# ChenyangQiQi/FateZero

Hardware: AMD Instinct MI355X
Metric: edited frames/sec (8f x 512^2 x 50 DDIM steps: capture inversion + 1 CFG edit, latents in/out) (higher is better)
Workload: dtype fp16; 1 GPU; config/teaser/jeep_posche.yaml shape: 8 x 512x512 (latents 8x64x64x4), 50-step DDIM inversion with HBM map capture + 50-step CFG edit (Replace, blend-masked self-attention), SD-1.x pseudo-3D UNet lora=160, random-init weights; frames=8, ddim_steps=50, n_edit=1, parallelism=single GPU, outputs_finite=True, n_ranks_seen=1

## Files before the change

fatezero_amd/_native.py:

```python
import ctypes as C
import os

HERE = os.path.dirname(os.path.abspath(__file__))
HIP_LIB = os.path.join(HERE, "libfatezero_hip.so")

FZ_ATTN_FLASH, FZ_ATTN_CAPTURE, FZ_ATTN_INJECT = 0, 1, 2
FZ_ATTN_CAPTURE8, FZ_ATTN_INJECT8 = 3, 4
FZ_MAX_KV_SLOTS = 4
FZ_CROSS_MAX_KEYS = 96
FZ_CROSS_P_STRIDE = 80
FZ_TEMPORAL_MAX_FRAMES = 256


class FzAttnSelfDesc(C.Structure):
    _fields_ = [
        ("n_frames", C.c_int32), ("frame0", C.c_int32), ("clip_len", C.c_int32), ("heads", C.c_int32),
        ("head_dim", C.c_int32), ("lq", C.c_int32), ("lkf", C.c_int32), ("n_kv", C.c_int32),
        ("kv_abs", C.c_int32 * FZ_MAX_KV_SLOTS), ("kv_val", C.c_int32 * FZ_MAX_KV_SLOTS),
        ("scale", C.c_float), ("mode", C.c_int32),
        ("q_frame_stride", C.c_int64), ("q_row_stride", C.c_int64),
        ("k_frame_stride", C.c_int64), ("k_row_stride", C.c_int64),
        ("vt_frame_stride", C.c_int64), ("vt_chan_stride", C.c_int64),
        ("o_frame_stride", C.c_int64), ("o_row_stride", C.c_int64),
        ("p_frame_stride", C.c_int64), ("p_head_stride", C.c_int64), ("p_row_stride", C.c_int64),
        ("p_frame_off", C.c_int32), ("mask_frame_off", C.c_int32),
        ("k_head_stride", C.c_int64),
        ("q_log2_scaled", C.c_int32), ("kv_clip_len", C.c_int32), ("kv_frame_off", C.c_int32), ("reserved0", C.c_int32),
    ]


class FzAttnCrossDesc(C.Structure):
    _fields_ = [
        ("n_frames", C.c_int32), ("frame0", C.c_int32), ("clip_len", C.c_int32), ("heads", C.c_int32),
        ("head_dim", C.c_int32), ("lq", C.c_int32), ("lk", C.c_int32),
        ("scale", C.c_float), ("mode", C.c_int32),
        ("q_frame_stride", C.c_int64), ("q_row_stride", C.c_int64),
        ("k_batch_stride", C.c_int64), ("k_row_stride", C.c_int64),
        ("vt_batch_stride", C.c_int64), ("vt_chan_stride", C.c_int64),
        ("o_frame_stride", C.c_int64), ("o_row_stride", C.c_int64),
        ("p_frame_stride", C.c_int64), ("p_head_stride", C.c_int64), ("p_row_stride", C.c_int64),
        ("p_frame_off", C.c_int32), ("store_cur", C.c_int32),
    ]


class FzGemmDesc(C.Structure):
    _fields_ = [
        ("rows", C.c_int64), ("rows_store", C.c_int64), ("in_features", C.c_int32), ("out_features", C.c_int32),
        ("ldx", C.c_int64), ("ldw", C.c_int64), ("ldy", C.c_int64), ("ldres", C.c_int64),
        ("batch", C.c_int32), ("epilogue", C.c_int32),
        ("x_batch_stride", C.c_int64), ("y_batch_stride", C.c_int64), ("res_batch_stride", C.c_int64),
        ("transpose_out", C.c_int32), ("tile_cfg", C.c_int32), ("split_k", C.c_int32), ("reserved0", C.c_int32),
        ("workspace_floats", C.c_int64), ("w_batch_stride", C.c_int64),
    ]


class FzXattnChain(C.Structure):
    _fields_ = [
        ("x", C.c_void_p), ("res", C.c_void_p), ("packed", C.c_void_p), ("kv_packed", C.c_void_p), ("bias_out", C.c_void_p),
        ("y", C.c_void_p), ("y_ln", C.c_void_p), ("ln_gamma", C.c_void_p), ("ln_beta", C.c_void_p),
        ("y1", C.c_void_p),
        ("rows", C.c_int64), ("rows_per_frame", C.c_int64),
        ("frames_per_batch", C.c_int32), ("channels", C.c_int32), ("heads", C.c_int32), ("lk", C.c_int32),
        ("scale", C.c_float), ("ln_eps", C.c_float), ("ln1_eps", C.c_float), ("front", C.c_int32),
    ]


FZ_GEMM_PLAIN, FZ_GEMM_GEGLU = 0, 1
FZ_GEMM_NO_STATS = 1

_P = C.c_void_p
_SIGS = {
    "fz_gemm": (C.c_int, [C.POINTER(FzGemmDesc), _P, _P, _P, _P, _P, _P, _P, _P]),
    "fz_ff_chain_ok": (C.c_int, [C.c_int64, C.c_int, C.c_int]),
    "fz_ff_chain_preferred": (C.c_int, [C.c_int64, C.c_int, C.c_int]),
    "fz_ff_chain_pack_bytes": (C.c_int64, [C.c_int, C.c_int]),
    "fz_ff_chain_pack": (C.c_int, [_P, _P, _P, _P, C.c_int, C.c_int, _P]),
    "fz_ff_chain": (C.c_int, [_P, _P, _P, _P, _P, _P, _P, C.c_float, _P, C.c_int64, C.c_int, C.c_int, _P]),
    "fz_xattn_chain_ok": (C.c_int, [C.c_int64, C.c_int64, C.c_int, C.c_int, C.c_int]),
    "fz_xattn_chain_preferred": (C.c_int, [C.c_int64, C.c_int64, C.c_int, C.c_int, C.c_int]),
    "fz_xattn_chain_pack_bytes": (C.c_int64, [C.c_int]),
    "fz_xattn_chain_kv_pack_bytes": (C.c_int64, [C.c_int]),
    "fz_xattn_chain_pack": (C.c_int, [_P, _P, _P, _P, _P, _P, _P, _P]),
    "fz_xattn_chain_kv_pack": (C.c_int, [_P, C.c_int64, C.c_int64, _P, C.c_int64, C.c_int64, C.c_int, C.c_int, _P, _P]),
    "fz_xattn_chain": (C.c_int, [C.POINTER(FzXattnChain), _P]),
    "fz_gemm_lnout": (C.c_int, [C.POINTER(FzGemmDesc), _P, _P, _P, _P, _P, _P, _P, _P, C.c_float, _P, C.c_int64, _P, _P]),
    "fz_gemm_qkvt": (C.c_int, [C.POINTER(FzGemmDesc), _P, _P, _P, _P, C.c_int, C.c_int64, C.c_int64, C.c_int64, _P]),
    "fz_gn_epilogue_chunks": (C.c_int, [C.c_int64]),
    "fz_gemm_gn": (C.c_int, [C.POINTER(FzGemmDesc), _P, _P, _P, _P, _P, _P, _P, C.c_int, C.c_int64, _P]),
    "fz_temporal_conv3_gn": (C.c_int, [_P, _P, _P, _P, _P, C.c_int64, _P, C.c_int, C.c_int, C.c_int, C.c_int, C.c_int, _P, C.c_int64,
                                       _P, C.c_int, _P]),
    "fz_groupnorm_from_partials": (C.c_int, [_P, _P, _P, _P, C.c_int, C.c_int, C.c_int, C.c_int, C.c_int, C.c_float, C.c_int, _P,
                                             C.c_int, _P, _P]),
    "fz_gemm_workspace_floats": (C.c_int64, [C.c_int64, C.c_int, C.c_int]),
    "fz_attn_self": (C.c_int, [C.POINTER(FzAttnSelfDesc), _P, _P, _P, _P, _P, _P, _P]),
    "fz_attn_cross": (C.c_int, [C.POINTER(FzAttnCrossDesc), _P, _P, _P, _P, _P, _P, _P, _P, _P]),
    "fz_attn_temporal": (C.c_int, [_P, _P, _P, _P, C.c_int, C.c_int, C.c_int, C.c_int, C.c_int, C.c_int64,
                                   C.c_int64, C.c_float, _P]),
    "fz_attn_temporal_ex": (C.c_int, [_P, _P, _P, _P, C.c_int, C.c_int, C.c_int, C.c_int, C.c_int, C.c_int, C.c_int64,
                                      C.c_int64, C.c_int64, C.c_float, _P]),
    "fz_blend_mask": (C.c_int, [_P, C.c_int, C.c_int, C.c_int64, C.c_int, C.c_int, C.c_int, C.c_int64, _P,
                                C.c_float, C.c_int, C.c_int, C.c_int, _P, _P, _P]),
    "fz_groupnorm_chunks": (C.c_int, [C.c_int, C.c_int]),
    "fz_groupnorm": (C.c_int, [_P, _P, _P, _P, C.c_int, C.c_int, C.c_int, C.c_int, C.c_int, C.c_float, C.c_int,
                               _P, _P]),
    "fz_groupnorm_cat": (C.c_int, [_P, C.c_int, _P, C.c_int, _P, _P, _P, C.c_int, C.c_int, C.c_int, C.c_int, C.c_float, C.c_int,
                                   _P, _P]),
    "fz_groupnorm_stats": (C.c_int, [_P, C.c_int, C.c_int, C.c_int, C.c_int, _P, _P]),
    "fz_groupnorm_apply": (C.c_int, [_P, _P, _P, _P, C.c_int, C.c_int, C.c_int, C.c_int, C.c_int, C.c_float, C.c_int, _P,
                                     C.c_int, C.c_int, _P, _P]),
    "fz_conv3x3_up2_ok": (C.c_int, [C.c_int, C.c_int, C.c_int, C.c_int, C.c_int]),
    "fz_conv3x3_up2_preferred": (C.c_int, [C.c_int, C.c_int, C.c_int, C.c_int, C.c_int]),
    "fz_conv3x3_up2_pack_halves": (C.c_int64, [C.c_int, C.c_int]),
    "fz_conv3x3_up2_pack": (C.c_int, [_P, _P, C.c_int, C.c_int, _P]),
    "fz_conv3x3_up2": (C.c_int, [_P, _P, _P, _P, C.c_int, C.c_int, C.c_int, C.c_int, C.c_int, _P]),
    "fz_conv3x3": (C.c_int, [_P, _P, _P, _P, C.c_int64, _P, _P, C.c_int, C.c_int, C.c_int, C.c_int, C.c_int, C.c_int,
                             C.c_int, C.c_int, _P, C.c_int64, C.c_int, C.c_int, _P]),
    "fz_temporal_conv3": (C.c_int, [_P, _P, _P, _P, _P, C.c_int64, _P, C.c_int, C.c_int, C.c_int, C.c_int, C.c_int, _P, C.c_int64,
                                    _P]),
    "fz_lora_pair_ok": (C.c_int, [C.c_int, C.c_int, C.c_int, C.c_int, C.c_int]),
    "fz_lora_pair_preferred": (C.c_int, [C.c_int, C.c_int, C.c_int, C.c_int, C.c_int]),
    "fz_lora_pair_gn_chunks": (C.c_int, [C.c_int, C.c_int, C.c_int, C.c_int, C.c_int, C.c_int]),
    "fz_lora_pair_gn": (C.c_int, [_P, _P, _P, _P, C.c_int64, _P, _P, C.c_int, C.c_int, C.c_int, C.c_int, C.c_int, _P, C.c_int, _P]),
    "fz_lora_pair": (C.c_int, [_P, _P, _P, _P, C.c_int64, _P, _P, C.c_int, C.c_int, C.c_int, C.c_int, C.c_int, _P]),
    "fz_layernorm": (C.c_int, [_P, _P, _P, _P, C.c_int64, C.c_int, C.c_float, _P]),
    "fz_geglu": (C.c_int, [_P, _P, C.c_int64, C.c_int, _P]),
    "fz_softmax_rows": (C.c_int, [_P, _P, C.c_int64, C.c_int, C.c_int64, C.c_int64, C.c_float, _P]),
    "fz_transpose_pad": (C.c_int, [_P, _P, C.c_int, C.c_int, C.c_int, C.c_int64, C.c_int64, C.c_int, _P]),
    "fz_latent_update": (C.c_int, [_P, _P, _P, C.c_float, C.c_float, C.c_float, _P, _P, _P, C.c_int, C.c_int, _P]),
    "fz_accumulate": (C.c_int, [_P, _P, C.c_int64, _P]),
    "fz_peer_put": (C.c_int, [_P, C.c_int64, _P, _P, C.c_int, C.c_uint32, _P, _P]),
    "fz_peer_wait": (C.c_int, [_P, C.c_uint64, C.c_uint32, _P, C.c_int64, _P]),
    "fz_plan_begin": (C.c_int, [C.POINTER(_P)]),
    "fz_plan_pause": (C.c_int, [_P, C.c_int]),
    "fz_plan_end": (C.c_int, [_P]),
    "fz_plan_launches": (C.c_int64, [_P]),
    "fz_plan_relocate": (C.c_int64, [_P, C.c_int64, C.c_int64, _P, C.c_int64, _P]),
    "fz_plan_replay": (C.c_int, [_P, C.c_int64, C.c_int64, _P]),
    "fz_plan_graph_launch": (C.c_int, [_P, _P]),
    "fz_plan_destroy": (None, [_P]),
    "fz_version": (C.c_char_p, []),
}

_lib = None
_lib_path = None
_is_test_backend = False


class NativeLibraryError(RuntimeError):
    pass


def _open(path):
    if not os.path.exists(path):
        raise NativeLibraryError(
            f"{path} is missing: build it with `python -m fatezero_amd.build` (hipcc --offload-arch=gfx950). "
            "The FateZero hot path has no CPU fallback.")
    try:
        lib = C.CDLL(path)
    except OSError as e:
        raise NativeLibraryError(f"cannot load {path}: {e}") from e
    for name, (res, args) in _SIGS.items():
        try:
# ... 43 lines not shown
```

fatezero_amd/csrc/elementwise.hip:

```cpp
#include "fz_rt.h"
#include "../../include/fatezero_hip.h"

FZ_KERNEL void __launch_bounds__(256) geglu_kernel(const half_t* __restrict__ x, half_t* __restrict__ y, int64_t rows, int inner) {
    const int vper = inner >> 3;
    const int64_t total = rows * vper;
    for (int64_t i = (int64_t)blockIdx.x * blockDim.x + threadIdx.x; i < total; i += (int64_t)gridDim.x * blockDim.x) {
        const int64_t r = i / vper;
        const int v = (int)(i % vper);
        const half8_t hv = fz_ld_h8(x + r * 2 * inner + v * 8);
        const half8_t gv = fz_ld_h8(x + r * 2 * inner + inner + v * 8);
        half8_t o;
#pragma unroll
        for (int e = 0; e < 8; ++e) {
            const float g = (float)gv[e];
            const float ge = fz_gelu_erf(g);
            o[e] = (half_t)((float)hv[e] * ge);
        }
        fz_st_h8(y + r * inner + v * 8, o);
    }
}

extern "C" int fz_geglu(const void* x, void* y, int64_t rows, int inner, void* stream) {
    if (!x || !y || rows <= 0 || inner <= 0 || (inner & 7)) return FZ_ERR_BAD_ARG;
    const int64_t total = rows * (inner >> 3);
// ... 139 lines not shown
        nx[c] = (half_t)zn;
    }
    if (next_in != nullptr) *reinterpret_cast<half4_t*>(next_in + i * 4) = nx;
}

extern "C" int fz_latent_update(float* z, const void* eps_u, const void* eps_c, float guidance, float cz, float ce,
                                const float* inv, const float* mask, void* next_in, int frames, int hw, void* stream) {
    if (!z || !eps_c || frames <= 0 || hw <= 0) return FZ_ERR_BAD_ARG;
    if ((mask != nullptr) != (inv != nullptr)) return FZ_ERR_BAD_ARG;
    const int64_t total = (int64_t)frames * hw;
    FZ_LAUNCH(latent_update_kernel, dim3((unsigned)((total + 255) / 256)), dim3(256), 0, stream, z, (const half_t*)eps_u,
              (const half_t*)eps_c, guidance, cz, ce, inv, mask, (half_t*)next_in, frames, hw);
    return fz_last_launch_status();
}

FZ_KERNEL void __launch_bounds__(256) accumulate_kernel(float* __restrict__ acc, const half_t* __restrict__ x, int64_t n8) {
    for (int64_t i = (int64_t)blockIdx.x * blockDim.x + threadIdx.x; i < n8; i += (int64_t)gridDim.x * blockDim.x) {
        const half8_t v = fz_ld_h8(x + i * 8);
        float* a = acc + i * 8;
#pragma unroll
        for (int e = 0; e < 8; ++e) a[e] += (float)v[e];
    }
}

extern "C" int fz_accumulate(float* acc, const void* x, int64_t n, void* stream) {
    if (!acc || !x || n <= 0 || (n & 7)) return FZ_ERR_BAD_ARG;
    const int64_t n8 = n >> 3;
    int blocks = (int)((n8 + 255) / 256);
    if (blocks > 4096) blocks = 4096;
    FZ_LAUNCH(accumulate_kernel, dim3(blocks), dim3(256), 0, stream, acc, (const half_t*)x, n8);
    return fz_last_launch_status();
}

extern "C" const char* fz_version(void) {
#ifdef FZ_EMU
    return "fatezero_amd 0.1 (CPU emulation build -- tests only)";
#else
    return "fatezero_amd 0.1 (hip gfx950)";
#endif
}
```

fatezero_amd/csrc/igemm.hip:

```cpp
#include "fz_rt.h"
#include <type_traits>
#include <atomic>
#include <utility>
#include <stdlib.h>
#include "../../include/fatezero_hip.h"

#ifdef FZ_IGEMM_TRIALS
__attribute__((weak)) int fz_igemm_trial_no_pp = 0;
extern "C" { __attribute__((weak)) int fz_igemm_trial_no_kg2 = 0; __attribute__((weak)) int fz_igemm_trial_no_halo = 0; __attribute__((weak)) int fz_igemm_trial_no_halo_split = 0; }
__attribute__((weak)) int fz_igemm_trial_pp_splitk_min = 0;
#endif
#ifdef FZ_IGEMM_TUNING
#define FZ_TUNING_FLAG(name) (getenv(name) != nullptr)
#else
#define FZ_TUNING_FLAG(name) false
#endif
#ifndef FZ_A_AUX
#define FZ_A_AUX 0
#endif
#define FZ_PP_ON 1
#define FZ_PP_NOPRIO 2
#define FZ_PP_NOSTAGGER 4
#define FZ_PP_PREP_IN_R 8
#define FZ_PP_K32 16
// ... 4 lines not shown
#ifdef FZ_IGEMM_TIMING
__device__ long long fz_igemm_timing[2][8];
__device__ long long fz_igemm_timing2[2][6];
#define FZ_TK_DECL() long long tacc_[8] = {0, 0, 0, 0, 0, 0, 0, 0}
#define FZ_TK(i)                              \
    __builtin_amdgcn_sched_barrier(0);        \
    const long long tk##i = clock64();        \
    __builtin_amdgcn_sched_barrier(0)
#define FZ_TK_ADD(slot, a, b) tacc_[slot] += (b) - (a)
#define FZ_TK_FLUSH()                                                                                      \
    do {                                                                                                   \
        if (blockIdx.x == 0 && blockIdx.y == 0 && blockIdx.z == 0 && (tid & 255) == 0)                     \
            for (int s_ = 0; s_ < 8; ++s_) fz_igemm_timing[tid >> 8][s_] = tacc_[s_];                       \
    } while (0)
#else
#define FZ_TK_DECL() ((void)0)
#define FZ_TK(i) ((void)0)
#define FZ_TK_ADD(slot, a, b) ((void)0)
#define FZ_TK_FLUSH() ((void)0)
#endif

FZ_DEVICE_GLOBAL __attribute__((aligned(16))) half_t fz_zero_page[8192];

struct IgArgs {
    const half_t* a;
    const half_t* b;
    half_t* y;
    float* part;
    const half_t* bias;
    const half_t* temb;
    const half_t* res;
    const half_t* res2;
    int64_t lda, ldb, ldy, ldres, a_bs, b_bs, y_bs, res_bs, temb_stride;
    int64_t Nb;
    int64_t temb_group;
    int Ma, Ma_store;
    int Cin, taps, kchunks;
    int N, Hi, Wi, Ho, Wo, stride, upsample, fpb;
    int ksplit, tiles_a;
    int group_b;
    int tiles_b;
    int nt_flat;
    half_t* yt;
    int64_t yt_bs, ldyt;
    int vt_split, vt_rows;
    float* gs_out;
    int gs_cpg, gs_groups, gs_chunks, gs_rpf;
    half_t* lno_y;
    const half_t* lno_gamma;
    const half_t* lno_beta;
    int64_t lno_ld;
    float lno_eps;
};

template <int WA, int TA, int WB, int TB, int BK, int NS, bool GEGLU, int PP = 0>
struct IgCfg {
    static_assert(BK == 32 || BK == 64, "K step of 32 or 64 halves");
    static_assert(!(PP & FZ_PP_ON) || (BK == 32 && NS == 4 && WA * WB == 8), "ping-pong loop: K step 32, 4 slots, 8 waves = two groups of 4");
    static constexpr bool LC = (PP & FZ_LC) != 0;
    static_assert(!LC || (!(PP & (FZ_PP_ON | FZ_KG2)) && BK == 32 && NS == 4 && WA * WB == 4), "loader / consumer loop: K step 32, 4 slots, 4 + 4 waves");
    static constexpr int KG = (PP & FZ_KG2) ? 2 : 1;
    static constexpr bool KGPP = (PP & FZ_KGPP) != 0;
    static_assert(KG == 1 || (!(PP & FZ_PP_ON) && (KGPP ? (BK == 32 && NS == 4) : BK == 64)), "K groups: ring loop with K step 64, or their own ping-pong loop");
    static_assert(!KGPP || KG == 2, "the K-group ping-pong loop needs the two groups");
    static constexpr int NWG = WA * WB;
    static constexpr int NW = (LC ? 2 : KG) * NWG, T = 64 * NW;
// ... 796 lines not shown
                            *reinterpret_cast<half4_t*>(crow + (wa * TA / 2 + i / 2) * 32 + 8 * gq + 4 * hi) = v;
                        }
                } else {
#pragma unroll
                    for (int i = 0; i < TA; ++i)
#pragma unroll
                        for (int gq = 0; gq < 4; ++gq) {
                            half4_t v;
                            if constexpr (VT) {
                                f32x2 pk;
                                pk[0] = acc[i][j][4 * gq];
                                pk[1] = acc[i][j][4 * gq + 1];
                                v = __builtin_bit_cast(half4_t, pk);
                            } else {
#pragma unroll
                                for (int e = 0; e < 4; ++e) v[e] = (half_t)acc[i][j][4 * gq + e];
                            }
                            *reinterpret_cast<half4_t*>(crow + (wa * TA + i) * 32 + 8 * gq + 4 * hi) = v;
                        }
                }
            }
        }
        __syncthreads();
        for (int id = tid; id < C::RP * OCH; id += C::T) {
            const int pl = id / OCH, ch = id - pl * OCH;
            const int64_t px = b0 + ps * C::RP + pl;
            const int co = o0 + ch * 8;
            if (px >= g.Nb || co >= Mo_store) continue;
            const half8_t v = fz_ld_h8(Cs + pl * C::CSTR + ch * 8);
            float f[8];
#pragma unroll
            for (int e = 0; e < 8; ++e) f[e] = co + e < Mo ? (float)v[e] : 0.0f;
            const bool full = vec_ok && co + 8 <= Mo;
            if (full) {
                if (g.temb != nullptr) {
                    const half8_t t = fz_ld_h8(g.temb + (px / g.temb_group) * g.temb_stride + co);
#pragma unroll
                    for (int e = 0; e < 8; ++e) f[e] += (float)t[e];
                }
                if (R1 != nullptr) {
                    const half8_t r = fz_ld_h8(R1 + px * g.ldres + co);
#pragma unroll
                    for (int e = 0; e < 8; ++e) f[e] += (float)r[e];
                }
                if (R2 != nullptr) {
                    const half8_t r = fz_ld_h8(R2 + px * g.ldres + co);
#pragma unroll
                    for (int e = 0; e < 8; ++e) f[e] += (float)r[e];
                }
            } else {
                if (g.temb != nullptr) {
                    const half_t* t = g.temb + (px / g.temb_group) * g.temb_stride + co;
                    for (int e = 0; e < 8; ++e)
                        if (co + e < Mo) f[e] += (float)t[e];
                }
                if (R1 != nullptr) {
                    const half_t* r = R1 + px * g.ldres + co;
                    for (int e = 0; e < 8; ++e)
                        if (co + e < Mo) f[e] += (float)r[e];
                }
                if (R2 != nullptr) {
                    const half_t* r = R2 + px * g.ldres + co;
                    for (int e = 0; e < 8; ++e)
                        if (co + e < Mo) f[e] += (float)r[e];
                }
            }
            half_t* dst = Y + px * g.ldy + co;
            if (full) {
                half8_t o;
#pragma unroll
                for (int e = 0; e < 8; ++e) o[e] = (half_t)f[e];
                fz_st_h8(dst, o);
                if constexpr (GS != 0) fz_st_h8(Cs + pl * C::CSTR + ch * 8, o);
            } else {
#pragma unroll
                for (int e = 0; e < 8; ++e)
                    if (co + e < Mo_store) dst[e] = (half_t)f[e];
            }
        }
        if constexpr (GS == -1) {
            static_assert(C::CW == 320, "the tile must hold whole 320-channel rows");
            __syncthreads();
            const int l8 = tid & 7;
            FzRow5 gmv, btv;
#pragma unroll
            for (int i = 0; i < 5; ++i) {
                gmv.c[i] = fz_ld_h8(g.lno_gamma + (l8 + 8 * i) * 8);
                btv.c[i] = fz_ld_h8(g.lno_beta + (l8 + 8 * i) * 8);
            }
            for (int rb = tid >> 3; rb < C::RP; rb += C::T >> 3) {
// ... 58 lines not shown
                float* out = g.gs_out + ((fr * g.gs_groups + (a0 / cpg + tid)) * g.gs_chunks + chunk) * 3;
                out[0] = cnt;
                out[1] = mean;
                out[2] = m2;
            }
        }
    }
#ifdef FZ_IGEMM_TIMING
    if (blockIdx.x == 0 && blockIdx.y == 0 && blockIdx.z == 0 && (tid & 255) == 0) {
        fz_igemm_timing2[tid >> 8][0] = tk_setup;
        fz_igemm_timing2[tid >> 8][1] = clock64() - tk_entry;
        fz_igemm_timing2[tid >> 8][2] = tw_entry;
        fz_igemm_timing2[tid >> 8][3] = tw_loop;
        fz_igemm_timing2[tid >> 8][4] = tw_loop_end;
        fz_igemm_timing2[tid >> 8][5] = wall_clock64();
    }
#endif
}

FZ_KERNEL void __launch_bounds__(256) igemm_reduce_kernel(IgArgs g, int batch) {
    const int q = g.Ma / 4;
    const int cl = threadIdx.x & 63, rl = fz_uniform((int)(threadIdx.x >> 6));
    const int64_t rows = g.Nb * batch;
    for (int64_t row = (int64_t)blockIdx.x * 4 + rl; row < rows; row += (int64_t)gridDim.x * 4) {
        int z = 0;
        int64_t px = row;
        if (batch > 1) {
            z = (int)(row / g.Nb);
            px = row - (int64_t)z * g.Nb;
        }
        const float* const p0 = g.part + row * g.Ma;
        const int64_t slab = (int64_t)batch * g.Nb * g.Ma;
        const half_t* const trow = g.temb != nullptr ? g.temb + (px / g.temb_group) * g.temb_stride : nullptr;
        const half_t* const r1 = g.res != nullptr ? g.res + (int64_t)z * g.res_bs + px * g.ldres : nullptr;
        const half_t* const r2 = g.res2 != nullptr ? g.res2 + (int64_t)z * g.res_bs + px * g.ldres : nullptr;
        half_t* const yrow = g.y + (int64_t)z * g.y_bs + px * g.ldy;
        const int c4 = (int)blockIdx.y * 64 + cl;
        if (c4 < q) {
            const int co = c4 * 4;
            f32x4 s = *reinterpret_cast<const f32x4*>(p0 + co);
            for (int k = 1; k < g.ksplit; ++k) {
                const f32x4 t = *reinterpret_cast<const f32x4*>(p0 + k * slab + co);
                s += t;
            }
            float f[4] = {s[0], s[1], s[2], s[3]};
            if (g.bias != nullptr)
                for (int e = 0; e < 4; ++e) f[e] += (float)g.bias[co + e];
            if (trow != nullptr)
                for (int e = 0; e < 4; ++e) f[e] += (float)trow[co + e];
            if (r1 != nullptr)
                for (int e = 0; e < 4; ++e) f[e] += (float)r1[co + e];
            if (r2 != nullptr)
                for (int e = 0; e < 4; ++e) f[e] += (float)r2[co + e];
            half4_t o;
            for (int e = 0; e < 4; ++e) o[e] = (half_t)f[e];
            *reinterpret_cast<half4_t*>(yrow + co) = o;
        }
    }
}

template <int CIN>
FZ_KERNEL void __launch_bounds__(256) conv3x3_small_cin_kernel(IgArgs g) {
    FZ_DYN_SMEM(raw);
    half_t* wl = reinterpret_cast<half_t*>(raw);
    const int kk = 9 * g.Cin;
    for (int id = threadIdx.x; id < kk * g.Ma; id += 256) {
        const int k = id / g.Ma, co = id - k * g.Ma;
// ... 336 lines not shown
        if (GEGLU || workspace == nullptr || (g.Ma % 4) || g.Ma_store != g.Ma || (g.ldy % 4)) return FZ_ERR_UNSUPPORTED;
        if ((int64_t)ksplit * batch * g.Nb * g.Ma > workspace_floats) return FZ_ERR_BAD_ARG;
        g.part = workspace;
    }
    const int rc = ig_dispatch_cfg<MODE, GEGLU>(cfg, g, batch, stream);
    if (rc != FZ_OK || ksplit == 1) return rc != FZ_OK ? rc : (gs_dropped ? FZ_GEMM_NO_STATS : FZ_OK);
    const int64_t rblocks = (g.Nb * batch + 3) / 4;
    dim3 grid((unsigned)(rblocks < 16384 ? rblocks : 16384), (unsigned)((g.Ma / 4 + 63) / 64)), block(256);
    FZ_LAUNCH(igemm_reduce_kernel, grid, block, 0, stream, g, batch);
    const int rc2 = fz_last_launch_status();
    return rc2 != FZ_OK ? rc2 : (gs_dropped ? FZ_GEMM_NO_STATS : FZ_OK);
}

extern "C" int64_t fz_gemm_workspace_floats(int64_t rows, int out_features, int batch) {
    const int64_t out = rows * (int64_t)out_features * (batch > 0 ? batch : 1);
    const int64_t cap = 64ll << 20;
    return 8 * out < cap ? 8 * out : (2 * out < cap ? cap : 2 * out);
}

extern "C" int fz_gemm(const FzGemmDesc* d, const void* x, const void* w, const void* bias, const void* res, const void* res2,
                       void* y, void* workspace, void* stream) {
    if (!d || !x || !w || !y || d->rows <= 0 || d->in_features <= 0 || d->out_features <= 0) return FZ_ERR_BAD_ARG;
    const int batch = d->batch > 0 ? d->batch : 1;
    IgArgs g = {};
    g.taps = 1;
    g.fpb = 1;
    g.Cin = d->in_features;
    g.temb = nullptr;
    g.temb_group = 1;
    g.res = (const half_t*)res;
    g.res2 = (const half_t*)res2;
    g.ldres = d->ldres ? d->ldres : d->ldy;
    g.res_bs = d->res_batch_stride;
    g.y = (half_t*)y;
    g.ldy = d->ldy;
    g.y_bs = d->y_batch_stride;
    if (d->ldx < d->in_features || d->ldw < d->in_features || (d->ldx % 8) || (d->ldw % 8)) return FZ_ERR_BAD_ARG;
    const bool geglu = d->epilogue == FZ_GEMM_GEGLU;
    if (d->epilogue != FZ_GEMM_PLAIN && !geglu) return FZ_ERR_BAD_ARG;
    if (!d->transpose_out) {
        g.a = (const half_t*)w;
        g.lda = d->ldw;
        g.a_bs = d->w_batch_stride;
        g.Ma = d->out_features;
        g.Ma_store = d->out_features;
        g.b = (const half_t*)x;
        g.ldb = d->ldx;
        g.b_bs = d->x_batch_stride;
        g.Nb = d->rows;
        g.bias = (const half_t*)bias;
        const int outw = geglu ? d->out_features / 2 : d->out_features;
        if (d->ldy < outw) return FZ_ERR_BAD_ARG;
        if (geglu) {
            if (d->out_features % 64 || res || res2) return FZ_ERR_UNSUPPORTED;
            return ig_run<0, true>(g, batch, d->tile_cfg, 1, nullptr, 0, stream);
        }
        return ig_run<0, false>(g, batch, d->tile_cfg, d->split_k, (float*)workspace, d->workspace_floats, stream);
    }
    if (geglu || bias || res || res2) return FZ_ERR_UNSUPPORTED;
    if (d->rows >= (1ll << 31)) return FZ_ERR_UNSUPPORTED;
    g.a = (const half_t*)x;
    g.lda = d->ldx;
    g.a_bs = d->x_batch_stride;
    g.Ma = (int)d->rows;
    g.Ma_store = d->rows_store > d->rows ? (int)d->rows_store : (int)d->rows;
    g.b = (const half_t*)w;
// ... 107 lines not shown
        (g.ldy % 8) || (g.ldres % 8) || (g.temb != nullptr && (g.temb_stride % 8))) return false;
    g.gs_out = partial;
    g.gs_cpg = cpg;
    g.gs_groups = groups;
    g.gs_rpf = (int)rows_per_frame;
    g.gs_chunks = (int)(rows_per_frame / 128);
    return true;
}

extern "C" int fz_gn_epilogue_chunks(int64_t rows_per_frame) { return rows_per_frame % 128 == 0 ? (int)(rows_per_frame / 128) : 0; }

extern "C" int fz_gemm_gn(const FzGemmDesc* d, const void* x, const void* w, const void* bias, const void* res, const void* res2, void* y,
                          float* gn_partial, int gn_groups, int64_t rows_per_frame, void* stream) {
    if (!d || !x || !w || !y || !gn_partial || d->rows <= 0 || d->in_features <= 0 || d->out_features <= 0) return FZ_ERR_BAD_ARG;
    if (d->epilogue != FZ_GEMM_PLAIN || d->transpose_out || d->batch > 1 || d->w_batch_stride) return FZ_ERR_UNSUPPORTED;
    if (d->ldx < d->in_features || d->ldw < d->in_features || (d->ldx % 8) || (d->ldw % 8) || d->ldy < d->out_features) return FZ_ERR_BAD_ARG;
    IgArgs g = {};
    g.taps = 1;
    g.fpb = 1;
    g.Cin = d->in_features;
    g.temb_group = 1;
    g.a = (const half_t*)w;
    g.lda = d->ldw;
    g.Ma = g.Ma_store = d->out_features;
    g.b = (const half_t*)x;
    g.ldb = d->ldx;
    g.Nb = d->rows;
    g.bias = (const half_t*)bias;
    g.res = (const half_t*)res;
    g.res2 = (const half_t*)res2;
    g.y = (half_t*)y;
    g.ldy = d->ldy;
    g.ldres = d->ldres ? d->ldres : d->ldy;
    const bool want = ig_gs_setup(g, gn_partial, gn_groups, rows_per_frame);
    const int rc = ig_run<0, false>(g, 1, d->tile_cfg, 1, nullptr, 0, stream);
    return rc != FZ_OK ? rc : (want ? FZ_OK : FZ_GEMM_NO_STATS);
}

extern "C" int fz_gemm_lnout(const FzGemmDesc* d, const void* x, const void* w, const void* bias, const void* res, const void* res2, void* y,
                             const void* gamma, const void* beta, float eps, void* y_ln, int64_t ld_ln, void* workspace, void* stream) {
    if (!d || !x || !w || !y || !gamma || !beta || !y_ln || d->rows <= 0 || d->in_features <= 0 || d->out_features <= 0) return FZ_ERR_BAD_ARG;
    if (d->epilogue != FZ_GEMM_PLAIN || d->transpose_out || d->batch > 1 || d->w_batch_stride) return FZ_ERR_UNSUPPORTED;
    if (d->ldx < d->in_features || d->ldw < d->in_features || (d->ldx % 8) || (d->ldw % 8) || d->ldy < d->out_features || ld_ln < d->out_features)
        return FZ_ERR_BAD_ARG;
    IgArgs g = {};
    g.taps = 1;
    g.fpb = 1;
    g.Cin = d->in_features;
    g.temb_group = 1;
    g.a = (const half_t*)w;
    g.lda = d->ldw;
    g.Ma = g.Ma_store = d->out_features;
    g.b = (const half_t*)x;
    g.ldb = d->ldx;
    g.Nb = d->rows;
    g.bias = (const half_t*)bias;
    g.res = (const half_t*)res;
    g.res2 = (const half_t*)res2;
    g.y = (half_t*)y;
    g.ldy = d->ldy;
    g.ldres = d->ldres ? d->ldres : d->ldy;
    g.lno_y = (half_t*)y_ln;
    g.lno_gamma = (const half_t*)gamma;
    g.lno_beta = (const half_t*)beta;
    g.lno_ld = ld_ln;
    g.lno_eps = eps;
    return ig_run<0, false>(g, 1, d->tile_cfg, d->split_k, (float*)workspace, d->workspace_floats, stream);
}

static int temporal_conv3_impl(const void* x, const void* wt, const void* res, const void* res2, const void* temb, int64_t temb_stride,
                               void* y, int n, int tokens, int cin, int cout, int clip_len, void* workspace, int64_t workspace_floats,
                               float* gn_partial, int gn_groups, void* stream);

extern "C" int fz_temporal_conv3_gn(const void* x, const void* wt, const void* res, const void* res2, const void* temb,
                                    int64_t temb_stride, void* y, int n, int tokens, int cin, int cout, int clip_len, void* workspace,
                                    int64_t workspace_floats, float* gn_partial, int gn_groups, void* stream) {
    if (!gn_partial || gn_groups <= 0) return FZ_ERR_BAD_ARG;
    return temporal_conv3_impl(x, wt, res, res2, temb, temb_stride, y, n, tokens, cin, cout, clip_len, workspace, workspace_floats,
                               gn_partial, gn_groups, stream);
}

extern "C" int fz_temporal_conv3(const void* x, const void* wt, const void* res, const void* res2, const void* temb,
                                int64_t temb_stride, void* y, int n, int tokens, int cin, int cout, int clip_len,
                                void* workspace, int64_t workspace_floats, void* stream) {
    return temporal_conv3_impl(x, wt, res, res2, temb, temb_stride, y, n, tokens, cin, cout, clip_len, workspace, workspace_floats, nullptr,
                               0, stream);
}

static int temporal_conv3_impl(const void* x, const void* wt, const void* res, const void* res2, const void* temb, int64_t temb_stride,
                               void* y, int n, int tokens, int cin, int cout, int clip_len, void* workspace, int64_t workspace_floats,
                               float* gn_partial, int gn_groups, void* stream) {
    if (!x || !wt || !y || n <= 0 || tokens <= 0 || clip_len <= 0 || n % clip_len) return FZ_ERR_BAD_ARG;
    IgArgs g = {};
    g.taps = 3;
// ... 97 lines not shown
```

fatezero_amd/csrc/norms.hip:

```cpp
#include "fz_rt.h"
#include "../../include/fatezero_hip.h"
#include <stdlib.h>

static int gn_tb(int tokens, int channels) {
    const int V = channels / 8;
    const int R = V >= 256 ? 1 : 256 / (V > 0 ? V : 1);
    int tb = 64;
    while (tb > 8 && tb > 16 * R) tb >>= 1;
    while (tb > 8 && tokens / tb < 32) tb >>= 1;
    return tb;
}

extern "C" int fz_groupnorm_chunks(int tokens, int channels) {
    const int tb = gn_tb(tokens, channels);
    return (tokens + tb - 1) / tb;
}

struct GnArgs {
    const half_t* x;
    const half_t* x2;
    int C1;
    half_t* y;
    const half_t *gamma, *beta;
    float* partial;
    float* stats;
    int n_frames, span, tokens, C, G, chunks, V, R;
    int tb;
    int fin_span;
    int pchunks;
    float eps;
    int silu;
};

template <int ROWS>
FZ_KERNEL void __launch_bounds__(ROWS > 0 ? 512 : 1024) gn_stats_kernel(GnArgs a) {
    FZ_DYN_SMEM(raw);
    float* red = reinterpret_cast<float*>(raw);
    float* gmean = red + a.R * a.C;
    const int tid = threadIdx.x, v = tid % a.V, r = tid / a.V;
    const int chunk = blockIdx.x, n = blockIdx.y;
    const int t0 = chunk * a.tb;
    const int t1 = min(t0 + a.tb, a.tokens);
    const int cg = a.C / a.G;
    const float cnt = (float)((t1 - t0) * cg);
    const bool second = v * 8 >= a.C1;
    const int64_t rs = second ? a.C - a.C1 : a.C1;
    const half_t* base = (second ? a.x2 + ((int64_t)n * a.tokens) * rs + (v * 8 - a.C1) : a.x + ((int64_t)n * a.tokens) * rs + v * 8);
    float s[8];
#pragma unroll
    for (int e = 0; e < 8; ++e) s[e] = 0.0f;
    half8_t xr[ROWS > 0 ? ROWS : 1];
    if (ROWS > 0) {
#pragma unroll
        for (int i = 0; i < ROWS; ++i) {
            int t = t0 + r + i * a.R;
            t = t < t1 ? t : t1 - 1;
            xr[i] = fz_ld_h8(base + (int64_t)t * rs);
        }
#pragma unroll
        for (int i = 0; i < ROWS; ++i) {
            if (t0 + r + i * a.R < t1) {
#pragma unroll
                for (int e = 0; e < 8; ++e) s[e] += (float)xr[i][e];
            }
        }
    } else {
        for (int t = t0 + r; t < t1; t += a.R) {
            const half8_t xv = fz_ld_h8(base + (int64_t)t * rs);
#pragma unroll
            for (int e = 0; e < 8; ++e) s[e] += (float)xv[e];
        }
    }
#pragma unroll
    for (int e = 0; e < 8; ++e) red[r * a.C + v * 8 + e] = s[e];
    __syncthreads();
    if (tid < a.G) {
        float sum = 0.0f;
        for (int rr = 0; rr < a.R; ++rr)
            for (int c = tid * cg; c < (tid + 1) * cg; ++c) sum += red[rr * a.C + c];
        gmean[tid] = sum / cnt;
// ... 116 lines not shown
    const int sp = (int)blockIdx.x / a.G, g = (int)blockIdx.x % a.G;
    const int wave = threadIdx.x >> 6, lane = threadIdx.x & 63;
    const int total = a.fin_span * a.pchunks, per = (total + 3) / 4;
    float cnt, mean, m2;
    gn_merge_range(a, sp, g, lane, min(wave * per, total), min((wave + 1) * per, total), cnt, mean, m2);
    if (lane == 0) { part[wave][0] = cnt; part[wave][1] = mean; part[wave][2] = m2; }
    __syncthreads();
    if (threadIdx.x == 0) {
        cnt = part[0][0]; mean = part[0][1]; m2 = part[0][2];
        for (int w = 1; w < 4; ++w) chan_merge(cnt, mean, m2, part[w][0], part[w][1], part[w][2]);
        a.stats[(sp * a.G + g) * 2 + 0] = mean;
        a.stats[(sp * a.G + g) * 2 + 1] = 1.0f / sqrtf(m2 / cnt + a.eps);
    }
}

FZ_KERNEL void gn_apply_kernel(GnArgs a) {
    const int tid = threadIdx.x, v = tid % a.V, r = tid / a.V;
    const int chunk = blockIdx.x, n = blockIdx.y;
    const int t0 = chunk * a.tb;
    const int t1 = min(t0 + a.tb, a.tokens);
    const int cg = a.C / a.G;
    const int sp = n / a.span;
    float sc[8], sh[8];
    const half8_t gv = fz_ld_h8(a.gamma + v * 8), bv = fz_ld_h8(a.beta + v * 8);
#pragma unroll
    for (int e = 0; e < 8; ++e) {
        const int g = (v * 8 + e) / cg;
        const float mean = a.stats[(sp * a.G + g) * 2 + 0], rstd = a.stats[(sp * a.G + g) * 2 + 1];
        sc[e] = rstd * (float)gv[e];
        sh[e] = (float)bv[e] - mean * sc[e];
    }
    const bool second = v * 8 >= a.C1;
    const int64_t rs = second ? a.C - a.C1 : a.C1;
    const half_t* xb = (second ? a.x2 + ((int64_t)n * a.tokens) * rs + (v * 8 - a.C1) : a.x + ((int64_t)n * a.tokens) * rs + v * 8);
    half_t* yb = a.y + ((int64_t)n * a.tokens) * a.C + v * 8;
#pragma unroll 4
    for (int t = t0 + r; t < t1; t += a.R) {
        const half8_t xv = fz_ld_h8(xb + (int64_t)t * rs);
        half8_t yv;
#pragma unroll
        for (int e = 0; e < 8; ++e) {
            float f = (float)xv[e] * sc[e] + sh[e];
            if (a.silu) f = f / (1.0f + __builtin_expf(-f));
            yv[e] = (half_t)f;
        }
        fz_st_h8(yb + (int64_t)t * a.C, yv);
    }
}

#define GN_FUSED_THREADS 1024
#define GN_FUSED_MAX_NE 20
#define GN_FUSED_MAX_PAIRS (GN_FUSED_THREADS * GN_FUSED_MAX_NE)

FZ_DEVICE float gn_block_sum(float v, float* red, int tid) {
#pragma unroll
    for (int msk = 1; msk < 64; msk <<= 1) v += fz_shfl_xor(v, msk);
    __syncthreads();
    if ((tid & 63) == 0) red[tid >> 6] = v;
    __syncthreads();
    float s = 0.0f;
#pragma unroll
    for (int w = 0; w < GN_FUSED_THREADS / 64; ++w) s += red[w];
    return s;
}

template <int NE>
FZ_KERNEL void __launch_bounds__(GN_FUSED_THREADS) gn_fused_kernel(GnArgs a) {
    FZ_SHARED float red[GN_FUSED_THREADS / 64];
    FZ_SHARED float gsc[128], gsh[128];
    const int tid = threadIdx.x;
    const int sp = (int)blockIdx.x / a.G, g = (int)blockIdx.x % a.G;
    const int cg = a.C / a.G, P = cg >> 1;
    const int total = a.span * a.tokens * P;
    const int c0 = g * cg;
    const int64_t row0 = (int64_t)sp * a.span * a.tokens;
    const uint32_t rs1 = (uint32_t)a.C1, rs2 = (uint32_t)(a.C - a.C1);
    const half_t* const src1 = a.x + row0 * a.C1;
    const half_t* const src2 = a.x2 != nullptr ? a.x2 + row0 * (a.C - a.C1) : src1;
    half_t* const dst = a.y + row0 * a.C + c0;
    const int drow = GN_FUSED_THREADS / P, dpr = GN_FUSED_THREADS - drow * P;
    const int row = tid / P, pr = tid - row * P;
    const int last_row = a.span * a.tokens - 1;
    half2_t v[NE];
    {
        int r = row, q = pr;
#pragma unroll
        for (int i = 0; i < NE; ++i) {
            const int rr = r < last_row ? r : last_row;
            const uint32_t ch = (uint32_t)(c0 + 2 * q);
            const half_t* p = ch >= rs1 ? src2 + ((uint32_t)rr * rs2 + (ch - rs1)) : src1 + ((uint32_t)rr * rs1 + ch);
            v[i] = *reinterpret_cast<const half2_t*>(p);
            FZ_SCHED_FENCE();
            r += drow;
            q += dpr;
            if (q >= P) { q -= P; ++r; }
        }
    }
    const float cnt = (float)total * 2.0f;
    float s = 0.0f;
#pragma unroll
    for (int i = 0; i < NE; ++i)
        if (tid + GN_FUSED_THREADS * i < total) s += (float)v[i][0] + (float)v[i][1];
    const float mean = gn_block_sum(s, red, tid) / cnt;
#pragma unroll
    for (int i = 0; i < NE; ++i) FZ_PIN_V(v[i]);
    s = 0.0f;
#pragma unroll
    for (int i = 0; i < NE; ++i)
        if (tid + GN_FUSED_THREADS * i < total) {
            const float d0 = (float)v[i][0] - mean, d1 = (float)v[i][1] - mean;
            s += d0 * d0 + d1 * d1;
// ... 19 lines not shown
                float f1 = (float)v[i][1] * gsc[2 * q + 1] + gsh[2 * q + 1];
                if (a.silu) {
                    f0 = f0 / (1.0f + __builtin_expf(-f0));
                    f1 = f1 / (1.0f + __builtin_expf(-f1));
                }
                half2_t o;
                o[0] = (half_t)f0;
                o[1] = (half_t)f1;
                *reinterpret_cast<half2_t*>(dst + ((uint32_t)r * (uint32_t)a.C + 2u * (uint32_t)q)) = o;
            }
            FZ_SCHED_FENCE();
            r += drow;
            q += dpr;
            if (q >= P) { q -= P; ++r; }
        }
    }
}

#ifdef FZ_GN_TRIALS
template <int NE>
FZ_KERNEL void __launch_bounds__(GN_FUSED_THREADS) gn_fused2_kernel(GnArgs a) {
    FZ_SHARED float red[GN_FUSED_THREADS / 64];
    const int tid = threadIdx.x;
    const int sp = (int)blockIdx.x / a.G, g = (int)blockIdx.x % a.G;
    const int cg = a.C / a.G, P = cg >> 1;
    const int R = GN_FUSED_THREADS / P;
    const int rows = a.span * a.tokens;
    const int r0 = tid / P, q = tid - r0 * P;
    const bool active = r0 < R;
    const int ch = g * cg + 2 * q;
    const int64_t row0 = (int64_t)sp * rows;
    const bool second = ch >= a.C1;
    const uint32_t rs = (uint32_t)(second ? a.C - a.C1 : a.C1);
    const half_t* const src = second ? a.x2 + row0 * (a.C - a.C1) + (ch - a.C1) : a.x + row0 * a.C1 + ch;
    half_t* const dst = a.y + row0 * a.C + ch;
    const uint32_t step_in = (uint32_t)R * rs, step_out = (uint32_t)R * (uint32_t)a.C;
    const int r_first = active ? r0 : 0;
    half2_t v[NE];
    {
        uint32_t off = (uint32_t)r_first * rs;
        const uint32_t off_max = (uint32_t)(rows - 1) * rs;
#pragma unroll
        for (int i = 0; i < NE; ++i) {
            v[i] = *reinterpret_cast<const half2_t*>(src + (off < off_max ? off : off_max));
            FZ_SCHED_FENCE();
            off += step_in;
        }
    }
    const int r_lim = active ? rows - r0 : 0;
    const float cnt = (float)rows * (float)cg;
    float s = 0.0f;
#pragma unroll
    for (int i = 0; i < NE; ++i)
        if (i * R < r_lim) s += (float)v[i][0] + (float)v[i][1];
    const float mean = gn_block_sum(s, red, tid) / cnt;
#pragma unroll
    for (int i = 0; i < NE; ++i) FZ_PIN_V(v[i]);
    s = 0.0f;
#pragma unroll
    for (int i = 0; i < NE; ++i)
        if (i * R < r_lim) {
            const float d0 = (float)v[i][0] - mean, d1 = (float)v[i][1] - mean;
            s += d0 * d0 + d1 * d1;
        }
    const float var = gn_block_sum(s, red, tid) / cnt;
    const float rstd = 1.0f / sqrtf(var + a.eps);
#pragma unroll
// ... 55 lines not shown
    } else if (ne <= 4) {
        FZ_LAUNCH(gn_fused_kernel<4>, grid, block, 0, stream, a);
    } else if (ne <= 5) {
        FZ_LAUNCH(gn_fused_kernel<5>, grid, block, 0, stream, a);
    } else if (ne <= 8) {
        FZ_LAUNCH(gn_fused_kernel<8>, grid, block, 0, stream, a);
    } else if (ne <= 10) {
        FZ_LAUNCH(gn_fused_kernel<10>, grid, block, 0, stream, a);
    } else if (ne <= 16) {
        FZ_LAUNCH(gn_fused_kernel<16>, grid, block, 0, stream, a);
    } else {
        FZ_LAUNCH(gn_fused_kernel<GN_FUSED_MAX_NE>, grid, block, 0, stream, a);
    }
    return true;
}

static void gn_launch_stats(const GnArgs& a, dim3 grid, dim3 block, size_t smem, void* stream) {
    const int rows = (a.tb + a.R - 1) / a.R;
    if (rows > 32 || block.x > 512) {
        FZ_LAUNCH(gn_stats_kernel<0>, grid, block, smem, stream, a);
    } else if (rows <= 12) {
        FZ_LAUNCH(gn_stats_kernel<12>, grid, block, smem, stream, a);
    } else if (rows <= 24) {
        FZ_LAUNCH(gn_stats_kernel<24>, grid, block, smem, stream, a);
    } else {
        FZ_LAUNCH(gn_stats_kernel<32>, grid, block, smem, stream, a);
    }
}

static int gn_setup(GnArgs& a, int n_frames, int span, int tokens, int channels, int groups, int& threads, size_t& smem) {
    if (n_frames <= 0 || span <= 0 || n_frames % span || channels % 8 || channels % groups || groups > 64)
        return FZ_ERR_BAD_ARG;
    a.n_frames = n_frames; a.span = span; a.fin_span = span; a.tokens = tokens; a.C = channels; a.G = groups;
    a.tb = gn_tb(tokens, channels);
    a.chunks = fz_groupnorm_chunks(tokens, channels);
    a.pchunks = a.chunks;
    a.V = channels / 8;
    if (a.V > 1024) return FZ_ERR_UNSUPPORTED;
    a.R = a.V >= 256 ? 1 : 256 / a.V;
    if (a.V * a.R < 64) return FZ_ERR_UNSUPPORTED;
    threads = a.V * a.R;
    smem = ((size_t)a.R * channels + groups) * sizeof(float);
    return FZ_OK;
}

extern "C" int fz_groupnorm(const void* x, void* y, const void* gamma, const void* beta, int n_frames, int span,
                            int tokens, int channels, int groups, float eps, int silu, float* partial, void* stream) {
    if (!x || !y || !gamma || !beta || !partial) return FZ_ERR_BAD_ARG;
    GnArgs a;
    int threads;
    size_t smem;
    const int rc = gn_setup(a, n_frames, span, tokens, channels, groups, threads, smem);
    if (rc != FZ_OK) return rc;
    a.x = (const half_t*)x; a.x2 = nullptr; a.C1 = channels;
    a.y = (half_t*)y; a.gamma = (const half_t*)gamma; a.beta = (const half_t*)beta;
    a.eps = eps; a.silu = silu;
    a.partial = partial;
    a.stats = partial + (int64_t)n_frames * a.chunks * groups * 3;
    if (gn_try_fused(a, stream)) return fz_last_launch_status();
    dim3 grid(a.chunks, n_frames), block(threads);
    gn_launch_stats(a, grid, block, smem, stream);
    const int nst = (n_frames / span) * groups;
    FZ_LAUNCH(gn_finalize_kernel, dim3(nst), dim3(64), 0, stream, a);
    FZ_LAUNCH(gn_apply_kernel, grid, block, 0, stream, a);
    return fz_last_launch_status();
}

extern "C" int fz_groupnorm_cat(const void* x1, int channels1, const void* x2, int channels2, void* y, const void* gamma,
                                const void* beta, int n_frames, int span, int tokens, int groups, float eps, int silu, float* partial,
                                void* stream) {
    if (!x1 || !x2 || !y || !gamma || !beta || !partial || channels1 <= 0 || channels2 <= 0 || (channels1 % 8) || (channels2 % 8))
        return FZ_ERR_BAD_ARG;
    GnArgs a;
    int threads;
    size_t smem;
    const int rc = gn_setup(a, n_frames, span, tokens, channels1 + channels2, groups, threads, smem);
    if (rc != FZ_OK) return rc;
    a.x = (const half_t*)x1; a.x2 = (const half_t*)x2; a.C1 = channels1;
    a.y = (half_t*)y; a.gamma = (const half_t*)gamma; a.beta = (const half_t*)beta;
    a.eps = eps; a.silu = silu;
    a.partial = partial;
    a.stats = partial + (int64_t)n_frames * a.chunks * groups * 3;
    if (gn_try_fused(a, stream)) return fz_last_launch_status();
    dim3 grid(a.chunks, n_frames), block(threads);
    gn_launch_stats(a, grid, block, smem, stream);
    FZ_LAUNCH(gn_finalize_kernel, dim3((n_frames / span) * groups), dim3(64), 0, stream, a);
    FZ_LAUNCH(gn_apply_kernel, grid, block, 0, stream, a);
    return fz_last_launch_status();
}

extern "C" int fz_groupnorm_stats(const void* x, int n_frames, int tokens, int channels, int groups, float* partial,
                                  void* stream) {
    if (!x || !partial) return FZ_ERR_BAD_ARG;
    GnArgs a;
    int threads;
    size_t smem;
    const int rc = gn_setup(a, n_frames, 1, tokens, channels, groups, threads, smem);
    if (rc != FZ_OK) return rc;
    a.x = (const half_t*)x; a.x2 = nullptr; a.C1 = channels;
    a.y = nullptr; a.gamma = nullptr; a.beta = nullptr; a.eps = 0.0f; a.silu = 0;
    a.partial = partial; a.stats = nullptr;
    gn_launch_stats(a, dim3(a.chunks, n_frames), dim3(threads), smem, stream);
    return fz_last_launch_status();
}

extern "C" int fz_groupnorm_apply(const void* x, void* y, const void* gamma, const void* beta, int n_frames, int span,
                                  int tokens, int channels, int groups, float eps, int silu, const float* partial_all,
                                  int stat_sets, int frames_per_set, float* stats, void* stream) {
    if (!x || !y || !gamma || !beta || !partial_all || !stats || stat_sets <= 0 || frames_per_set <= 0) return FZ_ERR_BAD_ARG;
    GnArgs a;
    int threads;
// ... 134 lines not shown
```

fatezero_amd/csrc/xattn_chain.hip:

```cpp
#include "fz_rt.h"
#include <atomic>
#include <type_traits>
#include "../../include/fatezero_hip.h"

namespace {
constexpr int XC_C = 320;
constexpr int XC_H = 8, XC_D = 40;
constexpr int XC_KS = XC_C / 16;
constexpr int XC_CT = XC_C / 32;
constexpr int XC_ROWS = 128;
constexpr int XC_FRAG = 1024;
constexpr int XC_SLOTF = 41;
constexpr int XC_SLOT = XC_SLOTF * XC_FRAG;
constexpr int XC_NSLOT = 3;
constexpr int XC_HOFF = XC_NSLOT * XC_SLOT;
constexpr int XC_HPAIR = 8;
constexpr int XC_HBYTES = 4 * XC_HPAIR * XC_FRAG;
constexpr int XC_COFF = XC_HOFF + XC_HBYTES;
constexpr int XC_CBYTES = 2 * XC_FRAG;
constexpr size_t XC_LDS_BYTES = XC_COFF + XC_CBYTES;
constexpr int XC_OSTR = XC_C + 8;
constexpr int XC_BLK = 110;
constexpr int XC_NBLK = 5;
constexpr int XC_KVH = 21;
// ... 27 lines not shown
template <typename T>
FZ_DEVICE T* xc_uniform_ptr(T* p) {
#ifdef FZ_EMU
    return p;
#else
    const uint64_t v = (uint64_t)(uintptr_t)p;
    const uint32_t lo = __builtin_amdgcn_readfirstlane((uint32_t)v), hi = __builtin_amdgcn_readfirstlane((uint32_t)(v >> 32));
    return reinterpret_cast<T*>((uintptr_t)(((uint64_t)hi << 32) | lo));
#endif
}

#ifdef XC_TIMING
__device__ long long xc_timing[2][8];
#define XC_TK(i) __builtin_amdgcn_sched_barrier(0); const long long tk##i = clock64(); __builtin_amdgcn_sched_barrier(0)
#define XC_TK_ADD(slot, a, b) tacc[slot] += (b) - (a)
#else
#define XC_TK(i) ((void)0)
#define XC_TK_ADD(slot, a, b) ((void)0)
#endif

struct XcArgs {
    const half_t* xn;
    const half_t* res;
    const char* wpack;
    const char* kvpack;
    const half_t* bo;
    half_t* y;
    half_t* yln;
    const half_t* gamma;
    const half_t* beta;
    half_t* y1;
    int64_t rows, rows_per_frame;
    int frames_per_batch, lk;
    float cs;
    float eps, eps1;
};

template <bool FRONT>
FZ_KERNEL void __launch_bounds__(512, 2) xattn_chain_kernel(XcArgs g) {
    FZ_DYN_SMEM(raw);
    const int tid = threadIdx.x, wave = fz_uniform(tid >> 6), lane = tid & 63, l31 = lane & 31, hi = lane >> 5;
    const bool is_qa = wave < 4;
    const int pair = wave & 3;
    const int nt = gridDim.x, bid = blockIdx.x;
    const int q8 = nt >> 3, r8 = nt & 7, xcd = bid & 7;
    const int blk = (xcd < r8 ? xcd * (q8 + 1) : r8 * (q8 + 1) + (xcd - r8) * q8) + (bid >> 3);
    const int64_t row0 = (int64_t)blk * XC_ROWS + pair * 32;
    const int batch = (int)(((int64_t)blk * XC_ROWS / g.rows_per_frame) / g.frames_per_batch);
    const char* const kv = g.kvpack + (int64_t)batch * (XC_H * XC_KVH * XC_FRAG);
    const char* const wmain = g.wpack + (FRONT ? XC_FRONTF * XC_FRAG : 0);
    unsigned char* const hbase = raw + XC_HOFF + pair * XC_HPAIR * XC_FRAG;
    const uint32_t lane_off = (uint32_t)lane * 16u;
    constexpr int NSTEP = (FRONT ? XC_FRONT_STEPS : 0) + XC_MAIN_STEPS;

    const int w4 = wave & 3;
    auto dma = [&](const char* src, int n, unsigned char* dst) __attribute__((always_inline)) {
#pragma unroll
        for (int i = 0; i < 10; ++i) {
            const int j = w4 + 4 * i;
            if (j < n) fz_glds16_so(xc_uniform_ptr(src + j * XC_FRAG), lane_off, xc_uniform_ptr(dst + j * XC_FRAG));
        }
    };
    auto slot_of = [&](int n) __attribute__((always_inline)) -> unsigned char* { return raw + (n % XC_NSLOT) * XC_SLOT; };
    auto issue_step = [&](int n) __attribute__((always_inline)) {
        unsigned char* dst = slot_of(n);
        if (FRONT && n < XC_FRONT_STEPS) {
            dma(g.wpack + (2 + (n < 4 ? 30 * n : 120 + 40 * (n - 4))) * XC_FRAG, n < 4 ? 30 : 40, dst);
            return;
        }
        const int m = n - (FRONT ? XC_FRONT_STEPS : 0), hp = m >> 2, k = m & 3;
        const char* b = wmain + hp * (XC_BLK * XC_FRAG);
        if (k == 0) {
            if (hp < 4) dma(b, 30, dst);
        } else if (k == 1) {
            if (hp < 4) dma(b + 30 * XC_FRAG, 30, dst);
            if (hp >= 1) dma(b + 60 * XC_FRAG, 10, dst + 30 * XC_FRAG);
        } else {
            if (hp < 4) dma(kv + (2 * hp + (k - 2)) * (XC_KVH * XC_FRAG), XC_KVH, dst);
            if (hp >= 1) dma(b + (k == 2 ? 70 : 90) * XC_FRAG, 20, dst + XC_KVH * XC_FRAG);
        }
    };
    const int my_parity = is_qa ? 0 : 1;
    int step = 0;
#ifdef XC_TIMING
    long long tacc[8] = {0, 0, 0, 0, 0, 0, 0, 0};
    const long long tk_start = clock64();
#endif
    auto sync_step = [&]() __attribute__((always_inline)) {
        XC_TK(0);
        if ((step & 1) == my_parity) fz_wait_vm0();
        XC_TK(1);
        fz_barrier_nodrain();
        XC_TK(2);
        if ((step & 1) == my_parity && step + 2 < NSTEP) issue_step(step + 2);
        XC_TK(3);
        XC_TK_ADD(0, tk0, tk1);
        XC_TK_ADD(1, tk1, tk2);
        XC_TK_ADD(2, tk2, tk3);
        ++step;
    };
    auto slot_base = [&](int n) __attribute__((always_inline)) -> fz_lds_addr { return fz_lds_addr_of(slot_of(n)) + lane_off; };

    f32x16 yacc[XC_CT];

    if (is_qa) {
        half8_t xb[XC_KS];
        const int64_t row = row0 + l31;
        {
            const half_t* src = g.xn + row * XC_C + hi * 8;
#pragma unroll
            for (int s = 0; s < XC_KS; ++s) xb[s] = fz_ld_h8(src + s * 16);
        }
#pragma unroll
        for (int s = 0; s < XC_KS; ++s) FZ_PIN_V(xb[s]);
        issue_step(0);

        if constexpr (FRONT) {
            half8_t hv[XC_KS];
            const unsigned char* const cst = raw + XC_COFF + (hi * 8) * 2;
            half8_t rv[8];
            auto take_rv = [&](int nf) __attribute__((always_inline)) {
#pragma unroll
                for (int f = 0; f < 8; ++f)
                    if (f < nf) rv[f] = *reinterpret_cast<const half8_t*>(hbase + f * XC_FRAG + lane_off);
            };
            auto front_pass = [&](auto T0c, auto NTc, auto RV0c, auto TAKEc) __attribute__((always_inline)) {
                constexpr int T0 = decltype(T0c)::value, NT = decltype(NTc)::value, RV0 = decltype(RV0c)::value, TAKE = decltype(TAKEc)::value;
                constexpr int NSUB = NT == 3 ? 2 : 1, KPS = XC_KS / NSUB;
                f32x16 acc[NT];
#pragma unroll
                for (int c = 0; c < NT; ++c) acc[c] = fz_zero_f16v();
#pragma unroll
                for (int q = 0; q < NSUB; ++q) {
                    const int n = step;
                    sync_step();
                    if (q == 0 && TAKE > 0) take_rv(TAKE);
                    const fz_lds_addr base = slot_base(n);
                    half8_t fa[2 * NT], fb[2 * NT];
                    auto ldf = [&](half8_t* f, int kk) __attribute__((always_inline)) {
#pragma unroll
                        for (int i = 0; i < 2 * NT; ++i) f[i] = fz_lds_ld_h8(base, (kk * NT + i) * XC_FRAG);
                    };
// ... 215 lines not shown
                sync_step();
                if (live) {
                    XC_TK(6);
                    head(qf, slot_base(n), oga);
                    XC_TK(7);
                    XC_TK_ADD(6, tk6, tk7);
                    *reinterpret_cast<half8_t*>(hbase + lane_off) = oga[0];
                    *reinterpret_cast<half8_t*>(hbase + XC_FRAG + lane_off) = oga[1];
                }
            }
            {
                const int n = step;
                sync_step();
                if (live) {
                    XC_TK(6);
                    head(qf + 3, slot_base(n), ogb);
                    XC_TK(7);
                    XC_TK_ADD(6, tk6, tk7);
                    half8_t mid;
#pragma unroll
                    for (int e = 0; e < 8; ++e) mid[e] = hi ? ogb[2][e] : oga[2][e];
                    *reinterpret_cast<half8_t*>(hbase + 2 * XC_FRAG + lane_off) = mid;
                    *reinterpret_cast<half8_t*>(hbase + 3 * XC_FRAG + lane_off) = ogb[0];
                    *reinterpret_cast<half8_t*>(hbase + 4 * XC_FRAG + lane_off) = ogb[1];
                }
            }
        }
    } else {
        fz_setprio_hi();
#pragma unroll
        for (int c = 0; c < XC_CT; ++c) yacc[c] = fz_zero_f16v();
        if constexpr (FRONT) {
            const int64_t row = row0 + l31;
            const half_t* rs = g.res + row * XC_C + hi * 8;
            half8_t ra[8];
#pragma unroll
            for (int f = 0; f < 6; ++f) ra[f] = fz_ld_h8(rs + f * 16);
            if (w4 == 0) {
                fz_glds16_so(xc_uniform_ptr(g.wpack), lane_off, xc_uniform_ptr(raw + XC_COFF));
                fz_glds16_so(xc_uniform_ptr(g.wpack + XC_FRAG), lane_off, xc_uniform_ptr(raw + XC_COFF + XC_FRAG));
            }
            issue_step(1);
            fz_wait_vm0();
#pragma unroll
            for (int f = 0; f < 6; ++f) *reinterpret_cast<half8_t*>(hbase + f * XC_FRAG + lane_off) = ra[f];
            sync_step();
#pragma unroll
            for (int f = 0; f < 6; ++f) ra[f] = fz_ld_h8(rs + (6 + f) * 16);
            fz_wait_vm0();
#pragma unroll
            for (int f = 0; f < 6; ++f) FZ_PIN_V(ra[f]);
            fz_barrier_nodrain();
            if (step + 2 < NSTEP) issue_step(step + 2);
            ++step;
#pragma unroll
            for (int f = 0; f < 6; ++f) *reinterpret_cast<half8_t*>(hbase + f * XC_FRAG + lane_off) = ra[f];
            sync_step();
#pragma unroll
            for (int f = 0; f < 8; ++f) ra[f] = fz_ld_h8(rs + (12 + f) * 16);
            fz_wait_vm0();
#pragma unroll
            for (int f = 0; f < 8; ++f) FZ_PIN_V(ra[f]);
            fz_barrier_nodrain();
            if (step + 2 < NSTEP) issue_step(step + 2);
            ++step;
#pragma unroll
            for (int f = 0; f < 8; ++f) *reinterpret_cast<half8_t*>(hbase + f * XC_FRAG + lane_off) = ra[f];
// ... 38 lines not shown
#pragma unroll
                for (int c = 0; c < XC_CT; ++c) yacc[c] = fz_mfma_32x32x16_f16(fb[c], hf[2 * k - 2], yacc[c]);
            }
        }
    }

#ifdef XC_TIMING
    tacc[3] = clock64() - tk_start;
#endif
    fz_wait_vm0();
    __syncthreads();
    half_t* Call = reinterpret_cast<half_t*>(raw);
    if (!is_qa) {
        half_t* Cs = Call + pair * 32 * XC_OSTR;
#pragma unroll
        for (int c = 0; c < XC_CT; ++c)
#pragma unroll
            for (int gq = 0; gq < 4; ++gq) {
                const int co = c * 32 + 8 * gq + 4 * hi;
                half4_t bv;
                if (g.bo != nullptr) {
                    bv = *reinterpret_cast<const half4_t*>(g.bo + co);
                } else {
#pragma unroll
                    for (int e = 0; e < 4; ++e) bv[e] = (half_t)0.0f;
                }
                half4_t v;
#pragma unroll
                for (int e = 0; e < 4; ++e) v[e] = (half_t)(yacc[c][4 * gq + e] + (float)bv[e]);
                *reinterpret_cast<half4_t*>(Cs + l31 * XC_OSTR + co) = v;
            }
    }
    __syncthreads();
    const half_t* resp = FRONT ? g.y1 : g.res;
    const int l8 = lane & 7;
    FzRow5 gmv, btv;
    if (g.yln != nullptr) {
#pragma unroll
        for (int i = 0; i < 5; ++i) {
            gmv.c[i] = fz_ld_h8(g.gamma + (l8 + 8 * i) * 8);
            btv.c[i] = fz_ld_h8(g.beta + (l8 + 8 * i) * 8);
        }
    }
#pragma unroll
    for (int it = 0; it < 2; ++it) {
        const int rl = wave * 16 + it * 8 + (lane >> 3);
        const int64_t px = (int64_t)blk * XC_ROWS + rl;
        FzRow5 v;
#pragma unroll
        for (int i = 0; i < 5; ++i) {
            const half8_t a = fz_ld_h8(Call + rl * XC_OSTR + (l8 + 8 * i) * 8);
            float f[8];
#pragma unroll
            for (int e = 0; e < 8; ++e) f[e] = (float)a[e];
            if (resp != nullptr) {
                const half8_t r = fz_ld_h8(resp + px * XC_C + (l8 + 8 * i) * 8);
#pragma unroll
                for (int e = 0; e < 8; ++e) f[e] += (float)r[e];
            }
#pragma unroll
            for (int e = 0; e < 8; ++e) v.c[i][e] = (half_t)f[e];
            fz_st_h8(g.y + px * XC_C + (l8 + 8 * i) * 8, v.c[i]);
        }
#ifdef XC_DEBUG_XN
        continue;
#endif
        if (g.yln == nullptr) continue;
// ... 100 lines not shown

extern "C" int fz_xattn_chain_preferred(int64_t rows, int64_t rows_per_frame, int channels, int heads, int lk) {
    return fz_xattn_chain_ok(rows, rows_per_frame, channels, heads, lk) && rows >= 128 * 192;
}

extern "C" int64_t fz_xattn_chain_pack_bytes(int with_front) { return (int64_t)((with_front ? XC_FRONTF : 0) + XC_NBLK * XC_BLK) * XC_FRAG; }

extern "C" int64_t fz_xattn_chain_kv_pack_bytes(int batch) { return batch > 0 ? (int64_t)batch * XC_H * XC_KVH * XC_FRAG : 0; }

extern "C" int fz_xattn_chain_pack(const void* wq, const void* wo, const void* wo1, const void* bias_out1, const void* ln1_gamma,
                                   const void* ln1_beta, void* packed, void* stream) {
    if (!wq || !wo || !packed) return FZ_ERR_BAD_ARG;
    if (wo1 != nullptr && (!ln1_gamma || !ln1_beta)) return FZ_ERR_BAD_ARG;
    XcPackArgs g = {(const half_t*)wq, (const half_t*)wo, (const half_t*)wo1, (const half_t*)bias_out1, (const half_t*)ln1_gamma,
                    (const half_t*)ln1_beta, (char*)packed};
    const int64_t total = fz_xattn_chain_pack_bytes(wo1 != nullptr) / 16;
    FZ_LAUNCH(xattn_chain_pack_kernel, dim3((unsigned)((total + 255) / 256)), dim3(256), 0, stream, g);
    return fz_last_launch_status();
}

extern "C" int fz_xattn_chain_kv_pack(const void* k, int64_t k_batch_stride, int64_t k_row_stride, const void* vt, int64_t vt_batch_stride,
                                      int64_t vt_chan_stride, int batch, int lk, void* packed, void* stream) {
    if (!k || !vt || !packed || batch <= 0 || lk <= 0 || lk > FZ_CROSS_MAX_KEYS) return FZ_ERR_BAD_ARG;
    if ((k_batch_stride | k_row_stride | vt_batch_stride | vt_chan_stride) & 7) return FZ_ERR_BAD_ARG;
    XcKvArgs g = {(const half_t*)k, (const half_t*)vt, (char*)packed, k_batch_stride, k_row_stride, vt_batch_stride, vt_chan_stride, batch, lk};
    const int64_t total = fz_xattn_chain_kv_pack_bytes(batch) / 16;
    FZ_LAUNCH(xattn_chain_kv_pack_kernel, dim3((unsigned)((total + 255) / 256)), dim3(256), 0, stream, g);
    return fz_last_launch_status();
}

extern "C" int fz_xattn_chain(const FzXattnChain* d, void* stream) {
    if (!d || !d->x || !d->packed || !d->kv_packed || !d->y) return FZ_ERR_BAD_ARG;
    if (!fz_xattn_chain_ok(d->rows, d->rows_per_frame, d->channels, d->heads, d->lk)) return FZ_ERR_UNSUPPORTED;
    if (d->frames_per_batch <= 0) return FZ_ERR_BAD_ARG;
    if (d->y_ln != nullptr && (!d->ln_gamma || !d->ln_beta)) return FZ_ERR_BAD_ARG;
    const bool front = d->front != 0;
    if (front && (!d->res || !d->y1)) return FZ_ERR_BAD_ARG;
    XcArgs g = {};
    g.xn = (const half_t*)d->x;
    g.res = (const half_t*)d->res;
    g.wpack = (const char*)d->packed;
    g.kvpack = (const char*)d->kv_packed;
    g.bo = (const half_t*)d->bias_out;
    g.y = (half_t*)d->y;
    g.yln = (half_t*)d->y_ln;
    g.gamma = (const half_t*)d->ln_gamma;
    g.beta = (const half_t*)d->ln_beta;
    g.y1 = (half_t*)d->y1;
    g.rows = d->rows;
    g.rows_per_frame = d->rows_per_frame;
    g.frames_per_batch = d->frames_per_batch;
    g.lk = d->lk;
    g.cs = d->scale * 1.4426950408889634f;
    g.eps = d->ln_eps;
    g.eps1 = d->ln1_eps;
    const int64_t nwg = d->rows / XC_ROWS;
#ifndef FZ_EMU
    static std::atomic<uint64_t> attr_set_mask[2] = {{0}, {0}};
    int dev = 0;
    if (hipGetDevice(&dev) != hipSuccess) return FZ_ERR_LAUNCH;
    if (dev >= 64 || !(attr_set_mask[front].load(std::memory_order_relaxed) >> dev & 1)) {
        const void* fn = front ? reinterpret_cast<const void*>(&xattn_chain_kernel<true>) : reinterpret_cast<const void*>(&xattn_chain_kernel<false>);
        if (hipFuncSetAttribute(fn, hipFuncAttributeMaxDynamicSharedMemorySize, (int)XC_LDS_BYTES) != hipSuccess) return FZ_ERR_LAUNCH;
        if (dev < 64) attr_set_mask[front].fetch_or(1ull << dev, std::memory_order_relaxed);
    }
#endif
    if (front) {
        FZ_LAUNCH(xattn_chain_kernel<true>, dim3((unsigned)nwg), dim3(512), XC_LDS_BYTES, stream, g);
    } else {
        FZ_LAUNCH(xattn_chain_kernel<false>, dim3((unsigned)nwg), dim3(512), XC_LDS_BYTES, stream, g);
    }
    return fz_last_launch_status();
}
```

fatezero_amd/issue.py:

```python
import ctypes as C
import os

import torch
from torch.utils._python_dispatch import TorchDispatchMode

from . import _native as N
from . import kernels as K

_TENSOR_FIELDS = ("p", "row_mask", "mapper_t", "coef", "cur_out", "capture_first")
_PARK_BASE = 0x7000_0000_0000_0000

_ALLOC_OPS = {"aten.empty.memory_format", "aten.empty_like.default", "aten.empty_strided.default", "aten.new_empty.default",
              "aten.new_empty_strided.default"}
_VIEW_OPS = {"aten.view.default", "aten._unsafe_view.default", "aten.reshape.default", "aten._reshape_alias.default", "aten.as_strided.default",
             "aten.slice.Tensor", "aten.select.int", "aten.permute.default", "aten.transpose.int", "aten.t.default", "aten.expand.default",
             "aten.unsqueeze.default", "aten.squeeze.dim", "aten.squeeze.default", "aten.detach.default", "aten.alias.default",
             "aten.split.Tensor", "aten.split_with_sizes.default", "aten.unbind.int", "aten.narrow.default", "aten.unflatten.int",
             "aten.flatten.using_ints", "aten.chunk.default", "aten.view_as.default", "aten.lift_fresh.default", "aten.unfold.default",
             "aten.movedim.int"}


class _Watch(TorchDispatchMode):

    def __init__(self, rec):
# ... 45 lines not shown
                    self.pool_ctx = self.enter_pool()
                    self.pool_ctx.__enter__()
        N.check(L.fz_plan_pause(self.handle, 1), "fz_plan_pause")
        if self.pool_ctx is not None:
            self.pool_ctx.__exit__(None, None, None)
            self.pool_ctx = None
        self.live += 1
        try:
            plan = planner(*args)
        finally:
            self.live -= 1
            if self.enter_pool is not None:
                self.pool_ctx = self.enter_pool()
                self.pool_ctx.__enter__()
            N.check(L.fz_plan_pause(self.handle, 0), "fz_plan_pause")
        self.events.append(_Event(args, int(L.fz_plan_launches(self.handle)), plan))
        return plan


class PlanMismatch(RuntimeError):
    """A replay met a forward its plan does not describe (another kind of controller step, a tensor of another size, an argument word
    that is not the pointer it was taken for)."""


_recording = None
ENABLED = True


def recording():
    return _recording


def _model_switches():
    from .video_diffusion.models import attention as A, lora as Lo, resnet as R
    return (A.QKV_FUSION, A.LN_FROM_PRODUCER, R.GN_FROM_EPILOGUE, Lo.LORA_PAIR_FUSION, Lo.LORA_PAIR_GN, Lo.LORA_PAIR_ALWAYS)


class ForwardPlan:

    def __init__(self, handle, events, keep, out, inputs, n_launches, ctx_kv, scratch=()):
        self.handle, self.events, self.keep, self.out = handle, events, keep, out
        self.scratch = list(scratch)
        self.graph_ok = True
        self.inputs = inputs
        self.n = n_launches
        self.ctx_kv = ctx_kv
        self.replays = 0
        self._lib = N.lib()

    def __del__(self):
        try:
            if self.handle is not None:
                self._lib.fz_plan_destroy(self.handle)
                self.handle = None
        except Exception:
            pass

    def _relocate(self, first, count, slot, tensor, what):
        ptr = tensor.data_ptr()
        if ptr == slot[0]:
            return
        nbytes = tensor.numel() * tensor.element_size()
        if nbytes != slot[1]:
            raise PlanMismatch(f"issue plan: {what} changed size ({slot[1]} -> {nbytes} bytes): the plan does not describe this forward")
        self._move(first, count, slot, nbytes, ptr, what)

    def _move(self, first, count, slot, nbytes, new_ptr, what):
        n = N.lib().fz_plan_relocate(self.handle, first, count, C.c_void_p(slot[0]), nbytes, C.c_void_p(new_ptr))
# ... 80 lines not shown
class IssuePlans:
    MAX_PLANS = 8
    _pool = None

    def __init__(self, unet, graph=None):
        self.unet = unet
        self.graph = (os.environ.get("FZ_ISSUE_GRAPH", "1") != "0") if graph is None else bool(graph)
        self.seen = {}
        self.plans = {}
        self._probe = None
        self.stats = {"walked": 0, "recorded": 0, "replayed": 0, "contexts_bound": 0, "unsupported": 0, "unrecordable": []}

    def _controller(self):
        if self._probe is None:
            from .video_diffusion.models.attention import CrossAttention
            self._probe = next(m for m in self.unet.modules() if isinstance(m, CrossAttention))
        return self._probe.controller

    def clear(self):
        self.seen.clear()
        self.plans.clear()

    def _key(self, x, temb_act, ctx, controller):
        from . import dist as D
        if D.active_shard() is not None or x.data.dtype != torch.float16 or not x.data.is_contiguous():
            return None
        if controller is None:
            sig = ("none",)
        else:
            sig_fn = getattr(controller, "issue_signature", None)
            sig = None if sig_fn is None or getattr(controller, "attention_plan", None) is None else sig_fn()
            if sig is None:
                return None
        return (tuple(x.data.shape), x.b, x.f, x.h, x.w, str(x.data.device), K._scratch_key(x.data)[1], tuple(temb_act.shape), tuple(ctx.shape),
                ctx.dtype, type(controller), sig, _model_switches())

    @classmethod
    def _pool_entry(cls, device):
        if torch.device(device).type != "cuda":
            return None
        if cls._pool is None:
            cls._pool = torch.cuda.MemPool()
        pool = cls._pool
        return lambda: torch.cuda.use_mem_pool(pool, device=device)

    def _record(self, key, x, temb_act, ctx, controller):
        global _recording
        L = N.lib()
        handle = C.c_void_p()
        N.check(L.fz_plan_begin(C.byref(handle)), "fz_plan_begin")
        enter_pool = self._pool_entry(x.data.device)
        rec = _Recording(handle, None if enter_pool is not None else [])
        rec.enter_pool = enter_pool
        _recording = rec
        try:
            with _Watch(rec):
                if enter_pool is not None:
                    rec.pool_ctx = enter_pool()
                    rec.pool_ctx.__enter__()
                try:
                    out = self.unet._forward_body(x, temb_act, ctx)
                finally:
                    if rec.pool_ctx is not None:
                        rec.pool_ctx.__exit__(None, None, None)
                        rec.pool_ctx = None
        except BaseException:
            _recording = None
# ... 96 lines not shown
```

fatezero_amd/kernels.py:

```python
import ctypes as C
from typing import List, Optional, Sequence, Tuple

import torch

from . import _native as N

FZ_ATTN_FLASH, FZ_ATTN_CAPTURE, FZ_ATTN_INJECT = N.FZ_ATTN_FLASH, N.FZ_ATTN_CAPTURE, N.FZ_ATTN_INJECT
FZ_ATTN_CAPTURE8, FZ_ATTN_INJECT8 = N.FZ_ATTN_CAPTURE8, N.FZ_ATTN_INJECT8
MAP8_DTYPES = (torch.uint8, torch.float8_e5m2)
CROSS_P_STRIDE = N.FZ_CROSS_P_STRIDE
CROSS_KEYS = N.FZ_CROSS_MAX_KEYS
TEMPORAL_MAX_FRAMES = N.FZ_TEMPORAL_MAX_FRAMES
SUPPORTED_HEAD_DIMS = (16, 32, 40, 64, 80, 128, 160)


def _raw_stream(dev_index: int) -> int:
    return torch._C._cuda_getCurrentRawStream(dev_index)


def refresh_stream():
    """Kept for callers of earlier revisions: the launch stream is read from PyTorch at EVERY launch now (per device), so there is
    nothing to refresh."""


# ... 224 lines not shown
    plan = _gn_plans.get(key)
    if plan is None:
        n, tokens, c = x.shape
        assert x.is_contiguous()
        _chk16(x, gamma, beta)
        chunks = N.lib().fz_groupnorm_chunks(tokens, c)
        need = n * chunks * groups * 3 + (n // span) * groups * 2
        skey = _scratch_key(x)
        buf = _gn_scratch.get(skey)
        if buf is None or buf.numel() < need:
            buf = torch.empty(max(need, 1 << 20), dtype=torch.float32, device=x.device)
            _gn_scratch[skey] = buf
            _gn_plans.clear()
            _scratch_gen[0] += 1
        plan = _gn_plans[key] = (n, tokens, c, buf.data_ptr(), buf)
    n, tokens, c, scratch, _ = plan
    if not x.is_contiguous() or x.dtype != torch.float16 or gamma.dtype != torch.float16 or beta.dtype != torch.float16 or \
            ((x.data_ptr() | gamma.data_ptr() | beta.data_ptr()) & 15):
        raise ValueError("fz_groupnorm: x must be contiguous fp16, gamma / beta fp16, all 16-byte aligned")
    if out is None:
        out = torch.empty_like(x)
    elif not out.is_contiguous() or out.dtype != torch.float16 or out.shape != x.shape or (out.data_ptr() & 15):
        raise ValueError("fz_groupnorm: out must be a contiguous fp16 tensor of x's shape")
    rc = N.lib().fz_groupnorm(x.data_ptr(), out.data_ptr(), gamma.data_ptr(), beta.data_ptr(), n, span, tokens, c, groups, eps,
                              1 if silu else 0, scratch, _stream(x))
    if rc:
        N.check(rc, "fz_groupnorm")
    return out


def groupnorm_cat(x1: torch.Tensor, x2: torch.Tensor, gamma: torch.Tensor, beta: torch.Tensor, *, span: int, groups: int, eps: float,
                  silu: bool) -> torch.Tensor:
    n, tokens, c1 = x1.shape
    c2 = x2.shape[2]
    if not (x1.is_contiguous() and x2.is_contiguous() and x2.shape[:2] == x1.shape[:2] and x1.dtype == x2.dtype == torch.float16
            and gamma.dtype == beta.dtype == torch.float16 and gamma.numel() == c1 + c2):
        raise ValueError("fz_groupnorm_cat: two contiguous fp16 tensors [N, tokens, C1] / [N, tokens, C2], gamma / beta over C1 + C2")
    _chk16(x1, x2, gamma, beta)
    c = c1 + c2
    chunks = N.lib().fz_groupnorm_chunks(tokens, c)
    need = n * chunks * groups * 3 + (n // span) * groups * 2
    skey = _scratch_key(x1)
    buf = _gn_scratch.get(skey)
    if buf is None or buf.numel() < need:
        buf = torch.empty(max(need, 1 << 20), dtype=torch.float32, device=x1.device)
        _gn_scratch[skey] = buf
        _gn_plans.clear()
        _scratch_gen[0] += 1
    out = torch.empty(n, tokens, c, dtype=torch.float16, device=x1.device)
    N.check(N.lib().fz_groupnorm_cat(x1.data_ptr(), c1, x2.data_ptr(), c2, out.data_ptr(), gamma.data_ptr(), beta.data_ptr(), n, span,
                                     tokens, groups, eps, 1 if silu else 0, buf.data_ptr(), _stream(x1)), "fz_groupnorm_cat")
    return out


def groupnorm_stats(x: torch.Tensor, *, groups: int) -> torch.Tensor:
    n, tokens, c = x.shape
    assert x.is_contiguous()
    _chk16(x)
    chunks = N.lib().fz_groupnorm_chunks(tokens, c)
    partial = torch.empty(n, groups, chunks, 3, dtype=torch.float32, device=x.device)
    N.check(N.lib().fz_groupnorm_stats(_ptr(x), n, tokens, c, groups, _ptr(partial), _stream(x)), "fz_groupnorm_stats")
    return partial


def groupnorm_apply(x: torch.Tensor, gamma: torch.Tensor, beta: torch.Tensor, partial_all: torch.Tensor, *, span: int,
                    groups: int, eps: float, silu: bool, out: Optional[torch.Tensor] = None):
    n, tokens, c = x.shape
    assert x.is_contiguous() and partial_all.is_contiguous() and partial_all.dtype == torch.float32
    sets, per_set = partial_all.shape[0], partial_all.shape[1]
    assert n // span == sets and partial_all.shape[3] == N.lib().fz_groupnorm_chunks(tokens, c)
    _chk16(x, gamma, beta)
    if out is None:
        out = torch.empty_like(x)
    stats = torch.empty(sets, groups, 2, dtype=torch.float32, device=x.device)
    N.check(N.lib().fz_groupnorm_apply(_ptr(x), _ptr(out), _ptr(gamma), _ptr(beta), n, span, tokens, c, groups, float(eps),
                                       1 if silu else 0, _ptr(partial_all), sets, per_set, _ptr(stats), _stream(x)),
            "fz_groupnorm_apply")
    return out


def groupnorm_from_partial(x: torch.Tensor, gamma: torch.Tensor, beta: torch.Tensor, partial: torch.Tensor, *, span: int, groups: int,
                           eps: float, silu: bool) -> torch.Tensor:
    n, tokens, c = x.shape
    if not (x.is_contiguous() and x.dtype == torch.float16 and partial.is_contiguous() and partial.dtype == torch.float32
            and partial.dim() == 4 and partial.shape[0] == n and partial.shape[1] == groups and partial.shape[3] == 3 and n % span == 0):
        raise ValueError("fz_groupnorm_from_partials: x [N, tokens, C] contiguous fp16, partial [N, groups, chunks, 3] fp32")
    _chk16(x, gamma, beta)
    out = torch.empty_like(x)
    stats = torch.empty(n // span, groups, 2, dtype=torch.float32, device=x.device)
    N.check(N.lib().fz_groupnorm_from_partials(x.data_ptr(), out.data_ptr(), gamma.data_ptr(), beta.data_ptr(), n, span, tokens, c, groups,
                                               float(eps), 1 if silu else 0, partial.data_ptr(), partial.shape[2], stats.data_ptr(),
                                               _stream(x)), "fz_groupnorm_from_partials")
    return out


def gemm_gn(x: torch.Tensor, w: torch.Tensor, bias: Optional[torch.Tensor], *, res: Optional[torch.Tensor] = None, gn_groups: int,
            rows_per_frame: int):
    k, o = x.shape[-1], w.shape[0]
    rows = x.numel() // k
    if not gn_epilogue_ok(rows_per_frame, o, gn_groups) or rows % rows_per_frame or not x.is_contiguous():
        return _gemm_unwrapped(x, w, bias, res=res), None
    _chk16(x, w, bias, res)
    y = torch.empty(tuple(x.shape[:-1]) + (o,), dtype=torch.float16, device=x.device)
    if res is not None and (not res.is_contiguous() or res.shape != y.shape):
        return _gemm_unwrapped(x, w, bias, res=res), None
    d = N.FzGemmDesc()
    d.rows, d.in_features, d.out_features = rows, k, o
    d.ldx, d.ldw, d.ldy, d.ldres = k, w.stride(0), o, o
    d.batch, d.epilogue = 1, N.FZ_GEMM_PLAIN
    partial = torch.empty(rows // rows_per_frame, gn_groups, rows_per_frame // 128, 3, dtype=torch.float32, device=x.device)
    rc = N.lib().fz_gemm_gn(C.byref(d), x.data_ptr(), w.data_ptr(), None if bias is None else bias.data_ptr(),
                            None if res is None else res.data_ptr(), None, y.data_ptr(), partial.data_ptr(), gn_groups, rows_per_frame,
                            _stream(x))
    if rc == N.FZ_GEMM_NO_STATS:
        return y, None
    if rc:
        N.check(rc, "fz_gemm_gn")
    return y, partial


def pack_conv3x3_weight(w: torch.Tensor) -> torch.Tensor:
    return w.detach().permute(0, 2, 3, 1).reshape(w.shape[0], 9, w.shape[1]).to(torch.float16).contiguous()


_ws = {}


def pack_geglu(w: torch.Tensor, b: Optional[torch.Tensor]):
    two, k = w.shape
    inner = two // 2
    assert inner % 32 == 0, inner
    wp = torch.stack([w[:inner].reshape(inner // 32, 32, k), w[inner:].reshape(inner // 32, 32, k)], 1).reshape(two, k)
    bp = None
    if b is not None:
        bp = torch.stack([b[:inner].reshape(inner // 32, 32), b[inner:].reshape(inner // 32, 32)], 1).reshape(two)
    return wp.contiguous(), (None if bp is None else bp.contiguous())


_WS_FLOATS = 64 << 20


_SCRATCH_STREAMS_MAX = 4
_scratch_lru = []


def _scratch_key(t_or_device):
    dev = t_or_device.device if isinstance(t_or_device, torch.Tensor) else torch.device(t_or_device)
    if dev.type != "cuda":
        return (dev, 0)
    key = (dev, _raw_stream(dev.index if dev.index is not None else torch.cuda.current_device()))
    if not _scratch_lru or _scratch_lru[-1] != key:
        if key in _scratch_lru:
            _scratch_lru.remove(key)
        _scratch_lru.append(key)
        while len(_scratch_lru) > _SCRATCH_STREAMS_MAX:
            old = _scratch_lru.pop(0)
            if _ws.pop(old, None) is not None:
                _scratch_gen[0] += 1
            if _gn_scratch.pop(old, None) is not None:
                _gn_plans.clear()
                _scratch_gen[0] += 1
    return key


def _ws_ptr(device):
    key = _scratch_key(device)
    buf = _ws.get(key)
    if buf is None:
        buf = _ws[key] = torch.empty(_WS_FLOATS, dtype=torch.float32, device=device)
        _scratch_gen[0] += 1
    return buf.data_ptr()


_gemm_plans = {}


def gemm(x: torch.Tensor, w: torch.Tensor, bias: Optional[torch.Tensor] = None, *, res: Optional[torch.Tensor] = None,
         res2: Optional[torch.Tensor] = None, out: Optional[torch.Tensor] = None, geglu: bool = False, tile_cfg: int = 0,
         split_k: int = 0):
    key = (x.shape, x.stride(), w.shape, w.stride(0), geglu, tile_cfg, split_k, x.device,
           None if res is None else res.stride(), res2 is not None, None if out is None else (out.shape, out.stride()))
    plan = _gemm_plans.get(key)
    if plan is None:
        plan = _gemm_plans[key] = _gemm_plan(x, w, bias, res, res2, out, geglu, tile_cfg, split_k)
    d_ref, out_shape, want_ws, _keep = plan
    if out is None:
        out = torch.empty(out_shape, dtype=torch.float16, device=x.device)
    ptrs = x.data_ptr() | w.data_ptr() | out.data_ptr()
    for t in (bias, res, res2):
        if t is not None:
            if t.dtype != torch.float16:
                raise ValueError("fz_gemm: bias / res / res2 must be fp16")
            ptrs |= t.data_ptr()
    if (ptrs & 15) or x.dtype != torch.float16 or w.dtype != torch.float16:
        raise ValueError("fz_gemm operands must be fp16 and 16-byte aligned")
    if res is not None and res2 is not None and res2.stride() != res.stride():
        raise ValueError("fz_gemm: res2 must have the layout of res")
    rc = N.lib().fz_gemm(d_ref, x.data_ptr(), w.data_ptr(), None if bias is None else bias.data_ptr(),
                         None if res is None else res.data_ptr(), None if res2 is None else res2.data_ptr(), out.data_ptr(),
                         _ws_ptr(x.device) if want_ws else None, _stream(x))
    if rc:
        N.check(rc, "fz_gemm")
    return out


def gemm_lnout(x: torch.Tensor, w: torch.Tensor, bias: Optional[torch.Tensor], ln, *, res: Optional[torch.Tensor] = None,
               res2: Optional[torch.Tensor] = None, tile_cfg: int = 0, split_k: int = 0):
    k, o = x.shape[-1], w.shape[0]
    rows = x.numel() // k
    gam, bet, eps = ln
    if (o != 320 or x.dtype != torch.float16 or not x.is_contiguous() or (res is not None and (not res.is_contiguous() or res.shape[-1] != o))
            or (res2 is not None and (not res2.is_contiguous() or res2.shape[-1] != o)) or gam.dtype != torch.float16):
        return _gemm_unwrapped(x, w, bias, res=res, res2=res2), None
    _chk16(x, w, bias, res, res2, gam, bet)
    y = torch.empty(tuple(x.shape[:-1]) + (o,), dtype=torch.float16, device=x.device)
    yln = torch.empty_like(y)
    d = N.FzGemmDesc()
    d.rows, d.in_features, d.out_features = rows, k, o
    d.ldx, d.ldw, d.ldy, d.ldres = k, w.stride(0), o, o
    d.batch, d.epilogue, d.tile_cfg, d.split_k = 1, N.FZ_GEMM_PLAIN, tile_cfg, split_k
    want_ws = o % 4 == 0 and (k >= 1024 or split_k > 1) and 2 * rows * o <= _WS_FLOATS
    if want_ws:
        d.workspace_floats = _WS_FLOATS
    rc = N.lib().fz_gemm_lnout(C.byref(d), x.data_ptr(), w.data_ptr(), _ptr(bias), _ptr(res), _ptr(res2), y.data_ptr(), gam.data_ptr(),
                               bet.data_ptr(), float(eps), yln.data_ptr(), o, _ws_ptr(x.device) if want_ws else None, _stream(x))
    if rc == N.FZ_GEMM_NO_STATS:
        return y, None
    if rc:
        N.check(rc, "fz_gemm_lnout")
    return y, yln


_gemm_unwrapped = gemm


def gemm_batched(x: torch.Tensor, w: torch.Tensor, out: Optional[torch.Tensor] = None):
    b, rows, k = x.shape
    o = w.shape[1]
    assert w.shape == (b, o, k) and x.stride(2) == 1 and w.stride(2) == 1 and x.dtype == w.dtype == torch.float16
    if out is None:
        out = torch.empty(b, rows, o, dtype=torch.float16, device=x.device)
    assert out.shape == (b, rows, o) and out.stride(2) == 1 and out.dtype == torch.float16
    for t in (x, w, out):
        if (t.data_ptr() & 15) or (t.stride(0) % 8) or (t.stride(1) % 8):
            raise ValueError("fz_gemm (batched): 16-byte aligned operands, row / batch strides multiples of 8 halves")
    d = N.FzGemmDesc()
    d.rows, d.in_features, d.out_features = rows, k, o
    d.ldx, d.ldw, d.ldy = x.stride(1), w.stride(1), out.stride(1)
    d.batch, d.epilogue = b, N.FZ_GEMM_PLAIN
    d.x_batch_stride, d.w_batch_stride, d.y_batch_stride = x.stride(0), w.stride(0), out.stride(0)
    want_ws = o % 4 == 0 and 2 * b * rows * o <= _WS_FLOATS
    d.workspace_floats = _WS_FLOATS if want_ws else 0
    rc = N.lib().fz_gemm(C.byref(d), x.data_ptr(), w.data_ptr(), None, None, None, out.data_ptr(),
                         _ws_ptr(x.device) if want_ws else None, _stream(x))
    if rc:
        N.check(rc, "fz_gemm (batched)")
    return out


def _gemm_plan(x, w, bias, res, res2, out, geglu, tile_cfg, split_k):
    k = x.shape[-1]
    o = w.shape[0]
    ow = o // 2 if geglu else o
    rows = x.numel() // k
    assert x.stride(-1) == 1 and w.stride(1) == 1 and w.shape[1] == k
    ldx = x.stride(-2) if x.dim() > 1 else k
    for d in range(x.dim() - 2):
        assert x.stride(d) == x.stride(d + 1) * x.shape[d + 1], "x must have a single row stride"
    _chk16(x, w, bias, res, res2)
    out_shape = tuple(x.shape[:-1]) + (ow,)
    ldy = ow
    if out is not None:
        assert out.stride(-1) == 1 and out.shape[-1] == ow and out.numel() // ow == rows and out.dtype == torch.float16
        ldy = out.stride(-2) if out.dim() > 1 else ow
    d = N.FzGemmDesc()
    d.rows, d.in_features, d.out_features = rows, k, o
    d.ldx, d.ldw, d.ldy = ldx, w.stride(0), ldy
    d.batch, d.epilogue = 1, (N.FZ_GEMM_GEGLU if geglu else N.FZ_GEMM_PLAIN)
    d.tile_cfg, d.split_k = tile_cfg, split_k
    for r in (res, res2):
        if r is not None:
            assert r.shape[-1] == ow and r.stride(-1) == 1 and r.numel() // ow == rows and r.dtype == torch.float16
    if res is not None:
        d.ldres = res.stride(-2) if res.dim() > 1 else ow
        if res2 is not None:
            assert (res2.stride(-2) if res2.dim() > 1 else ow) == d.ldres
    want_ws = (not geglu) and o % 4 == 0 and (k >= 1024 or split_k > 1) and 2 * rows * o <= _WS_FLOATS
    if want_ws:
        d.workspace_floats = _WS_FLOATS
    return (C.byref(d), out_shape, want_ws, d)


_vt_plans = {}


def gemm_vt(x: torch.Tensor, w: torch.Tensor, lp: int, out: Optional[torch.Tensor] = None, tile_cfg: int = 0):
    key = (x.shape, x.stride(), w.shape, w.stride(0), lp, tile_cfg, x.device, None if out is None else out.stride())
    plan = _vt_plans.get(key)
    n, l, k = x.shape
    c = w.shape[0]
    if out is None:
        out = torch.empty(n, c, lp, dtype=torch.float16, device=x.device)
    if plan is None:
        assert x.stride(2) == 1 and w.stride(1) == 1 and lp >= l and lp % 8 == 0
        _chk16(x, w, out)
        d = N.FzGemmDesc()
        d.rows, d.rows_store, d.in_features, d.out_features = l, lp, k, c
        d.ldx, d.ldw, d.ldy = x.stride(1), w.stride(0), out.stride(1)
        d.batch, d.x_batch_stride, d.y_batch_stride = n, x.stride(0), out.stride(0)
        d.transpose_out, d.tile_cfg = 1, tile_cfg
        plan = _vt_plans[key] = (C.byref(d), d)
    rc = N.lib().fz_gemm(plan[0], x.data_ptr(), w.data_ptr(), None, None, None, out.data_ptr(), None, _stream(x))
    if rc:
        N.check(rc, "fz_gemm(vt)")
    return out
# ... 69 lines not shown
    for t in vs:
        if t is not None and (t.dtype != torch.float16 or t.numel() != 320):
            raise ValueError("fz_xattn_chain_pack: fp16 [320] bias / LayerNorm parameters")
    if wo1 is not None and (vs[1] is None or vs[2] is None):
        raise ValueError("fz_xattn_chain_pack: the front form needs the LayerNorm's gamma and beta")
    _chk16(*ws, *vs)
    out = torch.empty(N.lib().fz_xattn_chain_pack_bytes(int(wo1 is not None)), dtype=torch.uint8, device=wq.device)
    rc = N.lib().fz_xattn_chain_pack(ws[0].data_ptr(), ws[1].data_ptr(), ws[2].data_ptr() if wo1 is not None else None, _ptr(vs[0]), _ptr(vs[1]),
                                     _ptr(vs[2]), out.data_ptr(), _stream(wq))
    if rc:
        N.check(rc, "fz_xattn_chain_pack")
    return out


def xattn_chain_kv_pack(k: torch.Tensor, vt: torch.Tensor, lk: int, out: Optional[torch.Tensor] = None) -> torch.Tensor:
    b = k.shape[0]
    if k.dtype != torch.float16 or vt.dtype != torch.float16 or vt.shape[0] != b or k.shape[2] < 320 or vt.shape[1] != 320 or \
            vt.shape[2] < CROSS_KEYS or k.stride(2) != 1 or vt.stride(2) != 1 or k.shape[1] < lk:
        raise ValueError(f"fz_xattn_chain_kv_pack: k [B, >= lk, 320] / vt [B, 320, >= 96] fp16, got {tuple(k.shape)} / {tuple(vt.shape)}")
    _chk16(k, vt)
    nbytes = N.lib().fz_xattn_chain_kv_pack_bytes(b)
    if out is None:
        out = torch.empty(nbytes, dtype=torch.uint8, device=k.device)
    elif out.numel() != nbytes or out.dtype != torch.uint8 or out.device != k.device:
        raise ValueError("fz_xattn_chain_kv_pack: `out` does not fit this context")
    rc = N.lib().fz_xattn_chain_kv_pack(k.data_ptr(), k.stride(0), k.stride(1), vt.data_ptr(), vt.stride(0), vt.stride(1), b, lk,
                                        out.data_ptr(), _stream(k))
    if rc:
        N.check(rc, "fz_xattn_chain_kv_pack")
    return out


def xattn_chain(x: torch.Tensor, packed: torch.Tensor, kv_packed: torch.Tensor, bias_out: Optional[torch.Tensor], *, res: Optional[torch.Tensor],
                frames_per_batch: int, heads: int, lk: int, scale: float, ln=None, front_eps: Optional[float] = None):
    n, l, c = x.shape
    rows = n * l
    front = front_eps is not None
    ts = [x] + ([] if res is None else [res])
    for t in ts:
        if t.dtype != torch.float16 or not t.is_contiguous() or t.shape != x.shape:
            raise ValueError("fz_xattn_chain: x / res must be contiguous fp16 tensors of one shape")
    if not xattn_chain_ok(rows, l, c, heads, lk):
        raise ValueError(f"fz_xattn_chain: unsupported shape {tuple(x.shape)} heads {heads} lk {lk}")
    if packed.numel() != N.lib().fz_xattn_chain_pack_bytes(int(front)) or packed.dtype != torch.uint8 or packed.data_ptr() % 16:
        raise ValueError("fz_xattn_chain: `packed` is not the stream of xattn_chain_pack for this form")
    nb = (n + frames_per_batch - 1) // frames_per_batch
    if kv_packed.numel() < N.lib().fz_xattn_chain_kv_pack_bytes(nb) or kv_packed.dtype != torch.uint8 or kv_packed.data_ptr() % 16:
        raise ValueError("fz_xattn_chain: `kv_packed` does not cover the batch")
    d = N.FzXattnChain()
    keep = [x, res, bias_out]
    y = torch.empty_like(x)
    yln = None
    d.x, d.res, d.packed, d.kv_packed, d.bias_out, d.y = x.data_ptr(), _ptr(res), packed.data_ptr(), kv_packed.data_ptr(), _ptr(bias_out), y.data_ptr()
    if ln is not None:
        gam, bet, eps = ln
        if gam.dtype != torch.float16 or bet.dtype != torch.float16:
            raise ValueError("fz_xattn_chain: LayerNorm weight / bias must be fp16")
        yln = torch.empty_like(x)
        d.y_ln, d.ln_gamma, d.ln_beta, d.ln_eps = yln.data_ptr(), gam.data_ptr(), bet.data_ptr(), float(eps)
        keep += [gam, bet]
    y1 = None
    if front:
        if res is None:
            raise ValueError("fz_xattn_chain: the front form needs the residual")
        y1 = torch.empty_like(x)
        d.front, d.y1, d.ln1_eps = 1, y1.data_ptr(), float(front_eps)
    _chk16(*[t for t in keep if t is not None])
    d.rows, d.rows_per_frame, d.frames_per_batch, d.channels, d.heads, d.lk, d.scale = rows, l, frames_per_batch, c, heads, lk, float(scale)
    rc = N.lib().fz_xattn_chain(C.byref(d), _stream(x))
    if rc:
        N.check(rc, "fz_xattn_chain")
    return (y, yln, y1) if front else (y, yln)


_qkvt_plans = {}


def gemm_qkvt_ok(x: torch.Tensor, w: torch.Tensor, split: int) -> bool:
    return x.dim() == 3 and x.shape[1] % 64 == 0 and split % 64 == 0 and 0 < split < w.shape[0] and x.shape[2] % 8 == 0


def gemm_qkvt(x: torch.Tensor, w: torch.Tensor, split: int, tile_cfg: int = 0):
    n, l, k = x.shape
    o = w.shape[0]
    cv = o - split
    key = (x.shape, x.stride(), w.shape, w.stride(0), split, tile_cfg, x.device)
    plan = _qkvt_plans.get(key)
    if plan is None:
        if not gemm_qkvt_ok(x, w, split) or x.stride(2) != 1 or w.stride(1) != 1 or w.shape[1] != k or x.stride(0) != l * x.stride(1):
            raise ValueError("fz_gemm_qkvt: x [N, L, K] with L % 64 == 0 and a single row stride, w [split + Cv, K], split % 64 == 0")
        d = N.FzGemmDesc()
        d.rows, d.in_features, d.out_features = n * l, k, o
        d.ldx, d.ldw, d.ldy = x.stride(1), w.stride(0), split
        d.batch, d.epilogue, d.tile_cfg = 1, N.FZ_GEMM_PLAIN, tile_cfg
        plan = _qkvt_plans[key] = (C.byref(d), d)
    if x.dtype != torch.float16 or w.dtype != torch.float16 or ((x.data_ptr() | w.data_ptr()) & 15):
        raise ValueError("fz_gemm_qkvt operands must be fp16 and 16-byte aligned")
    y = torch.empty(n, l, split, dtype=torch.float16, device=x.device)
# ... 179 lines not shown
    if out is None:
        out = torch.empty(x.shape, dtype=x.dtype, device=x.device)
    N.check(N.lib().fz_softmax_rows(_ptr(x), _ptr(out), rows, cols, ldx, cols, float(scale), _stream(x)), "fz_softmax_rows")
    return out


def transpose_pad(x: torch.Tensor, lp: int, out=None):
    n, l, c = x.shape
    assert x.stride(2) == 1 and x.dtype == torch.float16
    if out is None:
        out = torch.empty(n, c, lp, dtype=x.dtype, device=x.device)
    N.check(N.lib().fz_transpose_pad(_ptr(x), _ptr(out), n, l, c, x.stride(0), x.stride(1), lp, _stream(x)),
            "fz_transpose_pad")
    return out


def latent_update(z: torch.Tensor, eps_u: Optional[torch.Tensor], eps_c: torch.Tensor, guidance: float, cz: float,
                  ce: float, *, inv: Optional[torch.Tensor] = None, mask: Optional[torch.Tensor] = None,
                  next_in: Optional[torch.Tensor] = None):
    _, frames, hw = z.shape
    assert z.dtype == torch.float32 and z.is_contiguous() and eps_c.is_contiguous() and eps_c.dtype == torch.float16
    N.check(N.lib().fz_latent_update(_ptr(z), _ptr(eps_u), _ptr(eps_c), float(guidance), float(cz), float(ce), _ptr(inv),
                                     _ptr(mask), _ptr(next_in), frames, hw, _stream(z)), "fz_latent_update")
    return z


def accumulate(acc: torch.Tensor, x: torch.Tensor):
    assert acc.dtype == torch.float32 and x.dtype == torch.float16 and acc.numel() == x.numel()
    assert acc.is_contiguous() and x.is_contiguous()
    N.check(N.lib().fz_accumulate(_ptr(acc), _ptr(x), x.numel(), _stream(x)), "fz_accumulate")
    return acc


def version() -> str:
    return N.lib().fz_version().decode()
```

fatezero_amd/video_diffusion/models/attention.py:

```python
import copy
import os
from dataclasses import dataclass
from typing import Optional

import torch
from torch import nn

from ... import dist as D
from ... import issue as _issue
from ... import kernels as K
from .resnet import Tokens, _LinearParams, _NormParams, group_norm_tokens

_LOG2E = 1.4426950408889634


@dataclass
class SpatioTemporalTransformerModelOutput:
    sample: torch.Tensor


class AttnPlan:
    __slots__ = ("n_plain", "mode", "p", "row_mask", "mapper_t", "coef", "cur_out", "capture_first")

    def __init__(self, n_plain, mode=K.FZ_ATTN_FLASH, p=None, row_mask=None, mapper_t=None, coef=None, cur_out=None,
# ... 74 lines not shown
        if kvp is not None:
            K.xattn_chain_kv_pack(kk, vt, ctx.shape[1], out=kvp)
        self._ctx_kv = (ctx, ctx._version, kk, vt, kvp)

    def _context_kv(self, ctx, want_pack=False):
        kvc = self._ctx_kv
        if kvc is None or kvc[0] is not ctx or kvc[1] != ctx._version:
            kk = self.to_k.apply(ctx)
            vt = K.gemm_vt(ctx, self.to_v.packed(ctx.dtype, ctx.device)[0], K.CROSS_KEYS)
            kvc = self._ctx_kv = (ctx, ctx._version, kk, vt, None)
        if want_pack and kvc[4] is None:
            kvc = self._ctx_kv = kvc[:4] + (K.xattn_chain_kv_pack(kvc[2], kvc[3], ctx.shape[1]),)
        return kvc[2], kvc[3], kvc[4]

    def _chain_applies(self, n, lq, c, dtype, ctx):
        return (XATTN_CHAIN and lq > 32 ** 2 and dtype == torch.float16 and ctx.dtype == torch.float16 and self.inner_dim == c
                and self.to_q.bias is None and D.active_shard() is None and K.xattn_chain_preferred(n * lq, lq, c, self.heads, ctx.shape[1]))

    def _chain_weights(self, device, front=None):
        key = (str(device), None if front is None else (id(front[0]), id(front[1])))
        p = self._xchain.get(key)
        if p is None:
            wq = self.to_q.packed(torch.float16, device)[0]
            wo = self.to_out[0].packed(torch.float16, device)[0]
            fr = None
            if front is not None:
                w1, b1 = front[0].packed(torch.float16, device)
                fr = (w1, b1) + tuple(front[1].packed(device))
            p = self._xchain[key] = K.xattn_chain_pack(wq, wo, fr)
        return p

    def forward_cross_after(self, x: Tokens, o1, attn1_out, hs, norm_in, ctx, clip: int, ln_next):
        n, lq, c = o1.shape
        plan = _plan_for(self.controller, True, self.place_in_unet, n, clip, self.heads, lq, ctx.shape[1], o1.device)
        if plan is None or (plan.mode == K.FZ_ATTN_FLASH):
            _, _, kvp = self._context_kv(ctx, want_pack=True)
            packed = self._chain_weights(o1.device, (attn1_out, norm_in))
            g3, b3 = ln_next.packed(o1.device)
            bo = self.to_out[0].packed(o1.dtype, o1.device)[1]
            y, yln, _ = K.xattn_chain(o1, packed, kvp, bo, res=hs, frames_per_batch=clip, heads=self.heads, lk=ctx.shape[1], scale=self.scale,
                                      ln=(g3, b3, ln_next.eps), front_eps=norm_in.eps)
            return y, yln
        hs1, n_in = _out_proj(attn1_out, o1, hs, norm_in)
        if n_in is None:
            n_in = layer_norm_tokens(norm_in, hs1)
        return self.forward_cross(x.like(n_in), ctx, clip, residual=hs1, ln_next=ln_next, plan=plan)

    def _generic_controller_call(self, controller, is_cross, q, k, vt, out, clip, lq, lk_total, run_capture, run_inject):
        n = q.shape[0]
        width = K.CROSS_P_STRIDE if is_cross else lk_total
        p = torch.empty(n, self.heads, lq, width, dtype=torch.float16, device=q.device)
        run_capture(p)
        view = p[..., :lk_total] if is_cross else p
        new = controller(view, is_cross, self.place_in_unet)
        if new is not view:
            view.copy_(new)
        run_inject(p)

    def forward_cross(self, x: Tokens, ctx, clip: int, residual=None, ln_next=None, plan=False):
        n, lq, c = x.data.shape
        ctrl = self.controller
        if plan is False:
            if (ln_next is not None and residual is not None and residual.is_contiguous()
                    and self._chain_applies(n, lq, c, x.data.dtype, ctx)):
                plan = _plan_for(ctrl, True, self.place_in_unet, n, clip, self.heads, lq, ctx.shape[1], x.data.device)
                if plan is None or plan.mode == K.FZ_ATTN_FLASH:
                    _, _, kvp = self._context_kv(ctx, want_pack=True)
                    xn = x.data.contiguous()
                    g3, b3 = ln_next.packed(xn.device)
                    return K.xattn_chain(xn, self._chain_weights(xn.device), kvp, self.to_out[0].packed(xn.dtype, xn.device)[1],
                                         res=residual, frames_per_batch=clip, heads=self.heads, lk=ctx.shape[1], scale=self.scale,
                                         ln=(g3, b3, ln_next.eps))
        q = self.to_q.apply(x.data)
        kk, vt, _ = self._context_kv(ctx)
        lk = ctx.shape[1]
        out = torch.empty(n, lq, self.inner_dim, dtype=q.dtype, device=q.device)
        kw = dict(clip_len=clip, heads=self.heads, lk=lk, scale=self.scale)
        if plan is False:
            plan = _plan_for(ctrl, True, self.place_in_unet, n, clip, self.heads, lq, lk, q.device)
        if plan is None:
            if lq > 32 ** 2:
                K.attn_cross(q, kk, vt, out, mode=K.FZ_ATTN_FLASH, **kw)
            else:
                ident = torch.eye(K.CROSS_KEYS, dtype=torch.float16, device=q.device)
                coef = torch.zeros(2, K.CROSS_KEYS, dtype=torch.float32, device=q.device)
                coef[0] = 1.0
                self._generic_controller_call(
                    ctrl, True, q, kk, vt, out, clip, lq, lk,
                    lambda p: K.attn_cross(q, kk, vt, out, mode=K.FZ_ATTN_CAPTURE, p=p, **kw),
                    lambda p: K.attn_cross(q, kk, vt, out, mode=K.FZ_ATTN_INJECT, p=p, mapper_t=ident, coef=coef, **kw))
        elif plan.mode == K.FZ_ATTN_FLASH:
            K.attn_cross(q, kk, vt, out, mode=K.FZ_ATTN_FLASH, **kw)
        else:
            if plan.n_plain > 0:
                K.attn_cross(q, kk, vt, out, mode=K.FZ_ATTN_FLASH, frame0=0, n_frames=plan.n_plain, **kw)
            if plan.n_plain < n:
                K.attn_cross(q, kk, vt, out, mode=plan.mode, frame0=plan.n_plain, n_frames=n - plan.n_plain, p=plan.p,
                             mapper_t=plan.mapper_t, coef=plan.coef, cur_out=plan.cur_out, **kw)
        return _out_proj(self.to_out[0], out, residual, ln_next)

    def forward_temporal(self, x_norm, batch: int, clip: int, residual=None):
        n, l, c = x_norm.shape
        if self._qkv is None or self._qkv.device != x_norm.device:
            self._qkv = torch.cat([self._qk_weight(x_norm.dtype, x_norm.device),
                                   self.to_v.packed(x_norm.dtype, x_norm.device)[0]], 0).contiguous()
# ... 28 lines not shown
    def __init__(self, shard, batch, clip, index_list):
        self.shard, self.batch, self.clip = shard, batch, clip
        rel = [i for i in index_list if not isinstance(i, str)]
        self.left, self.right = max([0] + [-i for i in rel]), max([0] + [i for i in rel])
        self.anchors = [a for a in dict.fromkeys(K.kv_slots([i], shard.clip_len)[1][0] for i in index_list if isinstance(i, str))]
        kabs, kval = [], []
        for i in index_list:
            if isinstance(i, str):
                kabs.append(1)
                kval.append(self.left + clip + self.right + self.anchors.index(K.kv_slots([i], shard.clip_len)[1][0]))
            else:
                kabs.append(0)
                kval.append(int(i))
        self.ext = dict(kv_slots_override=(kabs, kval), kv_clip_len=self.left + clip + self.right + len(self.anchors),
                        kv_frame_off=self.left)

    def _wanted(self, r):
        fr = self.shard.frames_of(r)
        return list(range(fr.start - self.left, fr.start)) + list(range(fr.stop, fr.stop + self.right)) + self.anchors

    def post(self, t):
        t4 = t.reshape(self.batch, self.clip, *t.shape[1:])
        return t4, self.shard.fetch_frames_async(t4, self._wanted, tag="kv")

    def extend(self, handle):
        t4, pend = handle
        got = pend.wait()
        e = torch.cat([got[:, :self.left], t4, got[:, self.left:]], dim=1)
        return e.reshape(self.batch * e.shape[1], *t4.shape[2:])


class SparseCausalAttention(CrossAttention):

    def forward_self(self, x: Tokens, clip: int, index_list, residual=None, ln_next=None, raw_out=False):
        n, lq, c = x.data.shape
        xn = x.data
        d_head = self.inner_dim // self.heads
        folded = d_head % 16 != 0 and d_head % 8 == 0
        wqk = self._qk_weight(xn.dtype, xn.device, self.scale * _LOG2E if folded else 1.0)
        kw = dict(clip_len=clip, heads=self.heads, index_list=index_list, scale=self.scale, q_log2_scaled=folded)
        shard = D.active_shard()
        if shard is not None and len(index_list) > 0:
            skv = _ShardedKV(shard, n // clip, clip, index_list)
            kk = K.gemm(xn, wqk[self.inner_dim:])
            hk = skv.post(kk)
            vt = K.gemm_vt(xn, self.to_v.packed(xn.dtype, xn.device)[0], K.pad64(lq))
            hv = skv.post(vt)
            q = K.gemm(xn, wqk[: self.inner_dim])
            kk, vt = skv.extend(hk), skv.extend(hv)
            kw.update(skv.ext)
        else:
            wv = self.to_v.packed(xn.dtype, xn.device)[0]
            if QKV_FUSION and lq % 64 == 0 and (2 * self.inner_dim) % 64 == 0 and xn.is_contiguous():
                c = self._qkv_self
                if c is None or c[0] is not wqk or c[1] is not wv:
                    c = self._qkv_self = (wqk, wv, torch.cat([wqk, wv], 0).contiguous())
                qk, vt = K.gemm_qkvt(xn, c[2], 2 * self.inner_dim)
            else:
                qk = K.gemm(xn, wqk)
                vt = K.gemm_vt(xn, wv, K.pad64(lq))
            q, kk = qk[..., : self.inner_dim], qk[..., self.inner_dim:]
        out = torch.empty(n, lq, self.inner_dim, dtype=xn.dtype, device=xn.device)
        n_kv = max(1, len(index_list))
        ctrl = self.controller
        plan = _plan_for(ctrl, False, self.place_in_unet, n, clip, self.heads, lq, n_kv * lq, xn.device)
        if plan is None:
            if lq > 32 ** 2:
                K.attn_self(q, kk, vt, out, mode=K.FZ_ATTN_FLASH, **kw)
            else:
                self._generic_controller_call(
                    ctrl, False, q, kk, vt, out, clip, lq, n_kv * lq,
                    lambda p: K.attn_self(q, kk, vt, out, mode=K.FZ_ATTN_CAPTURE, p=p, **kw),
                    lambda p: K.attn_self(q, None, vt, out, mode=K.FZ_ATTN_INJECT, p=p, **kw))
        elif plan.mode == K.FZ_ATTN_FLASH and plan.capture_first is None:
            K.attn_self(q, kk, vt, out, mode=K.FZ_ATTN_FLASH, **kw)
        else:
            if plan.n_plain > 0:
                K.attn_self(q, kk, vt, out, mode=K.FZ_ATTN_FLASH, frame0=0, n_frames=plan.n_plain, **kw)
            if plan.n_plain < n:
                rest = dict(frame0=plan.n_plain, n_frames=n - plan.n_plain)
                if plan.capture_first is not None:
                    K.attn_self(q, kk, vt, out, mode=K.self_mode_for(K.FZ_ATTN_CAPTURE, plan.capture_first), p=plan.capture_first,
                                **rest, **kw)
                if plan.mode in (K.FZ_ATTN_INJECT, K.FZ_ATTN_INJECT8):
                    K.attn_self(q, kk if plan.row_mask is not None else None, vt, out, mode=plan.mode, p=plan.p,
                                row_mask=plan.row_mask, **rest, **kw)
                elif not (plan.mode == K.FZ_ATTN_FLASH and plan.capture_first is not None):
                    K.attn_self(q, kk, vt, out, mode=plan.mode, p=plan.p, **rest, **kw)
        if raw_out:
            return out
        return _out_proj(self.to_out[0], out, residual, ln_next)


class _GEGLU(nn.Module):
    def __init__(self, dim, inner):
        super().__init__()
        self.proj = _LinearParams(dim, inner * 2)
        self._packed = None
# ... 44 lines not shown
        else:
            h = K.geglu(g.proj.apply(x))
        return _out_proj(self.net[2], h, res, ln_next)


class SpatioTemporalTransformerBlock(nn.Module):

    def __init__(self, dim, num_attention_heads, attention_head_dim, cross_attention_dim=None, model_config: dict = {},
                 **unused):
        super().__init__()
        self.model_config = copy.deepcopy(model_config)
        if "least_sc_channel" in model_config and dim < model_config["least_sc_channel"]:
            self.model_config["SparseCausalAttention_index"] = []
        self.attn1 = SparseCausalAttention(query_dim=dim, heads=num_attention_heads, dim_head=attention_head_dim)
        self.norm1 = _NormParams(dim)
        self.attn2 = CrossAttention(query_dim=dim, cross_attention_dim=cross_attention_dim, heads=num_attention_heads,
                                    dim_head=attention_head_dim)
        self.norm2 = _NormParams(dim)
        self.attn_temporal = CrossAttention(query_dim=dim, heads=num_attention_heads, dim_head=attention_head_dim)
        nn.init.zeros_(self.attn_temporal.to_out[0].weight.data)
        self.norm_temporal = _NormParams(dim)
        self.ff = FeedForward(dim)
        self.norm3 = _NormParams(dim)

    @property
    def sc_index(self):
        return self.model_config.get("SparseCausalAttention_index", [-1, "first"])

    def forward_tokens(self, x: Tokens, ctx, prenorm1=None):
        hs = x.data
        clip = x.f
        lnp = LN_FROM_PRODUCER and hs.shape[-1] == LN_FROM_PRODUCER_C and hs.dtype == torch.float16 and D.active_shard() is None
        n1 = prenorm1 if prenorm1 is not None else layer_norm_tokens(self.norm1, hs)
        if (lnp and XATTN_CHAIN_FRONT and hs.is_contiguous()
                and self.attn2._chain_applies(hs.shape[0], hs.shape[1], hs.shape[2], hs.dtype, ctx)):
            o1 = self.attn1.forward_self(x.like(n1), clip, self.sc_index, raw_out=True)
            hs, n3 = self.attn2.forward_cross_after(x, o1, self.attn1.to_out[0], hs, self.norm2, ctx, clip, self.norm3)
        else:
            hs, n2 = self.attn1.forward_self(x.like(n1), clip, self.sc_index, residual=hs, ln_next=self.norm2 if lnp else None)
            if n2 is None:
                n2 = layer_norm_tokens(self.norm2, hs)
            hs, n3 = self.attn2.forward_cross(x.like(n2), ctx, clip, residual=hs, ln_next=self.norm3 if lnp else None)
        if n3 is None:
            n3 = layer_norm_tokens(self.norm3, hs)
        hs, nt = self.ff.apply(n3, res=hs, ln_next=self.norm_temporal if lnp else None)
        if nt is None:
            nt = layer_norm_tokens(self.norm_temporal, hs)
        hs = self.attn_temporal.forward_temporal(nt, x.b, clip, residual=hs)
        return x.like(hs)


class SpatioTemporalTransformerModel(nn.Module):

    def __init__(self, num_attention_heads=16, attention_head_dim=88, in_channels=None, num_layers=1,
                 norm_num_groups=32, cross_attention_dim=None, model_config: dict = {}, use_linear_projection=False, **unused):
        super().__init__()
        assert num_layers == 1
        inner = num_attention_heads * attention_head_dim
        self.use_linear_projection = use_linear_projection
        self.norm = _NormParams(in_channels, norm_num_groups, 1e-6)
        self.proj_in = _Conv1x1Params(in_channels, inner, linear=use_linear_projection)
        self.transformer_blocks = nn.ModuleList([SpatioTemporalTransformerBlock(
            inner, num_attention_heads, attention_head_dim, cross_attention_dim=cross_attention_dim,
            model_config=model_config)])
        self.proj_out = _Conv1x1Params(inner, in_channels, linear=use_linear_projection)

    def forward_tokens(self, x: Tokens, ctx) -> Tokens:
        h = group_norm_tokens(self.norm, x, span_frames=False, silu=False)
        blk = self.transformer_blocks[0]
        pre1 = None
        if (LN_FROM_PRODUCER and self.proj_in.weight.shape[0] == LN_FROM_PRODUCER_C and h.data.dtype == torch.float16 and h.data.is_contiguous()
                and D.active_shard() is None):
            y, pre1 = self.proj_in.apply_lnout(h.data, blk.norm1)
            h = h.like(y)
        else:
            h = h.like(self.proj_in.apply(h.data))
        h = blk.forward_tokens(h, ctx, prenorm1=pre1)
        from .resnet import GN_FROM_EPILOGUE
        if GN_FROM_EPILOGUE and D.active_shard() is None:
            y, part = self.proj_out.apply_gn(h.data, res=x.data, groups=self.norm.num_groups, rows_per_frame=x.data.shape[1])
            out = x.like(y)
            out.gn = None if part is None else (part, self.norm.num_groups)
            return out
        return x.like(self.proj_out.apply(h.data, res=x.data))


class _Conv1x1Params(nn.Module):

    def __init__(self, cin, cout, linear=False):
        super().__init__()
        self.weight = nn.Parameter(torch.empty((cout, cin) if linear else (cout, cin, 1, 1)))
        nn.init.kaiming_uniform_(self.weight, a=5 ** 0.5)
        self.bias = nn.Parameter(torch.zeros(cout))
        self._packed = None

    def _pack(self, x):
        if self._packed is None or self._packed[0].dtype != x.dtype or self._packed[0].device != x.device:
            self._packed = (self.weight.detach().reshape(self.weight.shape[0], -1).to(device=x.device, dtype=x.dtype).contiguous(),
                            self.bias.detach().to(device=x.device, dtype=x.dtype))
        return self._packed

    def apply(self, x, res=None):
        w, b = self._pack(x)
        return K.gemm(x, w, b, res=res)

    def apply_lnout(self, x, norm):
        w, b = self._pack(x)
        g, be = norm.packed(x.device)
        return K.gemm_lnout(x, w, b, (g, be, norm.eps))

    def apply_gn(self, x, res, groups, rows_per_frame):
        w, b = self._pack(x)
        return K.gemm_gn(x, w, b, res=res, gn_groups=groups, rows_per_frame=rows_per_frame)
```

fatezero_amd/video_diffusion/models/resnet.py:

```python
import copy
import os

import torch
from torch import nn

from ... import dist as D
from ... import kernels as K
from .lora import LoRALinearLayer, _Conv1dParams, pack_temporal_weight, temporal_conv_tokens


GN_FROM_EPILOGUE = os.environ.get("FZ_NO_GN_EPILOGUE") is None
CONV_UP2 = os.environ.get("FZ_NO_CONV_UP2") is None


class Tokens:
    __slots__ = ("data", "b", "f", "h", "w", "gn")

    def __init__(self, data, b, f, h, w, gn=None):
        self.data, self.b, self.f, self.h, self.w, self.gn = data, b, f, h, w, gn

    @property
    def c(self):
        return self.data.shape[-1]

    def like(self, data, h=None, w=None):
        return Tokens(data, self.b, self.f, self.h if h is None else h, self.w if w is None else w)

    @staticmethod
    def cat(a, b):
        return CatTokens(a, b)

    @staticmethod
    def from_bcfhw(x):
        b, c, f, h, w = x.shape
        return Tokens(x.permute(0, 2, 3, 4, 1).reshape(b * f, h * w, c).contiguous(), b, f, h, w)

    def to_bcfhw(self):
        return self.data.view(self.b, self.f, self.h, self.w, self.c).permute(0, 4, 1, 2, 3)


class CatTokens(Tokens):
    __slots__ = ("parts", "_cat")

    def __init__(self, a: Tokens, b: Tokens):
        self.parts, self._cat = (a.data, b.data), None
        self.b, self.f, self.h, self.w, self.gn = a.b, a.f, a.h, a.w, None

    @property
    def data(self):
        if self._cat is None:
            self._cat = torch.cat(self.parts, dim=-1)
        return self._cat

    @property
    def c(self):
        return self.parts[0].shape[-1] + self.parts[1].shape[-1]


class PseudoConv3d(nn.Module):

    def __init__(self, in_channels, out_channels, kernel_size, temporal_kernel_size=None, model_config: dict = {},
                 temporal_downsample=False, stride=1, padding=0):
        super().__init__()
        self.in_channels, self.out_channels, self.kernel_size = in_channels, out_channels, kernel_size
        self.stride = stride
        self.padding = padding[0] if isinstance(padding, (tuple, list)) else padding
        self.weight = nn.Parameter(torch.empty(out_channels, in_channels, kernel_size, kernel_size))
        self.bias = nn.Parameter(torch.zeros(out_channels))
        nn.init.kaiming_uniform_(self.weight, a=5 ** 0.5)
        if temporal_kernel_size is None:
            temporal_kernel_size = kernel_size
        assert not temporal_downsample, "temporal_downsample is not used by any shipped config"
        if kernel_size > 1:
            if "lora" in model_config:
                self.conv_temporal = LoRALinearLayer(out_channels, out_channels, rank=model_config["lora"])
            else:
                self.conv_temporal = _Conv1dParams(out_channels, out_channels, temporal_kernel_size, bias=True)
                nn.init.dirac_(self.conv_temporal.weight.data)
        else:
            self.conv_temporal = None
        self._packed = None
        self._packed_up = None

    def _pack(self, dtype, device):
        if self._packed is None or self._packed[0].dtype != dtype or self._packed[0].device != device:
            if dtype != torch.float16:
                raise RuntimeError("the MI355X engine computes in fp16 storage / fp32 accumulation: call unet.half()")
            w = self.weight.detach().to(device=device, dtype=dtype)
            if self.kernel_size == 1:
                w = w.reshape(self.out_channels, self.in_channels).contiguous()
            else:
                assert self.kernel_size == 3 and self.padding == 1, "the pseudo-3D UNet only uses 3x3 pad-1 and 1x1 convolutions"
                w = K.pack_conv3x3_weight(w)
            bias = self.bias.detach().to(device=device, dtype=dtype)
            wtt = btt = None
            if self.conv_temporal is not None and not isinstance(self.conv_temporal, LoRALinearLayer):
                tw, tb = self.conv_temporal.weight.detach(), self.conv_temporal.bias.detach()
                ident = torch.zeros_like(tw)
                nn.init.dirac_(ident)
                if not (bool((tw == ident).all()) and bool((tb == 0).all())):
                    wtt = pack_temporal_weight(tw, dtype, device)
                    btt = tb.to(device=device, dtype=dtype)
            self._packed = (w, bias, wtt, btt)
        return self._packed

    def forward_tokens(self, x: Tokens, residual=None, temb=None, upsample=False, gn_groups: int = 0) -> Tokens:
        probe = x.parts[0] if isinstance(x, CatTokens) and x._cat is None else x.data
        w, bias, wtt, btt = self._pack(probe.dtype, probe.device)
        n, hw = probe.shape[0], probe.shape[1]
        lora = self.conv_temporal if isinstance(self.conv_temporal, LoRALinearLayer) else None
        plain_t = self.conv_temporal is not None and lora is None and wtt is not None
        temporal_active = plain_t or (lora is not None and not lora.is_noop(probe.dtype, probe.device))
        fuse_tail = not temporal_active
        if self.kernel_size == 1 and isinstance(x, CatTokens) and x._cat is None and residual is None and temb is None \
                and x.parts[0].shape[-1] % 8 == 0:
            c1 = x.parts[0].shape[-1]
            y = K.gemm(x.parts[1], w[:, c1:], None, res=K.gemm(x.parts[0], w[:, :c1], bias))
            oh, ow = x.h, x.w
            fused = fuse_tail
        elif self.kernel_size == 1:
            y = K.gemm(x.data, w, bias, res=residual if (fuse_tail and temb is None) else None)
            oh, ow = x.h, x.w
            fused = fuse_tail and temb is None
        else:
            xin = x.data if x.data.is_contiguous() else x.data.contiguous()
            up2 = upsample and CONV_UP2 and self.stride == 1 and self.in_channels % 64 == 0 and self.out_channels % 160 == 0
            if up2 and (self._packed_up is None or self._packed_up[0] is not w):
                self._packed_up = (w, K.pack_conv3x3_up2_weight(w))
            if up2 and K.conv3x3_up2_preferred(n, x.h, x.w, self.in_channels, self.out_channels):
                y, (oh, ow) = K.conv3x3_up2(xin, self._packed_up[1], bias, hw=(x.h, x.w))
                fused = fuse_tail and temb is None and residual is None
            else:
                y, (oh, ow) = K.conv3x3(xin, w, bias, hw=(x.h, x.w), stride=self.stride, upsample=upsample,
                                        temb=temb if fuse_tail else None, frames_per_batch=x.f,
                                        res=residual if fuse_tail else None)
                fused = fuse_tail
        gn = None
        if lora is not None and temporal_active:
            y4 = lora.forward_tokens(y.view(x.b, x.f, oh * ow, self.out_channels), temb=temb, residual=residual, gn_groups=gn_groups)
            if isinstance(y4, tuple):
                y4, part = y4
                gn = None if part is None else (part, gn_groups)
            y = y4.reshape(n, oh * ow, self.out_channels)
            fused = True
        elif plain_t:
            rows = btt[None, :].expand(x.b, -1) if temb is None else temb + btt
            shard = D.active_shard()
            y4 = y.view(x.b, x.f, oh * ow, self.out_channels)
            if shard is not None:
                y4 = temporal_conv_tokens(shard.with_halo(y4, 1, 1, zero_outside=True, tag="temporal_conv"), wtt, rows_add=rows.contiguous())[:, 1:-1]
                y = y4.reshape(n, oh * ow, self.out_channels)
                if residual is not None:
                    y = y + residual
            else:
                y = temporal_conv_tokens(y4, wtt, rows_add=rows.contiguous(), residual=residual).reshape(n, oh * ow, self.out_channels)
            fused = True
        if not fused:
            if temb is not None:
                y = (y.view(x.b, x.f * oh * ow, self.out_channels) + temb[:, None, :]).view(n, oh * ow, self.out_channels)
            if residual is not None:
                y = y + residual
        out = x.like(y, oh, ow)
        out.gn = gn
        return out


class _NormParams(nn.Module):

    def __init__(self, channels, groups=None, eps=1e-5):
        super().__init__()
        self.weight = nn.Parameter(torch.ones(channels))
        self.bias = nn.Parameter(torch.zeros(channels))
        self.num_groups, self.eps = groups, eps
        self._packed = None

    def packed(self, device):
        if self._packed is None or self._packed[0].device != device:
            self._packed = (self.weight.detach().to(device=device, dtype=torch.float16).contiguous(),
                            self.bias.detach().to(device=device, dtype=torch.float16).contiguous())
        return self._packed


def group_norm_tokens(norm: _NormParams, x: Tokens, *, span_frames: bool, silu: bool) -> Tokens:
    lazy = isinstance(x, CatTokens) and x._cat is None
    g, b = norm.packed((x.parts[0] if lazy else x.data).device)
    shard = D.active_shard()
    if shard is not None and span_frames:
        n, _, _ = x.data.shape
        part = K.groupnorm_stats(x.data, groups=norm.num_groups)
        allp = shard.all_gather_frames(part.view(n // x.f, x.f, *part.shape[1:]), tag="groupnorm").contiguous()
        y = K.groupnorm_apply(x.data, g, b, allp, span=x.f, groups=norm.num_groups, eps=norm.eps, silu=silu)
        return x.like(y)
    if not lazy and x.gn is not None and x.gn[1] == norm.num_groups and x.gn[0].shape[0] == x.data.shape[0]:
        y = K.groupnorm_from_partial(x.data, g, b, x.gn[0], span=(x.f if span_frames else 1), groups=norm.num_groups, eps=norm.eps, silu=silu)
        return Tokens(y, x.b, x.f, x.h, x.w)
    if isinstance(x, CatTokens) and x._cat is None and x.parts[0].shape[-1] % 8 == 0 and x.parts[1].shape[-1] % 8 == 0:
        y = K.groupnorm_cat(x.parts[0], x.parts[1], g, b, span=(x.f if span_frames else 1), groups=norm.num_groups, eps=norm.eps,
                            silu=silu)
        return Tokens(y, x.b, x.f, x.h, x.w)
    y = K.groupnorm(x.data, g, b, span=(x.f if span_frames else 1), groups=norm.num_groups, eps=norm.eps, silu=silu)
    return Tokens(y, x.b, x.f, x.h, x.w)


def upsample_nearest2x(x: Tokens) -> Tokens:
    n, hw, c = x.data.shape
    y = x.data.view(n, x.h, 1, x.w, 1, c).expand(n, x.h, 2, x.w, 2, c).reshape(n, 4 * hw, c)
    return x.like(y, 2 * x.h, 2 * x.w)


class UpsamplePseudo3D(nn.Module):

    def __init__(self, channels, use_conv=False, use_conv_transpose=False, out_channels=None, name="conv",
                 model_config: dict = {}, **kwargs):
        super().__init__()
        assert use_conv and not use_conv_transpose
        self.channels, self.out_channels = channels, out_channels or channels
        self.conv = PseudoConv3d(self.channels, self.out_channels, 3, padding=1, model_config=model_config)

    def forward_tokens(self, x: Tokens) -> Tokens:
        return self.conv.forward_tokens(x, upsample=True)


class DownsamplePseudo3D(nn.Module):

    def __init__(self, channels, use_conv=False, out_channels=None, padding=1, model_config: dict = {}, name="conv"):
        super().__init__()
        assert use_conv and padding == 1
        self.channels, self.out_channels = channels, out_channels or channels
        self.conv = PseudoConv3d(self.channels, self.out_channels, 3, stride=2, padding=padding, model_config=model_config)

    def forward_tokens(self, x: Tokens) -> Tokens:
        return self.conv.forward_tokens(x)


# ... 52 lines not shown
```

fatezero_amd/video_diffusion/models/unet_3d_blocks.py:

```python
import torch
from torch import nn

from .attention import SpatioTemporalTransformerModel
from .resnet import DownsamplePseudo3D, ResnetBlockPseudo3D, Tokens, UpsamplePseudo3D


def _resnet(cin, cout, temb, eps, groups, scale, mc):
    return ResnetBlockPseudo3D(in_channels=cin, out_channels=cout, temb_channels=temb, eps=eps, groups=groups,
                               output_scale_factor=scale, model_config=mc)


def _transformer(heads, channels, cross_dim, groups, mc, linear=False):
    return SpatioTemporalTransformerModel(heads, channels // heads, in_channels=channels, num_layers=1,
                                          cross_attention_dim=cross_dim, norm_num_groups=groups, model_config=mc,
                                          use_linear_projection=linear)


class CrossAttnDownBlockPseudo3D(nn.Module):
    has_cross_attention = True

    def __init__(self, in_channels, out_channels, temb_channels, num_layers=1, resnet_eps=1e-6, resnet_groups=32,
                 attn_num_head_channels=1, cross_attention_dim=1280, output_scale_factor=1.0, add_downsample=True,
                 model_config: dict = {}, use_linear_projection=False, **unused):
        super().__init__()
# ... 4 lines not shown
                                                      resnet_groups, model_config, use_linear_projection) for _ in range(num_layers)])
        self.downsamplers = None
        if add_downsample:
            self.downsamplers = nn.ModuleList([DownsamplePseudo3D(out_channels, use_conv=True, out_channels=out_channels,
                                                                  padding=1, name="op", model_config=model_config)])

    def forward_tokens(self, x: Tokens, temb_act, ctx):
        outs = []
        for resnet, attn in zip(self.resnets, self.attentions):
            x = attn.forward_tokens(resnet.forward_tokens(x, temb_act), ctx)
            outs.append(x)
        if self.downsamplers is not None:
            x = self.downsamplers[0].forward_tokens(x)
            outs.append(x)
        return x, outs


class DownBlockPseudo3D(nn.Module):
    has_cross_attention = False

    def __init__(self, in_channels, out_channels, temb_channels, num_layers=1, resnet_eps=1e-6, resnet_groups=32,
                 output_scale_factor=1.0, add_downsample=True, model_config: dict = {}, **unused):
        super().__init__()
        self.resnets = nn.ModuleList([_resnet(in_channels if i == 0 else out_channels, out_channels, temb_channels,
                                              resnet_eps, resnet_groups, output_scale_factor, model_config)
                                      for i in range(num_layers)])
        self.downsamplers = None
        if add_downsample:
            self.downsamplers = nn.ModuleList([DownsamplePseudo3D(out_channels, use_conv=True, out_channels=out_channels,
                                                                  padding=1, name="op", model_config=model_config)])

    def forward_tokens(self, x: Tokens, temb_act, ctx=None):
        outs = []
        for resnet in self.resnets:
            x = resnet.forward_tokens(x, temb_act)
            outs.append(x)
        if self.downsamplers is not None:
            x = self.downsamplers[0].forward_tokens(x)
            outs.append(x)
        return x, outs


class UNetMidBlockPseudo3DCrossAttn(nn.Module):
    has_cross_attention = True

    def __init__(self, in_channels, temb_channels, resnet_eps=1e-6, resnet_groups=32, attn_num_head_channels=1,
                 output_scale_factor=1.0, cross_attention_dim=1280, model_config: dict = {},
                 use_linear_projection=False, **unused):
        super().__init__()
        self.resnets = nn.ModuleList([_resnet(in_channels, in_channels, temb_channels, resnet_eps, resnet_groups,
                                              output_scale_factor, model_config) for _ in range(2)])
        self.attentions = nn.ModuleList([_transformer(attn_num_head_channels, in_channels, cross_attention_dim,
                                                      resnet_groups, model_config, use_linear_projection)])

    def forward_tokens(self, x: Tokens, temb_act, ctx):
        x = self.resnets[0].forward_tokens(x, temb_act)
        x = self.attentions[0].forward_tokens(x, ctx)
        return self.resnets[1].forward_tokens(x, temb_act)


def _cat_skip(x: Tokens, skip: Tokens) -> Tokens:
    return Tokens.cat(x, skip)


class CrossAttnUpBlockPseudo3D(nn.Module):
    has_cross_attention = True

    def __init__(self, in_channels, out_channels, prev_output_channel, temb_channels, num_layers=1, resnet_eps=1e-6,
                 resnet_groups=32, attn_num_head_channels=1, cross_attention_dim=1280, output_scale_factor=1.0,
                 add_upsample=True, model_config: dict = {}, use_linear_projection=False, **unused):
        super().__init__()
        res = []
        for i in range(num_layers):
            skip_c = in_channels if (i == num_layers - 1) else out_channels
            rin = prev_output_channel if i == 0 else out_channels
            res.append(_resnet(rin + skip_c, out_channels, temb_channels, resnet_eps, resnet_groups, output_scale_factor,
                               model_config))
        self.resnets = nn.ModuleList(res)
        self.attentions = nn.ModuleList([_transformer(attn_num_head_channels, out_channels, cross_attention_dim,
                                                      resnet_groups, model_config, use_linear_projection) for _ in range(num_layers)])
        self.upsamplers = None
        if add_upsample:
            self.upsamplers = nn.ModuleList([UpsamplePseudo3D(out_channels, use_conv=True, out_channels=out_channels,
                                                              model_config=model_config)])

    def forward_tokens(self, x: Tokens, skips, temb_act, ctx):
        for resnet, attn in zip(self.resnets, self.attentions):
            x = resnet.forward_tokens(_cat_skip(x, skips.pop()), temb_act)
            x = attn.forward_tokens(x, ctx)
        if self.upsamplers is not None:
            x = self.upsamplers[0].forward_tokens(x)
        return x


class UpBlockPseudo3D(nn.Module):
    has_cross_attention = False

    def __init__(self, in_channels, prev_output_channel, out_channels, temb_channels, num_layers=1, resnet_eps=1e-6,
                 resnet_groups=32, output_scale_factor=1.0, add_upsample=True, model_config: dict = {}, **unused):
        super().__init__()
        res = []
        for i in range(num_layers):
            skip_c = in_channels if (i == num_layers - 1) else out_channels
            rin = prev_output_channel if i == 0 else out_channels
            res.append(_resnet(rin + skip_c, out_channels, temb_channels, resnet_eps, resnet_groups, output_scale_factor,
                               model_config))
        self.resnets = nn.ModuleList(res)
        self.upsamplers = None
        if add_upsample:
            self.upsamplers = nn.ModuleList([UpsamplePseudo3D(out_channels, use_conv=True, out_channels=out_channels,
                                                              model_config=model_config)])

    def forward_tokens(self, x: Tokens, skips, temb_act, ctx=None):
        for resnet in self.resnets:
            x = resnet.forward_tokens(_cat_skip(x, skips.pop()), temb_act)
        if self.upsamplers is not None:
            x = self.upsamplers[0].forward_tokens(x)
        return x


_DOWN = {"CrossAttnDownBlockPseudo3D": CrossAttnDownBlockPseudo3D, "DownBlockPseudo3D": DownBlockPseudo3D}
_UP = {"CrossAttnUpBlockPseudo3D": CrossAttnUpBlockPseudo3D, "UpBlockPseudo3D": UpBlockPseudo3D}


def get_down_block(down_block_type, **kw):
    down_block_type = down_block_type[7:] if down_block_type.startswith("UNetRes") else down_block_type
    if down_block_type not in _DOWN:
        raise ValueError(f"{down_block_type} does not exist.")
    if down_block_type == "CrossAttnDownBlockPseudo3D" and kw.get("cross_attention_dim") is None:
        raise ValueError("cross_attention_dim must be specified for CrossAttnDownBlockPseudo3D")
    return _DOWN[down_block_type](**kw)


def get_up_block(up_block_type, **kw):
    up_block_type = up_block_type[7:] if up_block_type.startswith("UNetRes") else up_block_type
    if up_block_type not in _UP:
        raise ValueError(f"{up_block_type} does not exist.")
    if up_block_type == "CrossAttnUpBlockPseudo3D" and kw.get("cross_attention_dim") is None:
        raise ValueError("cross_attention_dim must be specified for CrossAttnUpBlockPseudo3D")
    return _UP[up_block_type](**kw)
```

fatezero_amd/video_diffusion/models/unet_3d_condition.py:

```python
import glob
import json
import math
import os
from dataclasses import dataclass
from types import SimpleNamespace
from typing import Optional, Tuple, Union

import torch
import torch.nn.functional as F
from torch import nn

from .resnet import PseudoConv3d, Tokens, _LinearParams, _NormParams, group_norm_tokens
from .unet_3d_blocks import UNetMidBlockPseudo3DCrossAttn, get_down_block, get_up_block


@dataclass
class UNetPseudo3DConditionOutput:
    sample: torch.Tensor

    def __getitem__(self, k):
        return getattr(self, k) if isinstance(k, str) else (self.sample,)[k]


class _TimestepEmbedding(nn.Module):
# ... 3 lines not shown
        self.linear_2 = _LinearParams(cout, cout)


_NEWER_KEY_DEFAULTS = {
    "time_embedding_type": "positional", "conv_in_kernel": 3, "conv_out_kernel": 3, "transformer_layers_per_block": 1,
    "reverse_transformer_layers_per_block": None, "encoder_hid_dim": None, "encoder_hid_dim_type": None,
    "addition_embed_type": None, "addition_time_embed_dim": None, "addition_embed_type_num_heads": 64,
    "time_embedding_dim": None, "time_embedding_act_fn": None, "timestep_post_act": None, "time_cond_proj_dim": None,
    "projection_class_embeddings_input_dim": None, "class_embeddings_concat": False, "mid_block_only_cross_attention": None,
    "cross_attention_norm": None, "resnet_skip_time_act": False, "resnet_out_scale_factor": 1.0, "attention_type": "default",
    "dropout": 0.0,
}


def _check_newer_keys(kwargs, attention_head_dim):
    rest = dict(kwargs)
    for key, default in _NEWER_KEY_DEFAULTS.items():
        if key not in rest:
            continue
        v = rest.pop(key)
        ok = v == default or (key == "transformer_layers_per_block" and isinstance(v, (list, tuple)) and all(x == 1 for x in v))
        if not ok:
            raise NotImplementedError(f"UNet config {key}={v!r} is not supported (only {default!r}, the reference's architecture)")
    if "num_attention_heads" in rest:
        v = rest.pop("num_attention_heads")
        if v is not None and v != attention_head_dim and list(v if isinstance(v, (list, tuple)) else [v]) != list(
                attention_head_dim if isinstance(attention_head_dim, (list, tuple)) else [attention_head_dim]):
            raise NotImplementedError(f"UNet config num_attention_heads={v!r} differs from attention_head_dim={attention_head_dim!r}: "
                                      "the reference takes the head count from attention_head_dim")
    return rest


TIME_EMBED_CACHE = True


class UNetPseudo3DConditionModel(nn.Module):
    def __init__(self, sample_size: Optional[int] = None, in_channels: int = 4, out_channels: int = 4,
                 center_input_sample: bool = False, flip_sin_to_cos: bool = True, freq_shift: int = 0,
                 down_block_types: Tuple[str] = ("CrossAttnDownBlockPseudo3D", "CrossAttnDownBlockPseudo3D",
                                                 "CrossAttnDownBlockPseudo3D", "DownBlockPseudo3D"),
                 mid_block_type: str = "UNetMidBlockPseudo3DCrossAttn",
                 up_block_types: Tuple[str] = ("UpBlockPseudo3D", "CrossAttnUpBlockPseudo3D", "CrossAttnUpBlockPseudo3D",
                                               "CrossAttnUpBlockPseudo3D"),
                 only_cross_attention=False, block_out_channels: Tuple[int] = (320, 640, 1280, 1280),
                 layers_per_block: int = 2, downsample_padding: int = 1, mid_block_scale_factor: float = 1,
                 act_fn: str = "silu", norm_num_groups: int = 32, norm_eps: float = 1e-5, cross_attention_dim: int = 1280,
                 attention_head_dim: Union[int, Tuple[int]] = 8, dual_cross_attention: bool = False,
                 use_linear_projection: bool = False, class_embed_type=None, num_class_embeds=None,
                 upcast_attention: bool = False, resnet_time_scale_shift: str = "default", **kwargs):
        super().__init__()
        if (center_input_sample or not flip_sin_to_cos or freq_shift != 0 or dual_cross_attention
                or class_embed_type is not None or num_class_embeds is not None or resnet_time_scale_shift != "default"
                or act_fn not in ("silu", "swish") or kwargs.get("temporal_downsample") or kwargs.get("temporal_downsample_time", 0)):
            raise NotImplementedError("only the SD-1.x / SD-2.x configuration surface used by FateZero is implemented")
        kwargs = _check_newer_keys(kwargs, attention_head_dim)
        cfg = dict(sample_size=sample_size, in_channels=in_channels, out_channels=out_channels,
                   down_block_types=tuple(down_block_types), up_block_types=tuple(up_block_types),
                   block_out_channels=tuple(block_out_channels), layers_per_block=layers_per_block,
                   norm_num_groups=norm_num_groups, norm_eps=norm_eps, cross_attention_dim=cross_attention_dim,
                   attention_head_dim=attention_head_dim, center_input_sample=False,
                   use_linear_projection=bool(use_linear_projection), upcast_attention=bool(upcast_attention), **kwargs)
        self.config = SimpleNamespace(**cfg)
        self.sample_size = sample_size
        model_config = dict(kwargs)
        time_embed_dim = block_out_channels[0] * 4
        self.conv_in = PseudoConv3d(in_channels, block_out_channels[0], kernel_size=3, padding=1, model_config=model_config)
# ... 87 lines not shown
            t = torch.as_tensor(timestep, dtype=torch.float32, device=device).reshape(-1).expand(batch)
            e = t[:, None] * freq[None]
        e = torch.cat([torch.cos(e), torch.sin(e)], dim=-1).to(torch.float16)
        e = self.time_embedding.linear_2.apply(F.silu(self.time_embedding.linear_1.apply(e)))
        e = F.silu(e)
        if key is not None:
            if len(self._temb_cache) >= 4096:
                self._temb_cache.clear()
            self._temb_cache[key] = e
        return e

    def _project_time_embeddings(self, temb_act):
        from ... import kernels as K
        pk = getattr(self, "_temb_pack", None)
        if pk is None or pk[0].device != temb_act.device:
            from .resnet import ResnetBlockPseudo3D
            blocks = [m for m in self.modules() if isinstance(m, ResnetBlockPseudo3D)]
            w = torch.cat([b.time_emb_proj.weight.detach() for b in blocks], 0).to(device=temb_act.device, dtype=torch.float16)
            bias = torch.cat([b.time_emb_proj.bias.detach() for b in blocks], 0).to(device=temb_act.device, dtype=torch.float16)
            offs, o = [], 0
            for b in blocks:
                offs.append((o, b.out_channels))
                o += b.out_channels
            pk = (w.contiguous(), bias, blocks, offs)
            self._temb_pack = pk
        w, bias, blocks, offs = pk
        t_all = K.gemm(temb_act, w, bias)
        for b, (o, c) in zip(blocks, offs):
            b._temb_cached = t_all[:, o:o + c]

    def forward_tokens(self, x: Tokens, timestep, ctx) -> Tokens:
        from ... import kernels as K
        K.refresh_stream()
        temb_act = self.time_embed(timestep, x.b, x.data.device)
        ctx = ctx.to(torch.float16)
        issuer = self._issuer
        if issuer is None and os.environ.get("FZ_ISSUE_PLANS") == "1":
            issuer = self.enable_issue_plans()
        if issuer is not None:
            y = issuer.run(x, temb_act, ctx)
            if y is not None:
                return y
        return self._forward_body(x, temb_act, ctx)

    def enable_issue_plans(self, on=True, graph=None):
        if on and self._issuer is None:
            from ...issue import IssuePlans
            self._issuer = IssuePlans(self, graph=graph)
        elif not on:
            self._issuer = None
        return self._issuer

    def _forward_body(self, x: Tokens, temb_act, ctx) -> Tokens:
        self._project_time_embeddings(temb_act)
        from .resnet import GN_FROM_EPILOGUE
        x = self.conv_in.forward_tokens(x, gn_groups=self.conv_norm_out.num_groups if GN_FROM_EPILOGUE else 0)
        skips = [x]
        for blk in self.down_blocks:
            x, outs = blk.forward_tokens(x, temb_act, ctx)
            skips.extend(outs)
        x = self.mid_block.forward_tokens(x, temb_act, ctx)
        for blk in self.up_blocks:
            x = blk.forward_tokens(x, skips, temb_act, ctx)
        x = group_norm_tokens(self.conv_norm_out, x, span_frames=True, silu=True)
        return self.conv_out.forward_tokens(x)

# ... 52 lines not shown
```

fatezero_amd/video_diffusion/pipelines/p2p_ddim_spatial_temporal.py:

```python
import os
from typing import Callable, List, Optional, Union

import numpy as np
import torch

from ... import dist as fz_dist
from ... import kernels as K
from ..models.resnet import Tokens
from ..prompt_attention import attention_util, spatial_blend
from .stable_diffusion import SpatioTemporalStableDiffusionPipeline, StableDiffusionPipelineOutput


class _LatentState:

    def __init__(self, latents: torch.Tensor, reps: int):
        b, c, f, h, w = latents.shape
        if b != 1:
            raise ValueError("Only support single video editing")
        self.f, self.h, self.w, self.reps = f, h, w, reps
        self.z = latents[0].to(torch.float32, copy=True).reshape(c, f, h * w).contiguous()
        self.tok = torch.empty(reps * f, h * w, c, dtype=torch.float16, device=latents.device)
        self.sync_tokens()

    def sync_tokens(self):
        t = self.z.permute(1, 2, 0).to(torch.float16)
        for r in range(self.reps):
            self.tok[r * self.f:(r + 1) * self.f].copy_(t)

    def tokens(self) -> Tokens:
        return Tokens(self.tok, self.reps, self.f, self.h, self.w)

    def as_latents(self, dtype) -> torch.Tensor:
        return self.z.view(1, self.z.shape[0], self.f, self.h, self.w).to(dtype)

    def assign(self, latents: torch.Tensor):
        self.z.copy_(latents[0].float().reshape(self.z.shape))
        self.sync_tokens()

    def update(self, eps_u, eps_c, guidance, cz, ce):
        K.latent_update(self.z, eps_u, eps_c, guidance, cz, ce, next_in=self.tok[: self.f])
        for r in range(1, self.reps):
            self.tok[r * self.f:(r + 1) * self.f].copy_(self.tok[: self.f])


class P2pDDIMSpatioTemporalPipeline(SpatioTemporalStableDiffusionPipeline):
    def __init__(self, vae, text_encoder, tokenizer, unet, scheduler, disk_store: bool = False, map_dtype: str = "fp16"):
        super().__init__(vae, text_encoder, tokenizer, unet, scheduler)
        self.map_dtype = self.default_map_dtype = map_dtype
        self.store_controller = attention_util.AttentionStore(disk_store=disk_store, map_dtype=map_dtype)
        self.empty_controller = attention_util.EmptyControl()
        self.frame_shard = None

    def _gather_frames(self, latents_local: List[torch.Tensor]) -> List[torch.Tensor]:
        shard = self.frame_shard
        x = torch.stack(latents_local)
        s_, b_, c_, fl, h_, w_ = x.shape
        full = shard.all_gather_frames(x.permute(0, 1, 3, 2, 4, 5).reshape(s_ * b_, fl, c_, h_, w_))
        full = full.reshape(s_, b_, shard.clip_len, c_, h_, w_).permute(0, 1, 3, 2, 4, 5)
        return [full[i].contiguous() for i in range(s_)]

    def set_map_dtype(self, map_dtype: str):
        if map_dtype != self.map_dtype:
            store = self.store_controller.with_map_dtype(map_dtype)
            self.release_attention_maps()
            self.store_controller, self.map_dtype = store, map_dtype

    def release_attention_maps(self):
        self.last_edit_controller = None
        if self.store_controller is not None:
            self.store_controller.release_arena()

    def check_inputs(self, prompt, height, width, callback_steps, strength=None):
        if not isinstance(prompt, str) and not isinstance(prompt, list):
            raise ValueError(f"`prompt` has to be of type `str` or `list` but is {type(prompt)}")
# ... 124 lines not shown
            attention_output = self._attention_strips(kwargs["prompt"], self.store_controller)
            dict_output = {"sdimage_output": sdimage_output, "attention_output": attention_output, "mask_list": None}
            attention_util.register_attention_control(self, self.empty_controller)
            return dict_output
        return self.p2preplace_edit(**kwargs)

    @torch.no_grad()
    def sd_ddim_pipeline(self, prompt: Union[str, List[str]], image=None, height: Optional[int] = None,
                         width: Optional[int] = None, strength: float = None, num_inference_steps: int = 50,
                         guidance_scale: float = 7.5, negative_prompt=None, num_images_per_prompt: Optional[int] = 1,
                         eta: float = 0.0, generator=None, latents: Optional[torch.Tensor] = None,
                         output_type: Optional[str] = "pil", return_dict: bool = True,
                         callback: Optional[Callable[[int, int, torch.Tensor], None]] = None,
                         callback_steps: Optional[int] = 1, controller=None, **args):
        sample_size = getattr(self.unet.config, "sample_size", None) or 64
        height = height or sample_size * self.vae_scale_factor
        width = width or sample_size * self.vae_scale_factor
        self.check_inputs(prompt, height, width, callback_steps, strength)
        if eta != 0.0:
            raise NotImplementedError("the editing path always runs eta = 0")
        batch_size = 1 if isinstance(prompt, str) else len(prompt)
        device = self._execution_device
        do_cfg = guidance_scale > 1.0
        text_embeddings = self._encode_prompt(prompt, device, num_images_per_prompt, do_cfg, negative_prompt)
        self.scheduler.set_timesteps(num_inference_steps, device=device)
        timesteps = self.scheduler.timesteps
        if latents is None:
            latents = self.prepare_latents_ddim_inverted(image, batch_size, num_images_per_prompt, text_embeddings,
                                                         store_attention=False, generator=generator)[-1]
        latents_dtype = latents.dtype
        shard = self.frame_shard
        if shard is not None:
            latents = shard.local(latents, 2).contiguous()
        state = _LatentState(latents.detach(), reps=2 if do_cfg else 1)
        emb = text_embeddings.to(torch.float16)
        n_t = len(timesteps)
        with fz_dist.frame_sharded(shard):
            for i, t in enumerate(self.progress_bar(timesteps)):
                t = int(t)
                eps = self.unet.forward_tokens(state.tokens(), t, emb).data
                cz, ce = self.scheduler.step_coefficients(t)
                if do_cfg:
                    state.update(eps[: state.f], eps[state.f:], guidance_scale, cz, ce)
                else:
                    state.update(None, eps, 0.0, cz, ce)
                if controller is not None:
                    cur = state.as_latents(latents_dtype)
                    new = controller.step_callback(cur)
                    if new is not cur:
                        state.assign(new)
                if callback is not None and i % callback_steps == 0:
                    callback(i, t, state.as_latents(latents_dtype).clone())
        latents = state.as_latents(latents_dtype).clone()
        if shard is not None:
            latents = self._gather_frames([latents])[0]
        if output_type == "latent":
            image = latents
        else:
            image = self.decode_latents(latents)
            if output_type == "pil":
                image = self.numpy_to_pil(image)
        if not return_dict:
            return (image, None)
        return StableDiffusionPipelineOutput(images=image, nsfw_content_detected=None)
```

include/fatezero_hip.h:

```cpp
#ifndef FATEZERO_HIP_H
#define FATEZERO_HIP_H
#include <stdint.h>

#ifdef __cplusplus
extern "C" {
#endif

#define FZ_ATTN_FLASH 0
#define FZ_ATTN_CAPTURE 1
#define FZ_ATTN_INJECT 2
#define FZ_ATTN_CAPTURE8 3
#define FZ_ATTN_INJECT8 4

#define FZ_MAX_KV_SLOTS 4

typedef struct FzAttnSelfDesc {
    int32_t n_frames;
    int32_t frame0;
    int32_t clip_len;
    int32_t heads;
    int32_t head_dim;
    int32_t lq;
    int32_t lkf;
    int32_t n_kv;
// ... 26 lines not shown
    float scale;
    int32_t mode;
    int64_t q_frame_stride, q_row_stride;
    int64_t k_batch_stride, k_row_stride;
    int64_t vt_batch_stride, vt_chan_stride;
    int64_t o_frame_stride, o_row_stride;
    int64_t p_frame_stride, p_head_stride, p_row_stride;
    int32_t p_frame_off;
    int32_t store_cur;
} FzAttnCrossDesc;

int fz_attn_cross(const FzAttnCrossDesc* desc, const void* q, const void* k, const void* vt, void* o,
                  void* p, const void* mapper_t, const float* coef, void* cur_out, void* stream);

#define FZ_TEMPORAL_MAX_FRAMES 256

int fz_attn_temporal(const void* q, const void* k, const void* v, void* o, int batch, int clip_len,
                     int tokens, int heads, int head_dim, int64_t qkv_row_stride, int64_t o_row_stride,
                     float scale, void* stream);

int fz_attn_temporal_ex(const void* q, const void* k, const void* v, void* o, int batch, int q_frames, int kv_frames,
                        int tokens, int heads, int head_dim, int64_t q_row_stride, int64_t kv_row_stride,
                        int64_t o_row_stride, float scale, void* stream);

int fz_blend_mask(const void* const* maps, int n_maps, int n_prompts, int64_t prompt_stride, int frames,
                  int heads, int res, int64_t p_row_stride, const float* alpha, float th, int out_h, int out_w,
                  int or_with_first, float* out, float* scratch, void* stream);

int fz_groupnorm_chunks(int tokens, int channels);
int fz_groupnorm(const void* x, void* y, const void* gamma, const void* beta, int n_frames, int span,
                 int tokens, int channels, int groups, float eps, int silu, float* partial, void* stream);

int fz_groupnorm_cat(const void* x1, int channels1, const void* x2, int channels2, void* y, const void* gamma, const void* beta,
                     int n_frames, int span, int tokens, int groups, float eps, int silu, float* partial, void* stream);

int fz_groupnorm_stats(const void* x, int n_frames, int tokens, int channels, int groups, float* partial, void* stream);
int fz_groupnorm_apply(const void* x, void* y, const void* gamma, const void* beta, int n_frames, int span, int tokens,
                       int channels, int groups, float eps, int silu, const float* partial_all, int stat_sets,
                       int frames_per_set, float* stats, void* stream);

#define FZ_GEMM_PLAIN 0
#define FZ_GEMM_GEGLU 1
typedef struct FzGemmDesc {
    int64_t rows;
    int64_t rows_store;
    int32_t in_features;
    int32_t out_features;
    int64_t ldx, ldw, ldy, ldres;
    int32_t batch;
    int32_t epilogue;
    int64_t x_batch_stride, y_batch_stride, res_batch_stride;
    int32_t transpose_out;
    int32_t tile_cfg;
    int32_t split_k;
    int32_t reserved0;
    int64_t workspace_floats;
    int64_t w_batch_stride;
} FzGemmDesc;
int64_t fz_gemm_workspace_floats(int64_t rows, int out_features, int batch);
int fz_gemm(const FzGemmDesc* desc, const void* x, const void* w, const void* bias, const void* res, const void* res2,
            void* y, void* workspace, void* stream);

int fz_gemm_qkvt(const FzGemmDesc* desc, const void* x, const void* w, void* y, void* yt, int split_col, int64_t rows_per_frame,
                 int64_t yt_frame_stride, int64_t ldyt, void* stream);

int fz_ff_chain_ok(int64_t rows, int channels, int inner);
int fz_ff_chain_preferred(int64_t rows, int channels, int inner);
int64_t fz_ff_chain_pack_bytes(int channels, int inner);
int fz_ff_chain_pack(const void* w1, const void* b1, const void* w2, void* packed, int channels, int inner, void* stream);
int fz_ff_chain(const void* xn, const void* packed, const void* b2, const void* res, void* y, const void* ln_gamma, const void* ln_beta,
                float ln_eps, void* y_ln, int64_t rows, int channels, int inner, void* stream);

typedef struct FzXattnChain {
    const void* x;
    const void* res;
    const void* packed;
    const void* kv_packed;
    const void* bias_out;
    void* y;
    void* y_ln;
    const void* ln_gamma;
    const void* ln_beta;
    void* y1;
    int64_t rows, rows_per_frame;
    int32_t frames_per_batch, channels, heads, lk;
    float scale;
    float ln_eps, ln1_eps;
    int32_t front;
} FzXattnChain;
int fz_xattn_chain_ok(int64_t rows, int64_t rows_per_frame, int channels, int heads, int lk);
int fz_xattn_chain_preferred(int64_t rows, int64_t rows_per_frame, int channels, int heads, int lk);
int64_t fz_xattn_chain_pack_bytes(int with_front);
int64_t fz_xattn_chain_kv_pack_bytes(int batch);
int fz_xattn_chain_pack(const void* wq, const void* wo, const void* wo1, const void* bias_out1, const void* ln1_gamma, const void* ln1_beta,
                        void* packed, void* stream);
int fz_xattn_chain_kv_pack(const void* k, int64_t k_batch_stride, int64_t k_row_stride, const void* vt, int64_t vt_batch_stride,
                           int64_t vt_chan_stride, int batch, int lk, void* packed, void* stream);
int fz_xattn_chain(const FzXattnChain* desc, void* stream);

#define FZ_GEMM_NO_STATS 1

int fz_conv3x3(const void* x, const void* wt, const void* bias, const void* temb, int64_t temb_stride, const void* res,
               void* y, int n, int hi, int wi, int cin, int cout, int stride, int upsample, int frames_per_batch,
               void* workspace, int64_t workspace_floats, int tile_cfg, int split_k, void* stream);

int fz_conv3x3_up2_ok(int n, int h, int w, int cin, int cout);
int fz_conv3x3_up2_preferred(int n, int h, int w, int cin, int cout);
int64_t fz_conv3x3_up2_pack_halves(int cin, int cout);
int fz_conv3x3_up2_pack(const void* wt, void* wt_up, int cin, int cout, void* stream);
int fz_conv3x3_up2(const void* x, const void* wt_up, const void* bias, void* y, int n, int h, int w, int cin, int cout, void* stream);

int fz_temporal_conv3(const void* x, const void* wt, const void* res, const void* res2, const void* temb,
                      int64_t temb_stride, void* y, int n, int tokens, int cin, int cout, int clip_len, void* workspace,
                      int64_t workspace_floats, void* stream);

int fz_lora_pair_ok(int n, int tokens, int channels, int rank, int clip_len);
int fz_lora_pair_preferred(int n, int tokens, int channels, int rank, int clip_len);
int fz_lora_pair(const void* x, const void* w_down, const void* w_up, const void* temb, int64_t temb_stride, const void* res2, void* y,
                 int n, int tokens, int channels, int rank, int clip_len, void* stream);
int fz_lora_pair_gn_chunks(int n, int tokens, int channels, int rank, int clip_len, int gn_groups);
int fz_lora_pair_gn(const void* x, const void* w_down, const void* w_up, const void* temb, int64_t temb_stride, const void* res2, void* y,
                    int n, int tokens, int channels, int rank, int clip_len, float* gn_partial, int gn_groups, void* stream);

int fz_gn_epilogue_chunks(int64_t rows_per_frame);
int fz_gemm_gn(const FzGemmDesc* desc, const void* x, const void* w, const void* bias, const void* res, const void* res2, void* y,
               float* gn_partial, int gn_groups, int64_t rows_per_frame, void* stream);
int fz_temporal_conv3_gn(const void* x, const void* wt, const void* res, const void* res2, const void* temb, int64_t temb_stride, void* y,
                         int n, int tokens, int cin, int cout, int clip_len, void* workspace, int64_t workspace_floats,
                         float* gn_partial, int gn_groups, void* stream);
int fz_groupnorm_from_partials(const void* x, void* y, const void* gamma, const void* beta, int n_frames, int span, int tokens,
                               int channels, int groups, float eps, int silu, const float* partial, int partial_chunks, float* stats,
                               void* stream);

int fz_gemm_lnout(const FzGemmDesc* desc, const void* x, const void* w, const void* bias, const void* res, const void* res2, void* y,
                  const void* gamma, const void* beta, float eps, void* y_ln, int64_t ld_ln, void* workspace, void* stream);

int fz_layernorm(const void* x, void* y, const void* gamma, const void* beta, int64_t rows, int channels,
                 float eps, void* stream);

int fz_geglu(const void* x, void* y, int64_t rows, int inner, void* stream);

int fz_softmax_rows(const void* x, void* y, int64_t rows, int cols, int64_t ldx, int64_t ldy, float scale, void* stream);

int fz_transpose_pad(const void* in, void* out, int n, int l, int c, int64_t in_frame_stride, int64_t in_row_stride,
                     int lp, void* stream);

int fz_latent_update(float* z, const void* eps_u, const void* eps_c, float guidance, float cz, float ce,
                     const float* inv, const float* mask, void* next_in, int frames, int hw, void* stream);

int fz_accumulate(float* acc, const void* x, int64_t n, void* stream);

int fz_peer_put(const void* src, int64_t bytes, void* const* dst, uint32_t* const* flags, int n_dst, uint32_t epoch,
                uint32_t* done_counter, void* stream);
int fz_peer_wait(const uint32_t* flags, uint64_t sender_mask, uint32_t epoch, uint32_t* err, int64_t timeout_us, void* stream);

typedef struct FzPlan FzPlan;
int fz_plan_begin(FzPlan** out);
int fz_plan_pause(FzPlan* plan, int paused);
int fz_plan_end(FzPlan* plan);
int64_t fz_plan_launches(const FzPlan* plan);
int64_t fz_plan_relocate(FzPlan* plan, int64_t first, int64_t count, const void* old_base, int64_t nbytes, const void* new_base);
int fz_plan_replay(const FzPlan* plan, int64_t first, int64_t count, void* stream);
int fz_plan_graph_launch(FzPlan* plan, void* stream);
void fz_plan_destroy(FzPlan* plan);

const char* fz_version(void);

#ifdef __cplusplus
}
#endif
#endif
```

Before: 4.119 frames/s.

## Share the unconditional/conditional CFG input head across batch halves

In CFG mode both batch halves get identical latent tokens, so the input is now stored once with a repeat factor. It is expanded lazily only where the conditioning differs, with frame-modulo indexing in the GEMM residual, groupnorm-cat skip input and cross-attention chain. This removes the duplicate token copies and the redundant early layers (conv_in, first block) that would otherwise run twice on identical data. It adds index-modulo arithmetic in several kernels and a new repeat kernel, and it is disabled when frame sharding is active.

```diff
diff --git a/fatezero_amd/_native.py b/fatezero_amd/_native.py
--- a/fatezero_amd/_native.py
+++ b/fatezero_amd/_native.py
@@ -50,7 +50,7 @@
         ("batch", C.c_int32), ("epilogue", C.c_int32),
         ("x_batch_stride", C.c_int64), ("y_batch_stride", C.c_int64), ("res_batch_stride", C.c_int64),
         ("transpose_out", C.c_int32), ("tile_cfg", C.c_int32), ("split_k", C.c_int32), ("reserved0", C.c_int32),
-        ("workspace_floats", C.c_int64), ("w_batch_stride", C.c_int64),
+        ("workspace_floats", C.c_int64), ("w_batch_stride", C.c_int64), ("res_rows", C.c_int64),
     ]
 
 
@@ -62,6 +62,7 @@
         ("rows", C.c_int64), ("rows_per_frame", C.c_int64),
         ("frames_per_batch", C.c_int32), ("channels", C.c_int32), ("heads", C.c_int32), ("lk", C.c_int32),
         ("scale", C.c_float), ("ln_eps", C.c_float), ("ln1_eps", C.c_float), ("front", C.c_int32),
+        ("in_frames", C.c_int32), ("reserved0", C.c_int32),
     ]
 
 
@@ -104,7 +105,7 @@
     "fz_groupnorm": (C.c_int, [_P, _P, _P, _P, C.c_int, C.c_int, C.c_int, C.c_int, C.c_int, C.c_float, C.c_int,
                                _P, _P]),
     "fz_groupnorm_cat": (C.c_int, [_P, C.c_int, _P, C.c_int, _P, _P, _P, C.c_int, C.c_int, C.c_int, C.c_int, C.c_float, C.c_int,
-                                   _P, _P]),
+                                   _P, C.c_int, _P]),
     "fz_groupnorm_stats": (C.c_int, [_P, C.c_int, C.c_int, C.c_int, C.c_int, _P, _P]),
     "fz_groupnorm_apply": (C.c_int, [_P, _P, _P, _P, C.c_int, C.c_int, C.c_int, C.c_int, C.c_int, C.c_float, C.c_int, _P,
                                      C.c_int, C.c_int, _P, _P]),
@@ -128,6 +129,7 @@
     "fz_transpose_pad": (C.c_int, [_P, _P, C.c_int, C.c_int, C.c_int, C.c_int64, C.c_int64, C.c_int, _P]),
     "fz_latent_update": (C.c_int, [_P, _P, _P, C.c_float, C.c_float, C.c_float, _P, _P, _P, C.c_int, C.c_int, _P]),
     "fz_accumulate": (C.c_int, [_P, _P, C.c_int64, _P]),
+    "fz_repeat": (C.c_int, [_P, _P, C.c_int64, C.c_int, _P]),
     "fz_peer_put": (C.c_int, [_P, C.c_int64, _P, _P, C.c_int, C.c_uint32, _P, _P]),
     "fz_peer_wait": (C.c_int, [_P, C.c_uint64, C.c_uint32, _P, C.c_int64, _P]),
     "fz_plan_begin": (C.c_int, [C.POINTER(_P)]),
diff --git a/fatezero_amd/csrc/elementwise.hip b/fatezero_amd/csrc/elementwise.hip
--- a/fatezero_amd/csrc/elementwise.hip
+++ b/fatezero_amd/csrc/elementwise.hip
@@ -195,6 +195,22 @@
     return fz_last_launch_status();
 }
 
+FZ_KERNEL void __launch_bounds__(256) repeat_kernel(const half_t* __restrict__ x, half_t* __restrict__ y, int64_t n8, int reps) {
+    for (int64_t i = (int64_t)blockIdx.x * blockDim.x + threadIdx.x; i < n8; i += (int64_t)gridDim.x * blockDim.x) {
+        const half8_t v = fz_ld_h8(x + i * 8);
+        for (int r = 0; r < reps; ++r) fz_st_h8(y + ((int64_t)r * n8 + i) * 8, v);
+    }
+}
+
+extern "C" int fz_repeat(const void* x, void* y, int64_t n, int reps, void* stream) {
+    if (!x || !y || n <= 0 || (n & 7) || reps <= 0) return FZ_ERR_BAD_ARG;
+    const int64_t n8 = n >> 3;
+    int blocks = (int)((n8 + 255) / 256);
+    if (blocks > 4096) blocks = 4096;
+    FZ_LAUNCH(repeat_kernel, dim3(blocks), dim3(256), 0, stream, (const half_t*)x, (half_t*)y, n8, reps);
+    return fz_last_launch_status();
+}
+
 extern "C" const char* fz_version(void) {
 #ifdef FZ_EMU
     return "fatezero_amd 0.1 (CPU emulation build -- tests only)";
diff --git a/fatezero_amd/csrc/igemm.hip b/fatezero_amd/csrc/igemm.hip
--- a/fatezero_amd/csrc/igemm.hip
+++ b/fatezero_amd/csrc/igemm.hip
@@ -60,6 +60,7 @@
     const half_t* res;
     const half_t* res2;
     int64_t lda, ldb, ldy, ldres, a_bs, b_bs, y_bs, res_bs, temb_stride;
+    int64_t res_rows;
     int64_t Nb;
     int64_t temb_group;
     int Ma, Ma_store;
@@ -922,6 +923,7 @@
 #pragma unroll
             for (int e = 0; e < 8; ++e) f[e] = co + e < Mo ? (float)v[e] : 0.0f;
             const bool full = vec_ok && co + 8 <= Mo;
+            const int64_t pr = g.res_rows > 0 ? (int64_t)((uint32_t)px % (uint32_t)g.res_rows) : px;
             if (full) {
                 if (g.temb != nullptr) {
                     const half8_t t = fz_ld_h8(g.temb + (px / g.temb_group) * g.temb_stride + co);
@@ -929,7 +931,7 @@
                     for (int e = 0; e < 8; ++e) f[e] += (float)t[e];
                 }
                 if (R1 != nullptr) {
-                    const half8_t r = fz_ld_h8(R1 + px * g.ldres + co);
+                    const half8_t r = fz_ld_h8(R1 + pr * g.ldres + co);
 #pragma unroll
                     for (int e = 0; e < 8; ++e) f[e] += (float)r[e];
                 }
@@ -945,7 +947,7 @@
                         if (co + e < Mo) f[e] += (float)t[e];
                 }
                 if (R1 != nullptr) {
-                    const half_t* r = R1 + px * g.ldres + co;
+                    const half_t* r = R1 + pr * g.ldres + co;
                     for (int e = 0; e < 8; ++e)
                         if (co + e < Mo) f[e] += (float)r[e];
                 }
@@ -1070,7 +1072,8 @@
         const float* const p0 = g.part + row * g.Ma;
         const int64_t slab = (int64_t)batch * g.Nb * g.Ma;
         const half_t* const trow = g.temb != nullptr ? g.temb + (px / g.temb_group) * g.temb_stride : nullptr;
-        const half_t* const r1 = g.res != nullptr ? g.res + (int64_t)z * g.res_bs + px * g.ldres : nullptr;
+        const int64_t pr = g.res_rows > 0 ? px % g.res_rows : px;
+        const half_t* const r1 = g.res != nullptr ? g.res + (int64_t)z * g.res_bs + pr * g.ldres : nullptr;
         const half_t* const r2 = g.res2 != nullptr ? g.res2 + (int64_t)z * g.res_bs + px * g.ldres : nullptr;
         half_t* const yrow = g.y + (int64_t)z * g.y_bs + px * g.ldy;
         const int c4 = (int)blockIdx.y * 64 + cl;
@@ -1473,6 +1476,8 @@
     g.res2 = (const half_t*)res2;
     g.ldres = d->ldres ? d->ldres : d->ldy;
     g.res_bs = d->res_batch_stride;
+    if (d->res_rows < 0 || (d->res_rows > 0 && (batch != 1 || d->transpose_out || d->rows >= (1ll << 31)))) return FZ_ERR_BAD_ARG;
+    g.res_rows = (res != nullptr && d->res_rows > 0 && d->res_rows < d->rows) ? d->res_rows : 0;
     g.y = (half_t*)y;
     g.ldy = d->ldy;
     g.y_bs = d->y_batch_stride;
@@ -1646,6 +1651,8 @@
     g.y = (half_t*)y;
     g.ldy = d->ldy;
     g.ldres = d->ldres ? d->ldres : d->ldy;
+    if (d->res_rows < 0 || (d->res_rows > 0 && d->rows >= (1ll << 31))) return FZ_ERR_BAD_ARG;
+    g.res_rows = (res != nullptr && d->res_rows > 0 && d->res_rows < d->rows) ? d->res_rows : 0;
     const bool want = ig_gs_setup(g, gn_partial, gn_groups, rows_per_frame);
     const int rc = ig_run<0, false>(g, 1, d->tile_cfg, 1, nullptr, 0, stream);
     return rc != FZ_OK ? rc : (want ? FZ_OK : FZ_GEMM_NO_STATS);
@@ -1674,6 +1681,8 @@
     g.y = (half_t*)y;
     g.ldy = d->ldy;
     g.ldres = d->ldres ? d->ldres : d->ldy;
+    if (d->res_rows < 0 || (d->res_rows > 0 && d->rows >= (1ll << 31))) return FZ_ERR_BAD_ARG;
+    g.res_rows = (res != nullptr && d->res_rows > 0 && d->res_rows < d->rows) ? d->res_rows : 0;
     g.lno_y = (half_t*)y_ln;
     g.lno_gamma = (const half_t*)gamma;
     g.lno_beta = (const half_t*)beta;
diff --git a/fatezero_amd/csrc/norms.hip b/fatezero_amd/csrc/norms.hip
--- a/fatezero_amd/csrc/norms.hip
+++ b/fatezero_amd/csrc/norms.hip
@@ -20,6 +20,7 @@
     const half_t* x;
     const half_t* x2;
     int C1;
+    int x2_frames;
     half_t* y;
     const half_t *gamma, *beta;
     float* partial;
@@ -45,7 +46,8 @@
     const float cnt = (float)((t1 - t0) * cg);
     const bool second = v * 8 >= a.C1;
     const int64_t rs = second ? a.C - a.C1 : a.C1;
-    const half_t* base = (second ? a.x2 + ((int64_t)n * a.tokens) * rs + (v * 8 - a.C1) : a.x + ((int64_t)n * a.tokens) * rs + v * 8);
+    const int n2 = a.x2_frames > 0 ? n % a.x2_frames : n;
+    const half_t* base = (second ? a.x2 + ((int64_t)n2 * a.tokens) * rs + (v * 8 - a.C1) : a.x + ((int64_t)n * a.tokens) * rs + v * 8);
     float s[8];
 #pragma unroll
     for (int e = 0; e < 8; ++e) s[e] = 0.0f;
@@ -228,7 +230,8 @@
     }
     const bool second = v * 8 >= a.C1;
     const int64_t rs = second ? a.C - a.C1 : a.C1;
-    const half_t* xb = (second ? a.x2 + ((int64_t)n * a.tokens) * rs + (v * 8 - a.C1) : a.x + ((int64_t)n * a.tokens) * rs + v * 8);
+    const int n2 = a.x2_frames > 0 ? n % a.x2_frames : n;
+    const half_t* xb = (second ? a.x2 + ((int64_t)n2 * a.tokens) * rs + (v * 8 - a.C1) : a.x + ((int64_t)n * a.tokens) * rs + v * 8);
     half_t* yb = a.y + ((int64_t)n * a.tokens) * a.C + v * 8;
 #pragma unroll 4
     for (int t = t0 + r; t < t1; t += a.R) {
@@ -272,7 +275,8 @@
     const int64_t row0 = (int64_t)sp * a.span * a.tokens;
     const uint32_t rs1 = (uint32_t)a.C1, rs2 = (uint32_t)(a.C - a.C1);
     const half_t* const src1 = a.x + row0 * a.C1;
-    const half_t* const src2 = a.x2 != nullptr ? a.x2 + row0 * (a.C - a.C1) : src1;
+    const int64_t row0_2 = a.x2_frames > 0 ? (int64_t)((sp * a.span) % a.x2_frames) * a.tokens : row0;
+    const half_t* const src2 = a.x2 != nullptr ? a.x2 + row0_2 * (a.C - a.C1) : src1;
     half_t* const dst = a.y + row0 * a.C + c0;
     const int drow = GN_FUSED_THREADS / P, dpr = GN_FUSED_THREADS - drow * P;
     const int row = tid / P, pr = tid - row * P;
@@ -358,7 +362,8 @@
     const int64_t row0 = (int64_t)sp * rows;
     const bool second = ch >= a.C1;
     const uint32_t rs = (uint32_t)(second ? a.C - a.C1 : a.C1);
-    const half_t* const src = second ? a.x2 + row0 * (a.C - a.C1) + (ch - a.C1) : a.x + row0 * a.C1 + ch;
+    const int64_t row0_2 = a.x2_frames > 0 ? (int64_t)((sp * a.span) % a.x2_frames) * a.tokens : row0;
+    const half_t* const src = second ? a.x2 + row0_2 * (a.C - a.C1) + (ch - a.C1) : a.x + row0 * a.C1 + ch;
     half_t* const dst = a.y + row0 * a.C + ch;
     const uint32_t step_in = (uint32_t)R * rs, step_out = (uint32_t)R * (uint32_t)a.C;
     const int r_first = active ? r0 : 0;
@@ -480,6 +485,7 @@
     if (n_frames <= 0 || span <= 0 || n_frames % span || channels % 8 || channels % groups || groups > 64)
         return FZ_ERR_BAD_ARG;
     a.n_frames = n_frames; a.span = span; a.fin_span = span; a.tokens = tokens; a.C = channels; a.G = groups;
+    a.x2_frames = 0;
     a.tb = gn_tb(tokens, channels);
     a.chunks = fz_groupnorm_chunks(tokens, channels);
     a.pchunks = a.chunks;
@@ -516,15 +522,17 @@
 
 extern "C" int fz_groupnorm_cat(const void* x1, int channels1, const void* x2, int channels2, void* y, const void* gamma,
                                 const void* beta, int n_frames, int span, int tokens, int groups, float eps, int silu, float* partial,
-                                void* stream) {
+                                int x2_frames, void* stream) {
     if (!x1 || !x2 || !y || !gamma || !beta || !partial || channels1 <= 0 || channels2 <= 0 || (channels1 % 8) || (channels2 % 8))
         return FZ_ERR_BAD_ARG;
+    if (x2_frames < 0 || (x2_frames > 0 && (span <= 0 || x2_frames % span || n_frames % x2_frames))) return FZ_ERR_BAD_ARG;
     GnArgs a;
     int threads;
     size_t smem;
     const int rc = gn_setup(a, n_frames, span, tokens, channels1 + channels2, groups, threads, smem);
     if (rc != FZ_OK) return rc;
     a.x = (const half_t*)x1; a.x2 = (const half_t*)x2; a.C1 = channels1;
+    a.x2_frames = x2_frames < n_frames ? x2_frames : 0;
     a.y = (half_t*)y; a.gamma = (const half_t*)gamma; a.beta = (const half_t*)beta;
     a.eps = eps; a.silu = silu;
     a.partial = partial;
diff --git a/fatezero_amd/csrc/xattn_chain.hip b/fatezero_amd/csrc/xattn_chain.hip
--- a/fatezero_amd/csrc/xattn_chain.hip
+++ b/fatezero_amd/csrc/xattn_chain.hip
@@ -83,6 +83,7 @@
     half_t* y1;
     int64_t rows, rows_per_frame;
     int frames_per_batch, lk;
+    int in_frames;
     float cs;
     float eps, eps1;
 };
@@ -97,7 +98,9 @@
     const int q8 = nt >> 3, r8 = nt & 7, xcd = bid & 7;
     const int blk = (xcd < r8 ? xcd * (q8 + 1) : r8 * (q8 + 1) + (xcd - r8) * q8) + (bid >> 3);
     const int64_t row0 = (int64_t)blk * XC_ROWS + pair * 32;
-    const int batch = (int)(((int64_t)blk * XC_ROWS / g.rows_per_frame) / g.frames_per_batch);
+    const int64_t frame = (int64_t)blk * XC_ROWS / g.rows_per_frame;
+    const int batch = (int)(frame / g.frames_per_batch);
+    const int64_t in_shift = g.in_frames > 0 ? (frame % g.in_frames - frame) * g.rows_per_frame : 0;
     const char* const kv = g.kvpack + (int64_t)batch * (XC_H * XC_KVH * XC_FRAG);
     const char* const wmain = g.wpack + (FRONT ? XC_FRONTF * XC_FRAG : 0);
     unsigned char* const hbase = raw + XC_HOFF + pair * XC_HPAIR * XC_FRAG;
@@ -158,7 +161,7 @@
         half8_t xb[XC_KS];
         const int64_t row = row0 + l31;
         {
-            const half_t* src = g.xn + row * XC_C + hi * 8;
+            const half_t* src = g.xn + (row + in_shift) * XC_C + hi * 8;
 #pragma unroll
             for (int s = 0; s < XC_KS; ++s) xb[s] = fz_ld_h8(src + s * 16);
         }
@@ -440,7 +443,7 @@
         for (int c = 0; c < XC_CT; ++c) yacc[c] = fz_zero_f16v();
         if constexpr (FRONT) {
             const int64_t row = row0 + l31;
-            const half_t* rs = g.res + row * XC_C + hi * 8;
+            const half_t* rs = g.res + (row + in_shift) * XC_C + hi * 8;
             half8_t ra[8];
 #pragma unroll
             for (int f = 0; f < 6; ++f) ra[f] = fz_ld_h8(rs + f * 16);
@@ -545,7 +548,7 @@
             }
     }
     __syncthreads();
-    const half_t* resp = FRONT ? g.y1 : g.res;
+    const half_t* resp = FRONT ? g.y1 : (g.res != nullptr ? g.res + in_shift * XC_C : nullptr);
     const int l8 = lane & 7;
     FzRow5 gmv, btv;
     if (g.yln != nullptr) {
@@ -712,7 +715,7 @@
 extern "C" int fz_xattn_chain(const FzXattnChain* d, void* stream) {
     if (!d || !d->x || !d->packed || !d->kv_packed || !d->y) return FZ_ERR_BAD_ARG;
     if (!fz_xattn_chain_ok(d->rows, d->rows_per_frame, d->channels, d->heads, d->lk)) return FZ_ERR_UNSUPPORTED;
-    if (d->frames_per_batch <= 0) return FZ_ERR_BAD_ARG;
+    if (d->frames_per_batch <= 0 || d->in_frames < 0) return FZ_ERR_BAD_ARG;
     if (d->y_ln != nullptr && (!d->ln_gamma || !d->ln_beta)) return FZ_ERR_BAD_ARG;
     const bool front = d->front != 0;
     if (front && (!d->res || !d->y1)) return FZ_ERR_BAD_ARG;
@@ -731,6 +734,7 @@
     g.rows_per_frame = d->rows_per_frame;
     g.frames_per_batch = d->frames_per_batch;
     g.lk = d->lk;
+    g.in_frames = d->in_frames > 0 && (int64_t)d->in_frames * d->rows_per_frame < d->rows ? d->in_frames : 0;
     g.cs = d->scale * 1.4426950408889634f;
     g.eps = d->ln_eps;
     g.eps1 = d->ln1_eps;
diff --git a/fatezero_amd/issue.py b/fatezero_amd/issue.py
--- a/fatezero_amd/issue.py
+++ b/fatezero_amd/issue.py
@@ -101,8 +101,9 @@
 
 
 def _model_switches():
-    from .video_diffusion.models import attention as A, lora as Lo, resnet as R
-    return (A.QKV_FUSION, A.LN_FROM_PRODUCER, R.GN_FROM_EPILOGUE, Lo.LORA_PAIR_FUSION, Lo.LORA_PAIR_GN, Lo.LORA_PAIR_ALWAYS)
+    from .video_diffusion.models import attention as A, lora as Lo, resnet as R, unet_3d_condition as U
+    return (A.QKV_FUSION, A.LN_FROM_PRODUCER, A.FF_CHAIN, A.XATTN_CHAIN, A.XATTN_CHAIN_FRONT, R.GN_FROM_EPILOGUE, R.CONV_UP2,
+            Lo.LORA_PAIR_FUSION, Lo.LORA_PAIR_GN, Lo.LORA_PAIR_ALWAYS, U.CFG_SHARED_HEAD)
 
 
 class ForwardPlan:
@@ -249,7 +250,7 @@
             sig = None if sig_fn is None or getattr(controller, "attention_plan", None) is None else sig_fn()
             if sig is None:
                 return None
-        return (tuple(x.data.shape), x.b, x.f, x.h, x.w, str(x.data.device), K._scratch_key(x.data)[1], tuple(temb_act.shape), tuple(ctx.shape),
+        return (tuple(x.data.shape), x.b, x.rep, x.f, x.h, x.w, str(x.data.device), K._scratch_key(x.data)[1], tuple(temb_act.shape), tuple(ctx.shape),
                 ctx.dtype, type(controller), sig, _model_switches())
 
     @classmethod
diff --git a/fatezero_amd/kernels.py b/fatezero_amd/kernels.py
--- a/fatezero_amd/kernels.py
+++ b/fatezero_amd/kernels.py
@@ -280,8 +280,9 @@
 def groupnorm_cat(x1: torch.Tensor, x2: torch.Tensor, gamma: torch.Tensor, beta: torch.Tensor, *, span: int, groups: int, eps: float,
                   silu: bool) -> torch.Tensor:
     n, tokens, c1 = x1.shape
-    c2 = x2.shape[2]
-    if not (x1.is_contiguous() and x2.is_contiguous() and x2.shape[:2] == x1.shape[:2] and x1.dtype == x2.dtype == torch.float16
+    n2, c2 = x2.shape[0], x2.shape[2]
+    if not (x1.is_contiguous() and x2.is_contiguous() and x2.shape[1] == tokens and 0 < n2 <= n and n % n2 == 0 and n2 % span == 0
+            and x1.dtype == x2.dtype == torch.float16
             and gamma.dtype == beta.dtype == torch.float16 and gamma.numel() == c1 + c2):
         raise ValueError("fz_groupnorm_cat: two contiguous fp16 tensors [N, tokens, C1] / [N, tokens, C2], gamma / beta over C1 + C2")
     _chk16(x1, x2, gamma, beta)
@@ -297,7 +298,7 @@
         _scratch_gen[0] += 1
     out = torch.empty(n, tokens, c, dtype=torch.float16, device=x1.device)
     N.check(N.lib().fz_groupnorm_cat(x1.data_ptr(), c1, x2.data_ptr(), c2, out.data_ptr(), gamma.data_ptr(), beta.data_ptr(), n, span,
-                                     tokens, groups, eps, 1 if silu else 0, buf.data_ptr(), _stream(x1)), "fz_groupnorm_cat")
+                                     tokens, groups, eps, 1 if silu else 0, buf.data_ptr(), n2 if n2 < n else 0, _stream(x1)), "fz_groupnorm_cat")
     return out
 
 
@@ -343,19 +344,20 @@
 
 
 def gemm_gn(x: torch.Tensor, w: torch.Tensor, bias: Optional[torch.Tensor], *, res: Optional[torch.Tensor] = None, gn_groups: int,
-            rows_per_frame: int):
+            rows_per_frame: int, tile_cfg: int = 0):
     k, o = x.shape[-1], w.shape[0]
     rows = x.numel() // k
     if not gn_epilogue_ok(rows_per_frame, o, gn_groups) or rows % rows_per_frame or not x.is_contiguous():
         return _gemm_unwrapped(x, w, bias, res=res), None
     _chk16(x, w, bias, res)
     y = torch.empty(tuple(x.shape[:-1]) + (o,), dtype=torch.float16, device=x.device)
-    if res is not None and (not res.is_contiguous() or res.shape != y.shape):
+    res_rows = _res_rows(res, rows, o)
+    if res is not None and (not res.is_contiguous() or (res.shape != y.shape and not res_rows)):
         return _gemm_unwrapped(x, w, bias, res=res), None
     d = N.FzGemmDesc()
     d.rows, d.in_features, d.out_features = rows, k, o
     d.ldx, d.ldw, d.ldy, d.ldres = k, w.stride(0), o, o
-    d.batch, d.epilogue = 1, N.FZ_GEMM_PLAIN
+    d.batch, d.epilogue, d.res_rows, d.tile_cfg = 1, N.FZ_GEMM_PLAIN, res_rows, tile_cfg
     partial = torch.empty(rows // rows_per_frame, gn_groups, rows_per_frame // 128, 3, dtype=torch.float32, device=x.device)
     rc = N.lib().fz_gemm_gn(C.byref(d), x.data_ptr(), w.data_ptr(), None if bias is None else bias.data_ptr(),
                             None if res is None else res.data_ptr(), None, y.data_ptr(), partial.data_ptr(), gn_groups, rows_per_frame,
@@ -365,6 +367,17 @@
     if rc:
         N.check(rc, "fz_gemm_gn")
     return y, partial
+
+
+def _res_rows(res: Optional[torch.Tensor], rows: int, ow: int) -> int:
+    if res is None:
+        return 0
+    rr = res.numel() // ow
+    if rr == rows:
+        return 0
+    if rr <= 0 or rows % rr or res.numel() != rr * ow:
+        raise ValueError(f"fz_gemm: a residual of {rr} rows cannot be broadcast over {rows} output rows")
+    return rr
 
 
 def pack_conv3x3_weight(w: torch.Tensor) -> torch.Tensor:
@@ -427,7 +440,7 @@
          res2: Optional[torch.Tensor] = None, out: Optional[torch.Tensor] = None, geglu: bool = False, tile_cfg: int = 0,
          split_k: int = 0):
     key = (x.shape, x.stride(), w.shape, w.stride(0), geglu, tile_cfg, split_k, x.device,
-           None if res is None else res.stride(), res2 is not None, None if out is None else (out.shape, out.stride()))
+           None if res is None else (res.stride(), res.numel()), res2 is not None, None if out is None else (out.shape, out.stride()))
     plan = _gemm_plans.get(key)
     if plan is None:
         plan = _gemm_plans[key] = _gemm_plan(x, w, bias, res, res2, out, geglu, tile_cfg, split_k)
@@ -467,6 +480,7 @@
     d.rows, d.in_features, d.out_features = rows, k, o
     d.ldx, d.ldw, d.ldy, d.ldres = k, w.stride(0), o, o
     d.batch, d.epilogue, d.tile_cfg, d.split_k = 1, N.FZ_GEMM_PLAIN, tile_cfg, split_k
+    d.res_rows = _res_rows(res, rows, o)
     want_ws = o % 4 == 0 and (k >= 1024 or split_k > 1) and 2 * rows * o <= _WS_FLOATS
     if want_ws:
         d.workspace_floats = _WS_FLOATS
@@ -526,9 +540,11 @@
     d.ldx, d.ldw, d.ldy = ldx, w.stride(0), ldy
     d.batch, d.epilogue = 1, (N.FZ_GEMM_GEGLU if geglu else N.FZ_GEMM_PLAIN)
     d.tile_cfg, d.split_k = tile_cfg, split_k
+    d.res_rows = _res_rows(res, rows, ow)
     for r in (res, res2):
         if r is not None:
-            assert r.shape[-1] == ow and r.stride(-1) == 1 and r.numel() // ow == rows and r.dtype == torch.float16
+            assert r.shape[-1] == ow and r.stride(-1) == 1 and r.dtype == torch.float16
+            assert r.numel() // ow == rows or (r is res and d.res_rows and r.is_contiguous())
     if res is not None:
         d.ldres = res.stride(-2) if res.dim() > 1 else ow
         if res2 is not None:
@@ -664,8 +680,11 @@
 
 
 def xattn_chain(x: torch.Tensor, packed: torch.Tensor, kv_packed: torch.Tensor, bias_out: Optional[torch.Tensor], *, res: Optional[torch.Tensor],
-                frames_per_batch: int, heads: int, lk: int, scale: float, ln=None, front_eps: Optional[float] = None):
-    n, l, c = x.shape
+                frames_per_batch: int, heads: int, lk: int, scale: float, ln=None, front_eps: Optional[float] = None, out_frames: int = 0):
+    n_in, l, c = x.shape
+    n = out_frames or n_in
+    if n % n_in:
+        raise ValueError("fz_xattn_chain: out_frames must be a multiple of the input's frames")
     rows = n * l
     front = front_eps is not None
     ts = [x] + ([] if res is None else [res])
@@ -681,21 +700,22 @@
         raise ValueError("fz_xattn_chain: `kv_packed` does not cover the batch")
     d = N.FzXattnChain()
     keep = [x, res, bias_out]
-    y = torch.empty_like(x)
+    y = torch.empty(n, l, c, dtype=x.dtype, device=x.device)
     yln = None
+    d.in_frames = n_in if n_in < n else 0
     d.x, d.res, d.packed, d.kv_packed, d.bias_out, d.y = x.data_ptr(), _ptr(res), packed.data_ptr(), kv_packed.data_ptr(), _ptr(bias_out), y.data_ptr()
     if ln is not None:
         gam, bet, eps = ln
         if gam.dtype != torch.float16 or bet.dtype != torch.float16:
             raise ValueError("fz_xattn_chain: LayerNorm weight / bias must be fp16")
-        yln = torch.empty_like(x)
+        yln = torch.empty_like(y)
         d.y_ln, d.ln_gamma, d.ln_beta, d.ln_eps = yln.data_ptr(), gam.data_ptr(), bet.data_ptr(), float(eps)
         keep += [gam, bet]
     y1 = None
     if front:
         if res is None:
             raise ValueError("fz_xattn_chain: the front form needs the residual")
-        y1 = torch.empty_like(x)
+        y1 = torch.empty_like(y)
         d.front, d.y1, d.ln1_eps = 1, y1.data_ptr(), float(front_eps)
     _chk16(*[t for t in keep if t is not None])
     d.rows, d.rows_per_frame, d.frames_per_batch, d.channels, d.heads, d.lk, d.scale = rows, l, frames_per_batch, c, heads, lk, float(scale)
@@ -941,5 +961,14 @@
     return acc
 
 
+def repeat_frames(x: torch.Tensor, reps: int) -> torch.Tensor:
+    if x.dtype != torch.float16 or not x.is_contiguous() or x.numel() % 8 or reps < 1:
+        raise ValueError("fz_repeat: a contiguous fp16 tensor of a multiple of 8 elements")
+    _chk16(x)
+    out = torch.empty((reps * x.shape[0],) + tuple(x.shape[1:]), dtype=x.dtype, device=x.device)
+    N.check(N.lib().fz_repeat(x.data_ptr(), out.data_ptr(), x.numel(), reps, _stream(x)), "fz_repeat")
+    return out
+
+
 def version() -> str:
     return N.lib().fz_version().decode()
diff --git a/fatezero_amd/video_diffusion/models/attention.py b/fatezero_amd/video_diffusion/models/attention.py
--- a/fatezero_amd/video_diffusion/models/attention.py
+++ b/fatezero_amd/video_diffusion/models/attention.py
@@ -130,6 +130,7 @@
 
     def forward_cross_after(self, x: Tokens, o1, attn1_out, hs, norm_in, ctx, clip: int, ln_next):
         n, lq, c = o1.shape
+        n *= x.rep
         plan = _plan_for(self.controller, True, self.place_in_unet, n, clip, self.heads, lq, ctx.shape[1], o1.device)
         if plan is None or (plan.mode == K.FZ_ATTN_FLASH):
             _, _, kvp = self._context_kv(ctx, want_pack=True)
@@ -137,7 +138,7 @@
             g3, b3 = ln_next.packed(o1.device)
             bo = self.to_out[0].packed(o1.dtype, o1.device)[1]
             y, yln, _ = K.xattn_chain(o1, packed, kvp, bo, res=hs, frames_per_batch=clip, heads=self.heads, lk=ctx.shape[1], scale=self.scale,
-                                      ln=(g3, b3, ln_next.eps), front_eps=norm_in.eps)
+                                      ln=(g3, b3, ln_next.eps), front_eps=norm_in.eps, out_frames=n)
             return y, yln
         hs1, n_in = _out_proj(attn1_out, o1, hs, norm_in)
         if n_in is None:
@@ -157,6 +158,7 @@
 
     def forward_cross(self, x: Tokens, ctx, clip: int, residual=None, ln_next=None, plan=False):
         n, lq, c = x.data.shape
+        n *= x.rep
         ctrl = self.controller
         if plan is False:
             if (ln_next is not None and residual is not None and residual.is_contiguous()
@@ -168,7 +170,10 @@
                     g3, b3 = ln_next.packed(xn.device)
                     return K.xattn_chain(xn, self._chain_weights(xn.device), kvp, self.to_out[0].packed(xn.dtype, xn.device)[1],
                                          res=residual, frames_per_batch=clip, heads=self.heads, lk=ctx.shape[1], scale=self.scale,
-                                         ln=(g3, b3, ln_next.eps))
+                                         ln=(g3, b3, ln_next.eps), out_frames=n)
+        if x.rep > 1:
+            residual = None if residual is None else K.repeat_frames(residual.contiguous(), x.rep)
+            x = x.expanded()
         q = self.to_q.apply(x.data)
         kk, vt, _ = self._context_kv(ctx)
         lk = ctx.shape[1]
@@ -263,7 +268,17 @@
 
 class SparseCausalAttention(CrossAttention):
 
-    def forward_self(self, x: Tokens, clip: int, index_list, residual=None, ln_next=None, raw_out=False):
+    def self_plan(self, x: Tokens, clip: int, index_list):
+        n, lq, _ = x.data.shape
+        return _plan_for(self.controller, False, self.place_in_unet, n * x.rep, clip, self.heads, lq, max(1, len(index_list)) * lq, x.data.device)
+
+    @staticmethod
+    def plan_is_plain(plan, lq):
+        if plan is None:
+            return lq > 32 ** 2
+        return plan.mode == K.FZ_ATTN_FLASH and plan.capture_first is None
+
+    def forward_self(self, x: Tokens, clip: int, index_list, residual=None, ln_next=None, raw_out=False, plan=False):
         n, lq, c = x.data.shape
         xn = x.data
         d_head = self.inner_dim // self.heads
@@ -294,7 +309,10 @@
         out = torch.empty(n, lq, self.inner_dim, dtype=xn.dtype, device=xn.device)
         n_kv = max(1, len(index_list))
         ctrl = self.controller
-        plan = _plan_for(ctrl, False, self.place_in_unet, n, clip, self.heads, lq, n_kv * lq, xn.device)
+        if plan is False:
+            plan = _plan_for(ctrl, False, self.place_in_unet, n * x.rep, clip, self.heads, lq, n_kv * lq, xn.device)
+        if x.rep > 1 and not self.plan_is_plain(plan, lq):
+            raise RuntimeError("forward_self: a CFG-shared input needs a plain attention plan (expand it first)")
         if plan is None:
             if lq > 32 ** 2:
                 K.attn_self(q, kk, vt, out, mode=K.FZ_ATTN_FLASH, **kw)
@@ -405,15 +423,23 @@
         clip = x.f
         lnp = LN_FROM_PRODUCER and hs.shape[-1] == LN_FROM_PRODUCER_C and hs.dtype == torch.float16 and D.active_shard() is None
         n1 = prenorm1 if prenorm1 is not None else layer_norm_tokens(self.norm1, hs)
+        plan1 = False
+        if x.rep > 1:
+            plan1 = self.attn1.self_plan(x, clip, self.sc_index)
+            if not self.attn1.plan_is_plain(plan1, hs.shape[1]):
+                hs, n1 = K.repeat_frames(hs.contiguous(), x.rep), K.repeat_frames(n1.contiguous(), x.rep)
+                x = Tokens(hs, x.b, x.f, x.h, x.w)
+        n_all = hs.shape[0] * x.rep
         if (lnp and XATTN_CHAIN_FRONT and hs.is_contiguous()
-                and self.attn2._chain_applies(hs.shape[0], hs.shape[1], hs.shape[2], hs.dtype, ctx)):
-            o1 = self.attn1.forward_self(x.like(n1), clip, self.sc_index, raw_out=True)
+                and self.attn2._chain_applies(n_all, hs.shape[1], hs.shape[2], hs.dtype, ctx)):
+            o1 = self.attn1.forward_self(x.like(n1), clip, self.sc_index, raw_out=True, plan=plan1)
             hs, n3 = self.attn2.forward_cross_after(x, o1, self.attn1.to_out[0], hs, self.norm2, ctx, clip, self.norm3)
         else:
-            hs, n2 = self.attn1.forward_self(x.like(n1), clip, self.sc_index, residual=hs, ln_next=self.norm2 if lnp else None)
+            hs, n2 = self.attn1.forward_self(x.like(n1), clip, self.sc_index, residual=hs, ln_next=self.norm2 if lnp else None, plan=plan1)
             if n2 is None:
                 n2 = layer_norm_tokens(self.norm2, hs)
             hs, n3 = self.attn2.forward_cross(x.like(n2), ctx, clip, residual=hs, ln_next=self.norm3 if lnp else None)
+        x = Tokens(hs, x.b, x.f, x.h, x.w)
         if n3 is None:
             n3 = layer_norm_tokens(self.norm3, hs)
         hs, nt = self.ff.apply(n3, res=hs, ln_next=self.norm_temporal if lnp else None)
@@ -452,10 +478,10 @@
         from .resnet import GN_FROM_EPILOGUE
         if GN_FROM_EPILOGUE and D.active_shard() is None:
             y, part = self.proj_out.apply_gn(h.data, res=x.data, groups=self.norm.num_groups, rows_per_frame=x.data.shape[1])
-            out = x.like(y)
+            out = h.like(y)
             out.gn = None if part is None else (part, self.norm.num_groups)
             return out
-        return x.like(self.proj_out.apply(h.data, res=x.data))
+        return h.like(self.proj_out.apply(h.data, res=x.data))
 
 
 class _Conv1x1Params(nn.Module):
diff --git a/fatezero_amd/video_diffusion/models/resnet.py b/fatezero_amd/video_diffusion/models/resnet.py
--- a/fatezero_amd/video_diffusion/models/resnet.py
+++ b/fatezero_amd/video_diffusion/models/resnet.py
@@ -14,17 +14,29 @@
 
 
 class Tokens:
-    __slots__ = ("data", "b", "f", "h", "w", "gn")
-
-    def __init__(self, data, b, f, h, w, gn=None):
-        self.data, self.b, self.f, self.h, self.w, self.gn = data, b, f, h, w, gn
+    __slots__ = ("data", "b", "f", "h", "w", "gn", "rep")
+
+    def __init__(self, data, b, f, h, w, gn=None, rep=1):
+        self.data, self.b, self.f, self.h, self.w, self.gn, self.rep = data, b, f, h, w, gn, rep
+        if b % rep:
+            raise ValueError(f"Tokens: a batch of {b} cannot be {rep} copies of anything")
 
     @property
     def c(self):
         return self.data.shape[-1]
 
+    @property
+    def nb(self):
+        return self.b // self.rep
+
     def like(self, data, h=None, w=None):
-        return Tokens(data, self.b, self.f, self.h if h is None else h, self.w if w is None else w)
+        return Tokens(data, self.b, self.f, self.h if h is None else h, self.w if w is None else w, rep=self.rep)
+
+    def expanded(self):
+        if self.rep == 1:
+            return self
+        d = self.data if self.data.is_contiguous() else self.data.contiguous()
+        return Tokens(K.repeat_frames(d, self.rep), self.b, self.f, self.h, self.w)
 
     @staticmethod
     def cat(a, b):
@@ -43,13 +55,18 @@
     __slots__ = ("parts", "_cat")
 
     def __init__(self, a: Tokens, b: Tokens):
+        if a.rep != 1:
+            a = a.expanded()
         self.parts, self._cat = (a.data, b.data), None
-        self.b, self.f, self.h, self.w, self.gn = a.b, a.f, a.h, a.w, None
+        self.b, self.f, self.h, self.w, self.gn, self.rep = a.b, a.f, a.h, a.w, None, 1
 
     @property
     def data(self):
         if self._cat is None:
-            self._cat = torch.cat(self.parts, dim=-1)
+            p0, p1 = self.parts
+            if p1.shape[0] != p0.shape[0]:
+                p1 = K.repeat_frames(p1.contiguous(), p0.shape[0] // p1.shape[0])
+            self._cat = torch.cat((p0, p1), dim=-1)
         return self._cat
 
     @property
@@ -108,6 +125,9 @@
         probe = x.parts[0] if isinstance(x, CatTokens) and x._cat is None else x.data
         w, bias, wtt, btt = self._pack(probe.dtype, probe.device)
         n, hw = probe.shape[0], probe.shape[1]
+        nb = x.nb
+        if temb is not None and temb.shape[0] != nb:
+            temb = temb[:nb]
         lora = self.conv_temporal if isinstance(self.conv_temporal, LoRALinearLayer) else None
         plain_t = self.conv_temporal is not None and lora is None and wtt is not None
         temporal_active = plain_t or (lora is not None and not lora.is_noop(probe.dtype, probe.device))
@@ -115,7 +135,10 @@
         if self.kernel_size == 1 and isinstance(x, CatTokens) and x._cat is None and residual is None and temb is None \
                 and x.parts[0].shape[-1] % 8 == 0:
             c1 = x.parts[0].shape[-1]
-            y = K.gemm(x.parts[1], w[:, c1:], None, res=K.gemm(x.parts[0], w[:, :c1], bias))
+            if x.parts[1].shape[0] != x.parts[0].shape[0]:
+                y = K.gemm(x.parts[0], w[:, :c1], bias, res=K.gemm(x.parts[1], w[:, c1:], None))
+            else:
+                y = K.gemm(x.parts[1], w[:, c1:], None, res=K.gemm(x.parts[0], w[:, :c1], bias))
             oh, ow = x.h, x.w
             fused = fuse_tail
         elif self.kernel_size == 1:
@@ -137,16 +160,16 @@
                 fused = fuse_tail
         gn = None
         if lora is not None and temporal_active:
-            y4 = lora.forward_tokens(y.view(x.b, x.f, oh * ow, self.out_channels), temb=temb, residual=residual, gn_groups=gn_groups)
+            y4 = lora.forward_tokens(y.view(nb, x.f, oh * ow, self.out_channels), temb=temb, residual=residual, gn_groups=gn_groups)
             if isinstance(y4, tuple):
                 y4, part = y4
                 gn = None if part is None else (part, gn_groups)
             y = y4.reshape(n, oh * ow, self.out_channels)
             fused = True
         elif plain_t:
-            rows = btt[None, :].expand(x.b, -1) if temb is None else temb + btt
+            rows = btt[None, :].expand(nb, -1) if temb is None else temb + btt
             shard = D.active_shard()
-            y4 = y.view(x.b, x.f, oh * ow, self.out_channels)
+            y4 = y.view(nb, x.f, oh * ow, self.out_channels)
             if shard is not None:
                 y4 = temporal_conv_tokens(shard.with_halo(y4, 1, 1, zero_outside=True, tag="temporal_conv"), wtt, rows_add=rows.contiguous())[:, 1:-1]
                 y = y4.reshape(n, oh * ow, self.out_channels)
@@ -157,7 +180,7 @@
             fused = True
         if not fused:
             if temb is not None:
-                y = (y.view(x.b, x.f * oh * ow, self.out_channels) + temb[:, None, :]).view(n, oh * ow, self.out_channels)
+                y = (y.view(nb, x.f * oh * ow, self.out_channels) + temb[:, None, :]).view(n, oh * ow, self.out_channels)
             if residual is not None:
                 y = y + residual
         out = x.like(y, oh, ow)
@@ -193,13 +216,13 @@
         return x.like(y)
     if not lazy and x.gn is not None and x.gn[1] == norm.num_groups and x.gn[0].shape[0] == x.data.shape[0]:
         y = K.groupnorm_from_partial(x.data, g, b, x.gn[0], span=(x.f if span_frames else 1), groups=norm.num_groups, eps=norm.eps, silu=silu)
-        return Tokens(y, x.b, x.f, x.h, x.w)
+        return x.like(y)
     if isinstance(x, CatTokens) and x._cat is None and x.parts[0].shape[-1] % 8 == 0 and x.parts[1].shape[-1] % 8 == 0:
         y = K.groupnorm_cat(x.parts[0], x.parts[1], g, b, span=(x.f if span_frames else 1), groups=norm.num_groups, eps=norm.eps,
                             silu=silu)
         return Tokens(y, x.b, x.f, x.h, x.w)
     y = K.groupnorm(x.data, g, b, span=(x.f if span_frames else 1), groups=norm.num_groups, eps=norm.eps, silu=silu)
-    return Tokens(y, x.b, x.f, x.h, x.w)
+    return x.like(y)
 
 
 def upsample_nearest2x(x: Tokens) -> Tokens:
diff --git a/fatezero_amd/video_diffusion/models/unet_3d_blocks.py b/fatezero_amd/video_diffusion/models/unet_3d_blocks.py
--- a/fatezero_amd/video_diffusion/models/unet_3d_blocks.py
+++ b/fatezero_amd/video_diffusion/models/unet_3d_blocks.py
@@ -60,6 +60,7 @@
 
     def forward_tokens(self, x: Tokens, temb_act, ctx=None):
         outs = []
+        x = x.expanded()
         for resnet in self.resnets:
             x = resnet.forward_tokens(x, temb_act)
             outs.append(x)
@@ -82,7 +83,7 @@
                                                       resnet_groups, model_config, use_linear_projection)])
 
     def forward_tokens(self, x: Tokens, temb_act, ctx):
-        x = self.resnets[0].forward_tokens(x, temb_act)
+        x = self.resnets[0].forward_tokens(x.expanded(), temb_act)
         x = self.attentions[0].forward_tokens(x, ctx)
         return self.resnets[1].forward_tokens(x, temb_act)
 
@@ -113,6 +114,7 @@
                                                               model_config=model_config)])
 
     def forward_tokens(self, x: Tokens, skips, temb_act, ctx):
+        x = x.expanded()
         for resnet, attn in zip(self.resnets, self.attentions):
             x = resnet.forward_tokens(_cat_skip(x, skips.pop()), temb_act)
             x = attn.forward_tokens(x, ctx)
@@ -140,6 +142,7 @@
                                                               model_config=model_config)])
 
     def forward_tokens(self, x: Tokens, skips, temb_act, ctx=None):
+        x = x.expanded()
         for resnet in self.resnets:
             x = resnet.forward_tokens(_cat_skip(x, skips.pop()), temb_act)
         if self.upsamplers is not None:
diff --git a/fatezero_amd/video_diffusion/models/unet_3d_condition.py b/fatezero_amd/video_diffusion/models/unet_3d_condition.py
--- a/fatezero_amd/video_diffusion/models/unet_3d_condition.py
+++ b/fatezero_amd/video_diffusion/models/unet_3d_condition.py
@@ -59,6 +59,12 @@
 
 
 TIME_EMBED_CACHE = True
+CFG_SHARED_HEAD = True
+
+
+def cfg_shared_head_active():
+    from ... import dist as D
+    return CFG_SHARED_HEAD and D.active_shard() is None
 
 
 class UNetPseudo3DConditionModel(nn.Module):
@@ -212,6 +218,8 @@
     def forward_tokens(self, x: Tokens, timestep, ctx) -> Tokens:
         from ... import kernels as K
         K.refresh_stream()
+        if x.rep > 1 and not cfg_shared_head_active():
+            x = x.expanded()
         temb_act = self.time_embed(timestep, x.b, x.data.device)
         ctx = ctx.to(torch.float16)
         issuer = self._issuer
diff --git a/fatezero_amd/video_diffusion/pipelines/p2p_ddim_spatial_temporal.py b/fatezero_amd/video_diffusion/pipelines/p2p_ddim_spatial_temporal.py
--- a/fatezero_amd/video_diffusion/pipelines/p2p_ddim_spatial_temporal.py
+++ b/fatezero_amd/video_diffusion/pipelines/p2p_ddim_spatial_temporal.py
@@ -7,28 +7,30 @@
 from ... import dist as fz_dist
 from ... import kernels as K
 from ..models.resnet import Tokens
+from ..models.unet_3d_condition import cfg_shared_head_active
 from ..prompt_attention import attention_util, spatial_blend
 from .stable_diffusion import SpatioTemporalStableDiffusionPipeline, StableDiffusionPipelineOutput
 
 
 class _LatentState:
 
-    def __init__(self, latents: torch.Tensor, reps: int):
+    def __init__(self, latents: torch.Tensor, reps: int, share: bool = True):
         b, c, f, h, w = latents.shape
         if b != 1:
             raise ValueError("Only support single video editing")
         self.f, self.h, self.w, self.reps = f, h, w, reps
+        self.copies = 1 if (reps > 1 and share and cfg_shared_head_active()) else reps
         self.z = latents[0].to(torch.float32, copy=True).reshape(c, f, h * w).contiguous()
-        self.tok = torch.empty(reps * f, h * w, c, dtype=torch.float16, device=latents.device)
+        self.tok = torch.empty(self.copies * f, h * w, c, dtype=torch.float16, device=latents.device)
         self.sync_tokens()
 
     def sync_tokens(self):
         t = self.z.permute(1, 2, 0).to(torch.float16)
-        for r in range(self.reps):
+        for r in range(self.copies):
             self.tok[r * self.f:(r + 1) * self.f].copy_(t)
 
     def tokens(self) -> Tokens:
-        return Tokens(self.tok, self.reps, self.f, self.h, self.w)
+        return Tokens(self.tok, self.reps, self.f, self.h, self.w, rep=self.reps // self.copies)
 
     def as_latents(self, dtype) -> torch.Tensor:
         return self.z.view(1, self.z.shape[0], self.f, self.h, self.w).to(dtype)
@@ -39,7 +41,7 @@
 
     def update(self, eps_u, eps_c, guidance, cz, ce):
         K.latent_update(self.z, eps_u, eps_c, guidance, cz, ce, next_in=self.tok[: self.f])
-        for r in range(1, self.reps):
+        for r in range(1, self.copies):
             self.tok[r * self.f:(r + 1) * self.f].copy_(self.tok[: self.f])
 
 
@@ -230,7 +232,7 @@
         shard = self.frame_shard
         if shard is not None:
             latents = shard.local(latents, 2).contiguous()
-        state = _LatentState(latents.detach(), reps=2 if do_cfg else 1)
+        state = _LatentState(latents.detach(), reps=2 if do_cfg else 1, share=shard is None)
         emb = text_embeddings.to(torch.float16)
         n_t = len(timesteps)
         with fz_dist.frame_sharded(shard):
diff --git a/include/fatezero_hip.h b/include/fatezero_hip.h
--- a/include/fatezero_hip.h
+++ b/include/fatezero_hip.h
@@ -82,7 +82,7 @@
                  int tokens, int channels, int groups, float eps, int silu, float* partial, void* stream);
 
 int fz_groupnorm_cat(const void* x1, int channels1, const void* x2, int channels2, void* y, const void* gamma, const void* beta,
-                     int n_frames, int span, int tokens, int groups, float eps, int silu, float* partial, void* stream);
+                     int n_frames, int span, int tokens, int groups, float eps, int silu, float* partial, int x2_frames, void* stream);
 
 int fz_groupnorm_stats(const void* x, int n_frames, int tokens, int channels, int groups, float* partial, void* stream);
 int fz_groupnorm_apply(const void* x, void* y, const void* gamma, const void* beta, int n_frames, int span, int tokens,
@@ -106,6 +106,7 @@
     int32_t reserved0;
     int64_t workspace_floats;
     int64_t w_batch_stride;
+    int64_t res_rows;
 } FzGemmDesc;
 int64_t fz_gemm_workspace_floats(int64_t rows, int out_features, int batch);
 int fz_gemm(const FzGemmDesc* desc, const void* x, const void* w, const void* bias, const void* res, const void* res2,
@@ -137,6 +138,8 @@
     float scale;
     float ln_eps, ln1_eps;
     int32_t front;
+    int32_t in_frames;
+    int32_t reserved0;
 } FzXattnChain;
 int fz_xattn_chain_ok(int64_t rows, int64_t rows_per_frame, int channels, int heads, int lk);
 int fz_xattn_chain_preferred(int64_t rows, int64_t rows_per_frame, int channels, int heads, int lk);
@@ -200,6 +203,8 @@
 
 int fz_accumulate(float* acc, const void* x, int64_t n, void* stream);
 
+int fz_repeat(const void* x, void* y, int64_t n, int reps, void* stream);
+
 int fz_peer_put(const void* src, int64_t bytes, void* const* dst, uint32_t* const* flags, int n_dst, uint32_t epoch,
                 uint32_t* done_counter, void* stream);
 int fz_peer_wait(const uint32_t* flags, uint64_t sender_mask, uint32_t epoch, uint32_t* err, int64_t timeout_us, void* stream);
```

New measurement: 4.172 frames/s, median of 6. 1.01x the previous value.
